# intellerce/controlanimate

Hardware: AMD Instinct MI355X
Metric: frames_per_sec (higher is better)
Workload: dtype fp16

## Files before the change

controlanimate_amd/_capi.py:

```python
from __future__ import annotations

import ctypes as C
import os

_HERE = os.path.dirname(os.path.abspath(__file__))
LIB_PATH = os.environ.get("CA_HIP_LIB") or os.path.join(_HERE, "csrc", "libcontrolanimate_hip.so")

CA_BF16, CA_F16 = 0, 1
CA_ACT_NONE, CA_ACT_SILU = 0, 1
ABI_VERSION = 15


class CAHipUnavailable(RuntimeError):
    pass


class CAHipError(RuntimeError):
    pass


class GemmArgs(C.Structure):
    _fields_ = [
        ("a", C.c_void_p), ("a2", C.c_void_p), ("w", C.c_void_p), ("c", C.c_void_p),
        ("bias", C.c_void_p), ("rowbias", C.c_void_p), ("residual", C.c_void_p),
        ("lda", C.c_int64), ("lda2", C.c_int64), ("ldc", C.c_int64), ("ld_res", C.c_int64),
        ("ld_rowbias", C.c_int64),
        ("m", C.c_int32), ("n", C.c_int32), ("k1", C.c_int32), ("k2", C.c_int32),
        ("rows_per_group", C.c_int32),
        ("alpha", C.c_float), ("post_scale", C.c_float),
        ("act", C.c_int32), ("geglu", C.c_int32), ("out_f32", C.c_int32), ("dtype", C.c_int32),
        ("ln_stats", C.c_void_p), ("ln_colsum", C.c_void_p), ("ln_eps", C.c_float),
        ("workspace", C.c_void_p), ("workspace_bytes", C.c_int64),
        ("row_sums_out", C.c_void_p), ("ln_parts", C.c_int32),
        ("w_frag", C.c_void_p),
    ]


class FfArgs(C.Structure):
    _fields_ = [
        ("x", C.c_void_p), ("w1_frag", C.c_void_p), ("bias1", C.c_void_p), ("colsum1", C.c_void_p), ("ln_stats", C.c_void_p),
        ("w2_frag", C.c_void_p), ("bias2", C.c_void_p), ("residual", C.c_void_p), ("y", C.c_void_p),
        ("lda", C.c_int64), ("ldc", C.c_int64), ("ld_res", C.c_int64),
        ("m", C.c_int32), ("c", C.c_int32), ("inner", C.c_int32), ("ln_eps", C.c_float), ("dtype", C.c_int32),
        ("w_out_frag", C.c_void_p), ("bias_out", C.c_void_p), ("residual_out", C.c_void_p), ("ld_res_out", C.c_int64),
    ]


class TattnArgs(C.Structure):
    _fields_ = [
        ("x", C.c_void_p), ("w_frag", C.c_void_p), ("gamma", C.c_void_p), ("bias_pe", C.c_void_p), ("o", C.c_void_p),
        ("lda", C.c_int64), ("ldo", C.c_int64), ("ld_bias_pe", C.c_int64),
        ("batch", C.c_int32), ("frames", C.c_int32), ("tokens", C.c_int32), ("heads", C.c_int32), ("c", C.c_int32),
        ("ln_eps", C.c_float), ("scale", C.c_float), ("dtype", C.c_int32),
        ("w_out_frag", C.c_void_p), ("bias_out", C.c_void_p), ("residual", C.c_void_p), ("ld_res", C.c_int64),
    ]


ATTN_WOUT_FRAG_ELEMS = 102400
TATTN_W_FRAG_ELEMS = 368640


class XattnArgs(C.Structure):
    _fields_ = [
        ("x", C.c_void_p), ("wq_frag", C.c_void_p), ("bias", C.c_void_p), ("kv_frag", C.c_void_p), ("o", C.c_void_p),
        ("lda", C.c_int64), ("ldo", C.c_int64),
        ("m", C.c_int32), ("tokens", C.c_int32), ("frames_per_kv", C.c_int32), ("kv_mod", C.c_int32), ("kv_batches", C.c_int32),
        ("nk", C.c_int32), ("heads", C.c_int32), ("c", C.c_int32),
        ("ln_eps", C.c_float), ("dtype", C.c_int32),
        ("w_out_frag", C.c_void_p), ("bias_out", C.c_void_p), ("residual", C.c_void_p), ("ld_res", C.c_int64),
        ("kv_frag_ip", C.c_void_p), ("nk_ip", C.c_int32), ("ip_scale", C.c_float),
    ]


XATTN_W_FRAG_ELEMS = 122880
XATTN_KV_FRAG_ELEMS = 7680


class ConvArgs(C.Structure):
    _fields_ = [
        ("x", C.c_void_p), ("x2", C.c_void_p), ("w", C.c_void_p), ("y", C.c_void_p),
        ("bias", C.c_void_p), ("rowbias", C.c_void_p), ("residual", C.c_void_p),
        ("ld_res", C.c_int64), ("ld_rowbias", C.c_int64),
        ("images", C.c_int32), ("hin", C.c_int32), ("win", C.c_int32),
        ("cin1", C.c_int32), ("cin2", C.c_int32), ("cout", C.c_int32),
        ("stride", C.c_int32), ("upsample", C.c_int32), ("rows_per_group", C.c_int32),
        ("alpha", C.c_float), ("post_scale", C.c_float),
        ("act", C.c_int32), ("out_f32", C.c_int32), ("dtype", C.c_int32),
        ("workspace", C.c_void_p), ("workspace_bytes", C.c_int64), ("pad_asym", C.c_int32),
        ("w_wino", C.c_void_p), ("x_is_wino_v", C.c_int32),
    ]


class GroupNormArgs(C.Structure):
    _fields_ = [
        ("x", C.c_void_p), ("x2", C.c_void_p), ("y", C.c_void_p),
        ("gamma", C.c_void_p), ("beta", C.c_void_p), ("partials", C.c_void_p),
        ("images", C.c_int32), ("hw", C.c_int32), ("c1", C.c_int32), ("c2", C.c_int32),
        ("groups", C.c_int32), ("frames_per_stat", C.c_int32),
        ("eps", C.c_float), ("act", C.c_int32), ("dtype", C.c_int32),
        ("wino_v", C.c_void_p), ("wino_h", C.c_int32), ("wino_w", C.c_int32),
    ]


class LayerNormArgs(C.Structure):
    _fields_ = [
        ("x", C.c_void_p), ("y", C.c_void_p), ("gamma", C.c_void_p), ("beta", C.c_void_p),
        ("pos", C.c_void_p),
        ("rows", C.c_int64),
        ("c", C.c_int32), ("rows_per_frame", C.c_int32), ("frames", C.c_int32),
        ("eps", C.c_float), ("dtype", C.c_int32), ("stats", C.c_void_p),
    ]


class AttnArgs(C.Structure):
    _fields_ = [
        ("q", C.c_void_p), ("k", C.c_void_p), ("v", C.c_void_p), ("o", C.c_void_p),
        ("q_outer", C.c_int64), ("q_inner", C.c_int64), ("q_row", C.c_int64),
        ("o_outer", C.c_int64), ("o_inner", C.c_int64), ("o_row", C.c_int64),
        ("k_outer", C.c_int64), ("k_inner", C.c_int64), ("k_row", C.c_int64),
        ("inner_count", C.c_int32), ("kv_inner_count", C.c_int32), ("kv_div", C.c_int32), ("kv_mod", C.c_int32),
        ("batches", C.c_int32), ("heads", C.c_int32), ("head_dim", C.c_int32),
        ("nq", C.c_int32), ("nk", C.c_int32),
        ("scale", C.c_float), ("out_scale", C.c_float),
        ("accumulate", C.c_int32), ("dtype", C.c_int32), ("causal", C.c_int32),
        ("key_mask", C.c_void_p), ("key_mask_stride", C.c_int64),
    ]


class ConvNarrowArgs(C.Structure):
    _fields_ = [
        ("x", C.c_void_p), ("w", C.c_void_p), ("y", C.c_void_p), ("bias", C.c_void_p), ("r1", C.c_void_p), ("r2", C.c_void_p),
        ("ldx", C.c_int64), ("ldy", C.c_int64), ("ld_r1", C.c_int64), ("ld_r2", C.c_int64),
        ("images", C.c_int32), ("hin", C.c_int32), ("win", C.c_int32), ("cin", C.c_int32), ("cout", C.c_int32),
        ("channel_offset", C.c_int32), ("upsample", C.c_int32), ("leaky_relu", C.c_int32),
        ("s0", C.c_float), ("s1", C.c_float), ("s2", C.c_float),
        ("out_u8", C.c_int32), ("dtype", C.c_int32),
    ]


SYMBOLS = {
    "ca_abi_version": (C.c_int, []),
    "ca_last_error": (C.c_char_p, []),
    "ca_gemm": (C.c_int, [C.POINTER(GemmArgs), C.c_void_p]),
    "ca_pack_w_frag": (C.c_int, [C.c_void_p, C.c_int32, C.c_int32, C.c_int32, C.c_void_p, C.c_void_p]),
    "ca_pack_w2_frag": (C.c_int, [C.c_void_p, C.c_int32, C.c_int32, C.c_void_p, C.c_void_p]),
    "ca_ff_fused": (C.c_int, [C.POINTER(FfArgs), C.c_void_p]),
    "ca_ff_fused_supported": (C.c_int, [C.POINTER(FfArgs)]),
    "ca_tattn_fused": (C.c_int, [C.POINTER(TattnArgs), C.c_void_p]),
    "ca_tattn_fused_supported": (C.c_int, [C.POINTER(TattnArgs)]),
    "ca_pack_w_tattn": (C.c_int, [C.c_void_p, C.c_int32, C.c_int32, C.c_void_p, C.c_void_p]),
    "ca_pack_w_out": (C.c_int, [C.c_void_p, C.c_int32, C.c_int32, C.c_void_p, C.c_void_p]),
    "ca_xattn_fused": (C.c_int, [C.POINTER(XattnArgs), C.c_void_p]),
    "ca_xattn_fused_supported": (C.c_int, [C.POINTER(XattnArgs)]),
    "ca_xattn_pack_w": (C.c_int, [C.c_void_p, C.c_int32, C.c_int32, C.c_void_p, C.c_void_p]),
    "ca_xattn_pack_kv": (C.c_int, [C.c_void_p, C.c_int64, C.c_int32, C.c_int32, C.c_int32, C.c_int32, C.c_float, C.c_int32, C.c_void_p, C.c_void_p]),
    "ca_gemm_ln_inline_supported": (C.c_int, [C.POINTER(GemmArgs)]),
    "ca_gemm_wants_finished_stats": (C.c_int, [C.POINTER(GemmArgs)]),
    "ca_ln_finish_sums": (C.c_int, [C.c_void_p, C.c_int, C.c_int64, C.c_int, C.c_float, C.c_void_p, C.c_void_p]),
    "ca_gemm_workspace_bytes": (C.c_int64, [C.POINTER(GemmArgs)]),
    "ca_gemm_row_sums_parts": (C.c_int, [C.POINTER(GemmArgs)]),
    "ca_gemm_plan_name": (C.c_int, [C.POINTER(GemmArgs), C.c_char_p, C.c_int32]),
    "ca_conv3x3_plan_name": (C.c_int, [C.POINTER(ConvArgs), C.c_char_p, C.c_int32]),
    "ca_conv3x3": (C.c_int, [C.POINTER(ConvArgs), C.c_void_p]),
    "ca_pack_w_wino": (C.c_int, [C.c_void_p, C.c_int32, C.c_int32, C.c_int32, C.c_void_p, C.c_void_p]),
    "ca_conv3x3_workspace_bytes": (C.c_int64, [C.POINTER(ConvArgs)]),
    "ca_softmax_rows": (C.c_int, [C.c_void_p, C.c_void_p, C.c_int64, C.c_int32, C.c_int64, C.c_int64, C.c_float, C.c_int32, C.c_void_p]),
    "ca_groupnorm_partials_floats": (C.c_int64, [C.c_int32, C.c_int32, C.c_int32, C.c_int32]),
    "ca_groupnorm_stats": (C.c_int, [C.POINTER(GroupNormArgs), C.c_void_p]),
    "ca_groupnorm_apply": (C.c_int, [C.POINTER(GroupNormArgs), C.c_void_p]),
    "ca_groupnorm": (C.c_int, [C.POINTER(GroupNormArgs), C.c_void_p]),
    "ca_groupnorm_wino_supported": (C.c_int, [C.POINTER(GroupNormArgs)]),
    "ca_layernorm": (C.c_int, [C.POINTER(LayerNormArgs), C.c_void_p]),
    "ca_attention": (C.c_int, [C.POINTER(AttnArgs), C.c_void_p]),
    "ca_attention_plan_name": (C.c_int, [C.POINTER(AttnArgs), C.c_char_p, C.c_int32]),
    "ca_add_bcast": (C.c_int, [C.c_void_p, C.c_void_p, C.c_void_p, C.c_int64, C.c_int64, C.c_int32, C.c_void_p]),
    "ca_repeat": (C.c_int, [C.c_void_p, C.c_void_p, C.c_int64, C.c_int32, C.c_void_p]),
    "ca_silu_f32": (C.c_int, [C.c_void_p, C.c_void_p, C.c_int64, C.c_void_p]),
    "ca_timestep_embedding": (C.c_int, [C.c_void_p, C.c_float, C.c_void_p, C.c_int32, C.c_int32, C.c_int32, C.c_void_p]),
    "ca_latents_to_nhwc": (C.c_int, [C.c_void_p, C.c_void_p, C.c_int32, C.c_int32, C.c_int32, C.c_int32, C.c_int32,
                                      C.c_int32, C.c_int32, C.c_float, C.c_int32, C.c_void_p]),
    "ca_nhwc_to_ncfhw_f32": (C.c_int, [C.c_void_p, C.c_void_p, C.c_int32, C.c_int32, C.c_int32, C.c_int32, C.c_int32,
                                        C.c_int32, C.c_int32, C.c_int32, C.c_void_p]),
    "ca_ncfhw_to_nhwc": (C.c_int, [C.c_void_p, C.c_int32, C.POINTER(C.c_int64), C.c_void_p, C.c_int32, C.c_int32,
                                    C.c_int32, C.c_int32, C.c_int32, C.c_int32, C.c_int32, C.c_void_p]),
    "ca_cfg_scheduler_step": (C.c_int, [C.c_void_p, C.c_int32, C.c_int32, C.c_float, C.c_void_p, C.c_void_p,
                                         C.c_void_p, C.c_void_p, C.c_int32, C.c_int32, C.c_int32, C.c_int32,
                                         C.POINTER(C.c_float), C.c_float, C.c_void_p]),
    "ca_lincomb": (C.c_int, [C.c_void_p, C.POINTER(C.c_void_p), C.POINTER(C.c_float), C.c_int32, C.c_int64, C.c_void_p]),
    "ca_conv3x3_narrow": (C.c_int, [C.POINTER(ConvNarrowArgs), C.c_void_p]),
    "ca_conv3x3_narrow_plan_name": (C.c_int, [C.POINTER(ConvNarrowArgs), C.c_char_p, C.c_int32]),
    "ca_rgb8_to_nhwc": (C.c_int, [C.c_void_p, C.c_void_p, C.c_int32, C.c_int32, C.c_int32, C.c_int32, C.c_void_p]),
    "ca_resize_lanczos4_u8": (C.c_int, [C.c_void_p, C.c_void_p, C.c_int32, C.c_int32, C.c_int32, C.c_int32, C.c_int32,
                                         C.c_void_p, C.c_void_p, C.c_void_p, C.c_void_p, C.c_void_p]),
    "ca_color_match_workspace_bytes": (C.c_int64, [C.c_int32, C.c_int64]),
    "ca_hist_u8x3": (C.c_int, [C.c_void_p, C.c_void_p, C.c_int32, C.c_int64, C.c_void_p]),
    "ca_color_moments_f64": (C.c_int, [C.c_void_p, C.c_void_p, C.c_void_p, C.c_void_p, C.c_int32, C.c_int64, C.c_void_p, C.c_int64, C.c_void_p]),
    "ca_color_transform_f64": (C.c_int, [C.c_void_p, C.c_void_p, C.c_void_p, C.c_void_p, C.c_void_p, C.c_void_p, C.c_int32, C.c_int64, C.c_void_p]),
    "ca_sort_f64_segments": (C.c_int, [C.c_void_p, C.c_void_p, C.c_int32, C.c_int64, C.c_void_p, C.c_int64, C.c_void_p]),
    "ca_color_rank_map_f64": (C.c_int, [C.c_void_p, C.c_void_p, C.c_void_p, C.c_void_p, C.c_void_p, C.c_void_p, C.c_int32, C.c_int64,
                                         C.c_void_p, C.c_int64, C.c_void_p]),
    "ca_color_finish_u8": (C.c_int, [C.c_void_p, C.c_void_p, C.c_int32, C.c_int64, C.c_int32, C.c_void_p, C.c_int64, C.c_void_p]),
}

_lib = None


def lib() -> C.CDLL:
    global _lib
    if _lib is not None:
        return _lib
    import torch
    if not os.path.exists(LIB_PATH):
        raise CAHipUnavailable(
            f"{LIB_PATH} is missing: the HIP extension is not built. Run "
            "`python -m controlanimate_amd._build` (needs hipcc); there is no CPU fallback.")
    try:
        handle = C.CDLL(LIB_PATH)
    except OSError as e:
        raise CAHipUnavailable(f"cannot load {LIB_PATH}: {e}") from e
    for name, (res, args) in SYMBOLS.items():
        fn = getattr(handle, name)
        fn.restype = res
        fn.argtypes = args
    if handle.ca_abi_version() != ABI_VERSION:
        raise CAHipUnavailable(f"ABI mismatch: library {handle.ca_abi_version()} vs binding {ABI_VERSION}; rebuild")
    _lib = handle
    return handle


def check(rc: int, what: str) -> None:
    if rc != 0:
        msg = lib().ca_last_error()
        raise CAHipError(f"{what} failed with code {rc}: {msg.decode() if msg else ''}")
```

controlanimate_amd/attention_processor.py:

```python
from __future__ import annotations

from typing import Optional

import torch
from torch import nn

from . import kernels as K
from .context import dispatch
from .layers import HipLinear, LnFold, WeightArena, ln_fold_enabled, pack_concat_rows


class AttnProcessor2_0(nn.Module):

    num_tokens = 0
    drop_ip_tokens = False

    def __init__(self, hidden_size=None, cross_attention_dim=None):
        super().__init__()

    def ip_branch(self, attn, q, ctx, out, images, tokens, kv_rows, frames_per_kv, kv_mod, cache):
        return out

    def ip_fragments(self, attn, ctx, cache):
        return None

    def __call__(self, attn: "Attention", hidden_states: torch.Tensor, encoder_hidden_states: Optional[torch.Tensor] = None,
                 attention_mask=None, temb=None, *, residual: Optional[torch.Tensor] = None, frames_per_kv: int = 1,
                 kv_mod: int = 0, temporal=None, cache: Optional[dict] = None, ln=None, row_sums: bool = False) -> torch.Tensor:
        if attention_mask is not None:
            raise NotImplementedError("attention_mask is not used anywhere on the reference's path")
        B, N, C = hidden_states.shape
        x = hidden_states.reshape(B * N, C)
        res = None if residual is None else residual.reshape(B * N, C)
        if ln is not None and encoder_hidden_states is None and temporal is not None and getattr(attn, "tfrag", None) is not None:
            b, f, n = temporal
            ofrag = getattr(attn, "ofrag", None)
            if ofrag is not None and dispatch.attn_out_fused:
                to_out = attn.to_out[0]
                out = K.tattn_fused(x, attn.tfrag.t, attn.tgamma.t, attn.tbias_pe.t, b, f, n, attn.heads, attn.tln_eps, attn.scale,
                                    w_out_frag=ofrag.t, bias_out=None if to_out.b is None else to_out.b.t, residual=res)
                if out is not None:
                    return out.reshape(B, N, C)
            o = K.tattn_fused(x, attn.tfrag.t, attn.tgamma.t, attn.tbias_pe.t, b, f, n, attn.heads, attn.tln_eps, attn.scale)
            if o is not None:
                out = attn.to_out[0].run(o, residual=res, row_sums=row_sums)
                return K.carry_row_sums(out.reshape(B, N, C), out)
        builtin = type(self).ip_branch is AttnProcessor2_0.ip_branch
        with_ip = (not builtin and type(self).ip_fragments is not AttnProcessor2_0.ip_fragments and dispatch.attn_out_fused and dispatch.xattn_ip_fused
                   and getattr(attn, "ofrag", None) is not None)
        if (ln is not None and encoder_hidden_states is not None and cache is not None and getattr(attn, "xfrag", None) is not None
                and (builtin or with_ip)):
            ctx = encoder_hidden_states
            nb, L, cd = ctx.shape
            nk = L - self.num_tokens
            kv = cache.get(("kv", id(attn)))
            if kv is None:
                kv = cache[("kv", id(attn))] = K.gemm(ctx.reshape(nb * L, cd), attn.kv.t)
            ent = cache.get(("kvf", id(attn)))
            if ent is None:
                ent = cache[("kvf", id(attn))] = (K.xattn_pack_kv(kv, nb, L, nk, attn.scale), nk, L)
            if ent[0] is not None and ent[1] == nk:
                ofrag = getattr(attn, "ofrag", None)
                if ofrag is not None and dispatch.attn_out_fused:
                    to_out = attn.to_out[0]
                    ipf = self.ip_fragments(attn, ctx, cache) if with_ip else None
                    if not with_ip or ipf is not None:
                        out = K.xattn_fused(x, attn.xfrag.t, ln[1].b.t, ent[0], B, N, frames_per_kv, kv_mod, nk, ln[1].eps, w_out_frag=ofrag.t,
                                            bias_out=None if to_out.b is None else to_out.b.t, residual=res,
                                            kv_frag_ip=None if ipf is None else ipf[0], nk_ip=0 if ipf is None else ipf[1],
                                            ip_scale=1.0 if ipf is None else ipf[2])
                        if out is not None:
                            return out.reshape(B, N, C)
                o = K.xattn_fused(x, attn.xfrag.t, ln[1].b.t, ent[0], B, N, frames_per_kv, kv_mod, nk, ln[1].eps) if builtin else None
                if o is not None:
                    out = attn.to_out[0].run(o, residual=res, row_sums=row_sums)
                    return K.carry_row_sums(out.reshape(B, N, C), out)
        if ln is not None:
            st, fold = ln
            if encoder_hidden_states is None and temporal is not None and fold.pe is not None:
                b, f, n = temporal
                qkv = K.gemm(x, fold.w.t, bias=fold.b.t, ln=(st, fold.cs.t), rowbias=fold.rowbias(b, f), rows_per_group=n)
            else:
                qkv = K.gemm(x, fold.w.t, bias=fold.b.t, ln=(st, fold.cs.t))
        if encoder_hidden_states is None:
            if ln is None:
                qkv = K.gemm(x, attn.qkv.t)
            if temporal is not None:
                b, f, n = temporal
                o = K.attention_temporal(qkv, b, f, n, attn.heads)
            else:
                o = K.attention_spatial(qkv, B, N, attn.heads)
        else:
            ctx = encoder_hidden_states
            nb, L, cd = ctx.shape
            q = qkv if ln is not None else K.gemm(x, attn.to_q.w.t)
            kv = None if cache is None else cache.get(("kv", id(attn)))
            if kv is None:
                kv = K.gemm(ctx.reshape(nb * L, cd), attn.kv.t)
                if cache is not None:
                    cache[("kv", id(attn))] = kv
            nk = L - self.num_tokens
            o = K.attention_cross(q, kv, B, N, attn.heads, nk, L, frames_per_kv, kv_mod=kv_mod)
            o = self.ip_branch(attn, q, ctx, o, B, N, L, frames_per_kv, kv_mod, cache)
        out = attn.to_out[0].run(o, residual=res, row_sums=row_sums)
        return K.carry_row_sums(out.reshape(B, N, C), out)


class IPAttnProcessor2_0(AttnProcessor2_0):

    def __init__(self, hidden_size, cross_attention_dim=None, scale=1.0, num_tokens=4):
        super().__init__()
        self.hidden_size = hidden_size
        self.cross_attention_dim = cross_attention_dim
        self.scale = scale
        self.num_tokens = num_tokens
        self.to_k_ip = HipLinear(cross_attention_dim or hidden_size, hidden_size, bias=False)
        self.to_v_ip = HipLinear(cross_attention_dim or hidden_size, hidden_size, bias=False)
        self.kv_ip = None

    def pack(self, arena: WeightArena, dtype):
        self.kv_ip = pack_concat_rows(arena, dtype, [self.to_k_ip, self.to_v_ip])

    def _kv_ip(self, ctx, cache):
        if self.kv_ip is None:
            raise RuntimeError("IPAttnProcessor2_0 installed after prepare(); call model.prepare() again")
        nb, L, cd = ctx.shape
        kvip = None if cache is None else cache.get(("kv_ip", id(self)))
        if kvip is None:
            kvip = K.gemm(ctx.reshape(nb * L, cd), self.kv_ip.t)
            if cache is not None:
                cache[("kv_ip", id(self))] = kvip
        return kvip

    def ip_fragments(self, attn, ctx, cache):
        nb, L, cd = ctx.shape
        if cache is None or not (1 <= self.num_tokens <= 16):
            return None
        ent = cache.get(("kvf_ip", id(self)))
        if ent is None:
            kvip = self._kv_ip(ctx, cache)
            ent = cache[("kvf_ip", id(self))] = (K.xattn_pack_kv(kvip, nb, L, self.num_tokens, attn.scale, row_offset=L - self.num_tokens),
                                                 self.num_tokens, L, attn.scale)
        if ent[0] is None or ent[1] != self.num_tokens or ent[2] != L:
            return None
        return ent[0], self.num_tokens, float(self.scale)

    def ip_branch(self, attn, q, ctx, out, images, tokens, kv_rows, frames_per_kv, kv_mod, cache):
        nb, L, cd = ctx.shape
        kvip = self._kv_ip(ctx, cache)
        return K.attention_cross(q, kvip, images, tokens, attn.heads, self.num_tokens, L, frames_per_kv, out=out,
                                 out_scale=float(self.scale), accumulate=True, kv_row_offset=L - self.num_tokens,
                                 kv_mod=kv_mod)


class CNAttnProcessor2_0(AttnProcessor2_0):

    def __init__(self, num_tokens=4):
        super().__init__()
        self.num_tokens = num_tokens


AttnProcessor = AttnProcessor2_0
IPAttnProcessor = IPAttnProcessor2_0
CNAttnProcessor = CNAttnProcessor2_0


class Attention(nn.Module):

    def __init__(self, query_dim: int, cross_attention_dim: Optional[int] = None, heads: int = 8, dim_head: int = 64,
                 dropout: float = 0.0, bias: bool = False, upcast_attention: bool = False, processor=None, **_):
        super().__init__()
        inner = heads * dim_head
        self.is_cross = cross_attention_dim is not None
        ctx_dim = cross_attention_dim if self.is_cross else query_dim
        self.query_dim, self.cross_attention_dim, self.inner_dim = query_dim, ctx_dim, inner
        self.heads = heads
        self.scale = dim_head ** -0.5
        self.spatial_norm = None
        self.group_norm = None
        self.norm_cross = None
        self.residual_connection = False
        self.rescale_output_factor = 1.0
        self.to_q = HipLinear(query_dim, inner, bias=bias)
        self.to_k = HipLinear(ctx_dim, inner, bias=bias)
        self.to_v = HipLinear(ctx_dim, inner, bias=bias)
        self.to_out = nn.ModuleList([HipLinear(inner, query_dim, bias=True), nn.Identity()])
        self.processor = processor if processor is not None else AttnProcessor2_0()
        self.qkv = self.kv = self.fold = None

    def set_processor(self, processor, _remove_lora: bool = False):
        if isinstance(getattr(self, "processor", None), nn.Module) and not isinstance(processor, nn.Module):
            self._modules.pop("processor", None)
        self.processor = processor

    def get_processor(self, return_deprecated_lora: bool = False):
        return self.processor

    def builtin_processor(self) -> bool:
        return type(self.processor) in (AttnProcessor2_0, IPAttnProcessor2_0, CNAttnProcessor2_0)

    def pack(self, arena: WeightArena, dtype, fold_ln=None, pe=None):
        self.fold = None
        if fold_ln is not None and self.builtin_processor() and ln_fold_enabled():
            self.fold = LnFold(arena, dtype, fold_ln, [self.to_q] if self.is_cross else [self.to_q, self.to_k, self.to_v], pe=pe)
            if self.is_cross:
                self.kv = pack_concat_rows(arena, dtype, [self.to_k, self.to_v])
                self.xfrag = None
                if (self.heads, self.inner_dim, self.query_dim) == (8, 320, 320):
                    from .layers import frag_order_xattn
                    fold = self.fold
                    self.xfrag = arena.add((122880,), dtype, lambda: frag_order_xattn(fold.w_fold().to(dtype).float()))
        elif self.is_cross:
            self.to_q.pack(arena, dtype)
            self.kv = pack_concat_rows(arena, dtype, [self.to_k, self.to_v])
        else:
            self.qkv = pack_concat_rows(arena, dtype, [self.to_q, self.to_k, self.to_v])
        self.to_out[0].pack(arena, dtype)
        self.ofrag = None
        if (self.heads, self.inner_dim, self.query_dim) == (8, 320, 320) and self.fold is not None:
            from .layers import _f32, frag_order_wout
            to_out = self.to_out[0]
            self.ofrag = arena.add((102400,), dtype, lambda: frag_order_wout(_f32(to_out.weight)))
        if hasattr(self.processor, "pack"):
            self.processor.pack(arena, dtype)

    def forward(self, hidden_states, encoder_hidden_states=None, attention_mask=None, **kw):
        return self.processor(self, hidden_states, encoder_hidden_states=encoder_hidden_states,
                              attention_mask=attention_mask, **kw)
```

controlanimate_amd/context.py:

```python
from __future__ import annotations

from dataclasses import dataclass, field
from typing import Optional

import torch


@dataclass
class ExecCtx:
    b: int
    f: int
    dtype: torch.dtype
    temb: torch.Tensor
    emb_groups: int
    ehs: Optional[torch.Tensor] = None
    frames_per_kv: int = 1
    kv_mod: int = 0
    gn_frames_per_stat: int = 1
    cache: dict = field(default_factory=dict)

    @property
    def images(self) -> int:
        return self.b * self.f

    def rows_per_emb_group(self, h: int, w: int) -> int:
        return self.images // self.emb_groups * h * w


class Dispatch:
    gemm_ar = True
    ff_fused = True
    tattn_fused = True
    xattn_fused = True
    attn_out_fused = True
    xattn_ip_fused = True
    conv_winograd = True
    gn_winograd = True
    ln_row_sums = True
    repeat_kernel = True
    ln_fold = True
    cfg_shared = True
    cn_cfg_dedup = True
    controlnet_streams = 2


dispatch = Dispatch()
```

controlanimate_amd/csrc/ca_attn_out.h:

```cpp
__device__ __forceinline__ int ca_wout_col(int j, int i) { return j < 4 ? 32 * (j >> 1) + 8 * (i >> 2) + 4 * (j & 1) + (i & 3) : 64 + i; }

constexpr int CA_WOUT_ELEMS = 320 * 320;

__global__ __launch_bounds__(256) void k_pack_w_out(const u16* __restrict__ w, u16* __restrict__ dst) {
  const int idx = blockIdx.x * 256 + threadIdx.x;
  if (idx >= CA_WOUT_ELEMS / 8) return;
  const int L = idx & 63;
  int t = idx >> 6;
  const int j = t % 5;
  t /= 5;
  const int kq = t % 10;
  const int cg = t / 10;
  const int row = cg * 80 + ca_wout_col(j, L & 15);
  st16(dst + (int64_t)idx * 8, ld16(w + (int64_t)row * 320 + kq * 32 + (L >> 4) * 8));
}

__device__ __forceinline__ void ca_lds_store8(unsigned char* p, u32x2 v) {
  const unsigned addr = (unsigned)(size_t)(__attribute__((address_space(3))) unsigned char*)p;
  asm volatile("ds_write_b64 %0, %1" ::"v"(addr), "v"(v) : "memory");
}

struct AttnOutParams {
  const u16* wof;
  const float* bias;
  const u16* res;
  int ld_res;
  unsigned res_bytes;
};

struct AttnOutRegs {
  u32x4 fb[2][5];
  u32x4 rr[4][2];
  u32x2 r4[4];
};

__device__ __forceinline__ unsigned attn_out_row(unsigned row_base, unsigned step_a, unsigned step_b, int i) { return row_base + (unsigned)(i & 1) * step_a + (unsigned)(i >> 1) * step_b; }

template <int DT>
__device__ __forceinline__ void attn_out_prefetch(AttnOutRegs& R, const AttnOutParams& a, __amdgpu_buffer_rsrc_t rs_wo, __amdgpu_buffer_rsrc_t rs_res, int wid,
                                                  int lane, unsigned row_base, unsigned step_a, unsigned step_b) {
  const int cg = wid & 3, g = lane >> 4;
  const unsigned wv = (unsigned)lane * 16u;
  const unsigned wbase = (unsigned)cg * (10u * 5u * 1024u);
#pragma unroll
  for (int c = 0; c < 2; ++c)
#pragma unroll
    for (int j = 0; j < 5; ++j) R.fb[c][j] = __builtin_bit_cast(u32x4, __builtin_amdgcn_raw_buffer_load_b128(rs_wo, wv, wbase + (unsigned)(c * 5 + j) * 1024u, 0));
#pragma unroll
  for (int i = 0; i < 4; ++i) {
    const unsigned ro = attn_out_row(row_base, step_a, step_b, i) * (unsigned)a.ld_res * 2u + (unsigned)(cg * 80) * 2u;
    R.rr[i][0] = __builtin_bit_cast(u32x4, __builtin_amdgcn_raw_buffer_load_b128(rs_res, ro + (unsigned)(8 * g) * 2u, 0, 0));
    R.rr[i][1] = __builtin_bit_cast(u32x4, __builtin_amdgcn_raw_buffer_load_b128(rs_res, ro + (unsigned)(32 + 8 * g) * 2u, 0, 0));
    R.r4[i] = __builtin_bit_cast(u32x2, __builtin_amdgcn_raw_buffer_load_b64(rs_res, ro + (unsigned)(64 + 4 * g) * 2u, 0, 0));
  }
}

template <int DT>
__device__ __forceinline__ unsigned attn_out_add(unsigned w, unsigned r_) {
  if (DT == CA_F16) {
    unsigned s_;
    asm("v_pk_add_f16 %0, %1, %2" : "=v"(s_) : "v"(w), "v"(r_));
    return s_;
  }
  return pack2<DT>(Elem<DT>::to_f((u16)(w & 0xffffu)) + Elem<DT>::to_f((u16)(r_ & 0xffffu)), Elem<DT>::to_f((u16)(w >> 16)) + Elem<DT>::to_f((u16)(r_ >> 16)));
}

template <int DT>
__device__ __forceinline__ void attn_out_run(AttnOutRegs& R, const unsigned char* tile, const int (&fa_b)[2][2], const AttnOutParams& a,
                                             __amdgpu_buffer_rsrc_t rs_wo, __amdgpu_buffer_rsrc_t rs_bo, __amdgpu_buffer_rsrc_t rs_y, int wid, int lane,
                                             unsigned row_base, unsigned step_a, unsigned step_b, unsigned ldo) {
  constexpr int KQ = 10, ROWB = 640;
  const int rh = wid >> 2, cg = wid & 3;
  int lane_k = lane;
  asm volatile("" : "+v"(lane_k));
  const unsigned wv = (unsigned)lane_k * 16u;
  const unsigned wbase = (unsigned)cg * (10u * 5u * 1024u);
  f32x4 acc[4][5];
  u32x4 fa[4];
#pragma unroll
  for (int i = 0; i < 4; ++i) fa[i] = ld16(tile + fa_b[rh][0] + i * 16 * ROWB);
  __builtin_amdgcn_sched_barrier(0);
#pragma unroll
  for (int kq = 0; kq < KQ; ++kq) {
    const int nk = kq + 1;
    const int fa_off = (nk >> 1) * 128;
#pragma unroll
    for (int j = 0; j < 5; ++j) {
      __builtin_amdgcn_s_setprio(1);
#pragma unroll
      for (int i = 0; i < 4; ++i) {
        if (kq == 0) acc[i][j] = Elem<DT>::mfma(R.fb[0][j], fa[i], (f32x4){0.f, 0.f, 0.f, 0.f});
        else acc[i][j] = Elem<DT>::mfma(R.fb[kq & 1][j], fa[i], acc[i][j]);
        if (j == 4 && nk < KQ) {
          __builtin_amdgcn_sched_barrier(0);
          fa[i] = ld16(tile + fa_b[rh][nk & 1] + fa_off + i * 16 * ROWB);
          __builtin_amdgcn_sched_barrier(0);
        }
      }
      __builtin_amdgcn_s_setprio(0);
      __builtin_amdgcn_sched_barrier(0);
      if (kq + 2 < KQ) R.fb[kq & 1][j] = __builtin_bit_cast(u32x4, __builtin_amdgcn_raw_buffer_load_b128(rs_wo, wv, wbase + (unsigned)(((kq + 2) * 5 + j) * 1024), 0));
      __builtin_amdgcn_sched_barrier(0);
    }
  }
  int lane_e = lane;
  asm volatile("" : "+v"(lane_e));
  const int g = lane_e >> 4;
  f32x4 bi[5];
#pragma unroll
  for (int j = 0; j < 5; ++j) {
    const unsigned c4 = (unsigned)(cg * 80 + (j < 4 ? 32 * (j >> 1) + 8 * g + 4 * (j & 1) : 64 + 4 * g)) * 4u;
    bi[j] = __builtin_bit_cast(f32x4, __builtin_amdgcn_raw_buffer_load_b128(rs_bo, c4, 0, 0));
  }
  unsigned w[4][10];
#pragma unroll
  for (int i = 0; i < 4; ++i) {
#pragma unroll
    for (int j = 0; j < 5; ++j) {
      w[i][2 * j] = pack2<DT>(acc[i][j][0] + bi[j][0], acc[i][j][1] + bi[j][1]);
      w[i][2 * j + 1] = pack2<DT>(acc[i][j][2] + bi[j][2], acc[i][j][3] + bi[j][3]);
    }
    if (a.res) {
#pragma unroll
      for (int k = 0; k < 8; ++k) w[i][k] = attn_out_add<DT>(w[i][k], R.rr[i][k >> 2][k & 3]);
      w[i][8] = attn_out_add<DT>(w[i][8], R.r4[i][0]);
      w[i][9] = attn_out_add<DT>(w[i][9], R.r4[i][1]);
    }
  }
  __builtin_amdgcn_sched_barrier(0);
#pragma unroll
  for (int i = 0; i < 4; ++i) {
    const unsigned ro = attn_out_row(row_base, step_a, step_b, i) * ldo * 2u + (unsigned)(cg * 80) * 2u;
    __builtin_amdgcn_raw_buffer_store_b128((u32x4){w[i][0], w[i][1], w[i][2], w[i][3]}, rs_y, ro + (unsigned)(8 * g) * 2u, 0, 0);
    __builtin_amdgcn_raw_buffer_store_b128((u32x4){w[i][4], w[i][5], w[i][6], w[i][7]}, rs_y, ro + (unsigned)(32 + 8 * g) * 2u, 0, 0);
    __builtin_amdgcn_raw_buffer_store_b64((u32x2){w[i][8], w[i][9]}, rs_y, ro + (unsigned)(64 + 4 * g) * 2u, 0, 0);
  }
  __builtin_amdgcn_sched_barrier(0);
}
```

controlanimate_amd/csrc/ca_gemm_ar.hip:

```cpp
#include "ca_gemm_core.h"
#include <atomic>

__attribute__((visibility("hidden"))) int ar_cu_count() {
  static std::atomic<int> cache[64];
  int dev = 0;
  if (hipGetDevice(&dev) != hipSuccess || dev < 0 || dev >= 64) dev = 0;
  int n = cache[dev].load(std::memory_order_relaxed);
  if (n <= 0) {
    hipDeviceProp_t prop;
    n = (hipGetDeviceProperties(&prop, dev) == hipSuccess && prop.multiProcessorCount > 0) ? prop.multiProcessorCount : 256;
    cache[dev].store(n, std::memory_order_relaxed);
  }
  return n;
}

namespace {
using namespace ca_gemm_detail;
#include "ca_gemm_ar.h"
#include "ca_attn_out.h"
#include "ca_ff_fused.h"
#include "ca_tattn_fused.h"
#include "ca_xattn_fused.h"

template <int DT>
int launch_ar(const GemmKParams& p, hipStream_t st) {
  const int tiles_m = (p.m + 127) / 128;
  const unsigned c_bytes = (unsigned)((((int64_t)p.m - 1) * p.ldc + (p.geglu ? p.n / 2 : p.n)) * 2);
  const unsigned res_bytes = p.res ? (unsigned)((((int64_t)p.m - 1) * p.ld_res + p.n) * 2) : 0u;
  const int slots = 2 * ar_cu_count();
  const unsigned grid = (unsigned)(tiles_m < slots ? tiles_m : slots);
  float* ws = p.ln_inline ? p.partial : nullptr;
  if (p.geglu) hipLaunchKernelGGL((k_gemm_ar<DT, 2>), dim3(grid), dim3(256), 0, st, p, p.wf, tiles_m, c_bytes, 0u, ws);
  else if (p.ln_colsum) hipLaunchKernelGGL((k_gemm_ar<DT, 1>), dim3(grid), dim3(256), 0, st, p, p.wf, tiles_m, c_bytes, 0u, ws);
  else hipLaunchKernelGGL((k_gemm_ar<DT, 0>), dim3(grid), dim3(256), 0, st, p, p.wf, tiles_m, c_bytes, res_bytes, ws);
  return CA_OK;
}
}

int ca_launch_gemm_ar(const ca_gemm_detail::GemmKParams& p0, int dtype, hipStream_t st) {
  static const int dbg = CA_KNOB("CA_PP_DBG", 0);
  ca_gemm_detail::GemmKParams p = p0;
  p.dbg = dbg;
  return dtype == CA_BF16 ? launch_ar<CA_BF16>(p, st) : launch_ar<CA_F16>(p, st);
}

extern "C" int ca_pack_w_frag(const void* w, int32_t n, int32_t k, int32_t geglu, void* dst, void* stream) {
  CA_REQUIRE(w && dst, "ca_pack_w_frag: null operand");
  CA_REQUIRE(k == 320 && n > 0 && n % 64 == 0, "ca_pack_w_frag: n=%d (multiple of 64) k=%d (320)", n, k);
  CA_REQUIRE((((uintptr_t)w | (uintptr_t)dst) & 15) == 0, "ca_pack_w_frag: operands must be 16-byte aligned");
  const int64_t pieces = (int64_t)n * 40;
  hipLaunchKernelGGL(k_pack_w_frag, dim3((unsigned)((pieces + 255) / 256)), dim3(256), 0, (hipStream_t)stream, (const u16*)w, (u16*)dst, n, geglu);
  CA_CHECK_LAUNCH("ca_pack_w_frag");
  return CA_OK;
}

extern "C" int ca_pack_w2_frag(const void* w, int32_t n, int32_t k, void* dst, void* stream) {
  CA_REQUIRE(w && dst, "ca_pack_w2_frag: null operand");
  CA_REQUIRE(n == 320 && k == 1280, "ca_pack_w2_frag: n=%d k=%d (320 x 1280)", n, k);
  CA_REQUIRE((((uintptr_t)w | (uintptr_t)dst) & 15) == 0, "ca_pack_w2_frag: operands must be 16-byte aligned");
  hipLaunchKernelGGL(k_pack_w2_frag, dim3(200), dim3(256), 0, (hipStream_t)stream, (const u16*)w, (u16*)dst);
  CA_CHECK_LAUNCH("ca_pack_w2_frag");
  return CA_OK;
}

static int attn_out_args_ok(const void* w_out_frag, const float* bias_out, const void* residual, int64_t ld_res, int64_t rows) {
  if (!w_out_frag) return (bias_out || residual) ? 0 : 1;
  if ((((uintptr_t)w_out_frag | (uintptr_t)bias_out | (uintptr_t)residual) & 15) != 0) return 0;
  if (residual && (ld_res % 8 || ld_res < 320 || ((rows - 1) * ld_res + 320) * 2 >= 0x7FFFFF00ll)) return 0;
  return 1;
}

extern "C" int ca_ff_fused_supported(const ca_ff_args* a) {
  if (!a || !a->x || !a->w1_frag || !a->bias1 || !a->colsum1 || !a->w2_frag || !a->y) return 0;
  if (a->c != 320 || a->inner != 1280 || a->m < 16384) return 0;
  if (a->dtype != CA_BF16 && a->dtype != CA_F16) return 0;
  if (a->lda % 8 || a->ldc % 8 || (a->residual && a->ld_res % 8)) return 0;
  if (a->lda < 320 || a->ldc < 320 || (a->residual && a->ld_res < 320)) return 0;
  if ((((uintptr_t)a->x | (uintptr_t)a->y | (uintptr_t)a->w1_frag | (uintptr_t)a->w2_frag | (uintptr_t)a->residual) & 15) != 0) return 0;
  if (((uintptr_t)a->ln_stats & 7) != 0 || (((uintptr_t)a->bias1 | (uintptr_t)a->colsum1 | (uintptr_t)a->bias2) & 15) != 0) return 0;
  const int64_t lim = 0x7FFFFF00ll;
  if (((int64_t)(a->m - 1) * a->lda + 320) * 2 >= lim || ((int64_t)(a->m - 1) * a->ldc + 320) * 2 >= lim) return 0;
  if (a->residual && ((int64_t)(a->m - 1) * a->ld_res + 320) * 2 >= lim) return 0;
  if (!a->ln_stats && !(a->ln_eps > 0.f)) return 0;
  if (!attn_out_args_ok(a->w_out_frag, a->bias_out, a->residual_out, a->ld_res_out, a->m)) return 0;
  if (a->w_out_frag && a->m % 128) return 0;
  return 1;
}

extern "C" int ca_ff_fused(const ca_ff_args* a, void* stream) {
  CA_REQUIRE(a != nullptr, "ca_ff_fused: null args");
  CA_REQUIRE(ca_ff_fused_supported(a), "ca_ff_fused: arguments outside what the fused feed-forward takes (C = 320, inner 1280, M >= 16384, fragment-ordered weights, "
                                        "16-byte aligned operands, 32-bit byte offsets): ask ca_ff_fused_supported() first");
  FfParams p{};
  p.x = (const u16*)a->x;
  p.w1f = (const u16*)a->w1_frag;
  p.bias1 = a->bias1;
  p.cs1 = a->colsum1;
  p.w2f = (const u16*)a->w2_frag;
  p.bias2 = a->bias2;
  p.res = (const u16*)a->residual;
  p.y = (u16*)a->y;
  p.ln_stats = a->ln_stats;
  p.lda = a->lda, p.ldc = a->ldc, p.ld_res = a->ld_res;
  p.m = a->m;
  p.ln_eps = a->ln_eps;
  p.x_bytes = (unsigned)(((int64_t)(a->m - 1) * a->lda + 320) * 2);
  p.y_bytes = (unsigned)(((int64_t)(a->m - 1) * a->ldc + 320) * 2);
  p.res_bytes = a->residual ? (unsigned)(((int64_t)(a->m - 1) * a->ld_res + 320) * 2) : 0u;
  if (a->w_out_frag) {
    p.out.wof = (const u16*)a->w_out_frag;
    p.out.bias = a->bias_out;
    p.out.res = (const u16*)a->residual_out;
    p.out.ld_res = (int)a->ld_res_out;
    p.out.res_bytes = a->residual_out ? (unsigned)(((int64_t)(a->m - 1) * a->ld_res_out + 320) * 2) : 0u;
  }
  const int tiles_m = (a->m + 127) / 128;
  const unsigned grid = (unsigned)(tiles_m < ar_cu_count() ? tiles_m : ar_cu_count());
  if (a->w_out_frag) {
    if (a->dtype == CA_BF16) hipLaunchKernelGGL((k_ff_fused<CA_BF16, true>), dim3(grid), dim3(512), 0, (hipStream_t)stream, p, tiles_m);
    else hipLaunchKernelGGL((k_ff_fused<CA_F16, true>), dim3(grid), dim3(512), 0, (hipStream_t)stream, p, tiles_m);
  } else {
    if (a->dtype == CA_BF16) hipLaunchKernelGGL((k_ff_fused<CA_BF16, false>), dim3(grid), dim3(512), 0, (hipStream_t)stream, p, tiles_m);
    else hipLaunchKernelGGL((k_ff_fused<CA_F16, false>), dim3(grid), dim3(512), 0, (hipStream_t)stream, p, tiles_m);
  }
  CA_CHECK_LAUNCH("ca_ff_fused");
  return CA_OK;
}

extern "C" int ca_pack_w_tattn(const void* w, int32_t n, int32_t k, void* dst, void* stream) {
  CA_REQUIRE(w && dst, "ca_pack_w_tattn: null operand");
  CA_REQUIRE(n == 960 && k == 320, "ca_pack_w_tattn: n=%d k=%d (Wq | Wk | Wv rows: 960 x 320)", n, k);
  CA_REQUIRE((((uintptr_t)w | (uintptr_t)dst) & 15) == 0, "ca_pack_w_tattn: operands must be 16-byte aligned");
  static_assert(CA_TATTN_WF_ELEMS == CA_TATTN_W_FRAG_ELEMS, "header constant");
  hipLaunchKernelGGL(k_pack_w_tattn, dim3((CA_TATTN_WF_ELEMS / 8 + 255) / 256), dim3(256), 0, (hipStream_t)stream, (const u16*)w, (u16*)dst);
  CA_CHECK_LAUNCH("ca_pack_w_tattn");
  return CA_OK;
}

extern "C" int ca_pack_w_out(const void* w, int32_t n, int32_t k, void* dst, void* stream) {
  CA_REQUIRE(w && dst, "ca_pack_w_out: null operand");
  CA_REQUIRE(n == 320 && k == 320, "ca_pack_w_out: n=%d k=%d (to_out[0].weight: 320 x 320)", n, k);
  CA_REQUIRE((((uintptr_t)w | (uintptr_t)dst) & 15) == 0, "ca_pack_w_out: operands must be 16-byte aligned");
  static_assert(CA_WOUT_ELEMS == CA_ATTN_WOUT_FRAG_ELEMS, "header constant");
  hipLaunchKernelGGL(k_pack_w_out, dim3((CA_WOUT_ELEMS / 8 + 255) / 256), dim3(256), 0, (hipStream_t)stream, (const u16*)w, (u16*)dst);
  CA_CHECK_LAUNCH("ca_pack_w_out");
  return CA_OK;
}

extern "C" int ca_tattn_fused_supported(const ca_tattn_args* a) {
  if (!a || !a->x || !a->w_frag || !a->gamma || !a->bias_pe || !a->o) return 0;
  if (a->c != 320 || a->heads != 8 || a->batch < 1) return 0;
  if (a->frames != 16 && !((a->frames == 8 || a->frames == 32) && a->w_out_frag)) return 0;
  {
    const int px = 128 / a->frames;
    if (a->tokens < px || a->tokens % px) return 0;
  }
  if (a->dtype != CA_BF16 && a->dtype != CA_F16) return 0;
  const int64_t rows = (int64_t)a->batch * a->frames * a->tokens;
  if (rows < 16384) return 0;
  if (a->lda % 8 || a->ldo % 8 || a->lda < 320 || a->ldo < 320 || a->ld_bias_pe % 4 || a->ld_bias_pe < 320) return 0;
  if ((((uintptr_t)a->x | (uintptr_t)a->o | (uintptr_t)a->w_frag | (uintptr_t)a->gamma | (uintptr_t)a->bias_pe) & 15) != 0) return 0;
  const int64_t lim = 0x7FFFFF00ll;
  if (((rows - 1) * a->lda + 320) * 2 >= lim || ((rows - 1) * a->ldo + 320) * 2 >= lim) return 0;
  if (!(a->ln_eps > 0.f) || !(a->scale > 0.f)) return 0;
  if (!attn_out_args_ok(a->w_out_frag, a->bias_out, a->residual, a->ld_res, rows)) return 0;
  return 1;
}

extern "C" int ca_tattn_fused(const ca_tattn_args* a, void* stream) {
  CA_REQUIRE(a != nullptr, "ca_tattn_fused: null args");
  CA_REQUIRE(ca_tattn_fused_supported(a), "ca_tattn_fused: arguments outside what the fused temporal attention takes (C = 320, 8 heads, 16 frames -- or 8 / 32 with w_out_frag --, tokens %% (128 / frames) == 0, "
                                           ">= 16384 rows, fragment-ordered weights, 16-byte aligned operands, 32-bit byte offsets): ask ca_tattn_fused_supported() first");
  const int64_t rows = (int64_t)a->batch * a->frames * a->tokens;
  TattnParams p{};
  p.x = (const u16*)a->x;
  p.wf = (const u16*)a->w_frag;
  p.gamma = a->gamma;
  p.bp = a->bias_pe;
  p.o = (u16*)a->o;
  p.lda = (int)a->lda, p.ldo = (int)a->ldo, p.ld_bp = (int)a->ld_bias_pe;
  p.hw = a->tokens;
  p.ln_eps = a->ln_eps;
  p.scale_log2 = a->scale * 1.4426950408889634f;
  p.x_bytes = (unsigned)(((rows - 1) * a->lda + 320) * 2);
  p.o_bytes = (unsigned)(((rows - 1) * a->ldo + 320) * 2);
  const int tiles = (int)((int64_t)a->batch * a->tokens / (128 / a->frames));
  static const int dbg = CA_KNOB("CA_TATTN_DBG", 0);
  p.dbg = dbg;
  if (a->w_out_frag) {
    p.out.wof = (const u16*)a->w_out_frag;
    p.out.bias = a->bias_out;
    p.out.res = (const u16*)a->residual;
    p.out.ld_res = (int)a->ld_res;
    p.out.res_bytes = a->residual ? (unsigned)(((rows - 1) * a->ld_res + 320) * 2) : 0u;
    const unsigned grid1 = (unsigned)(tiles < ar_cu_count() ? tiles : ar_cu_count());
#define CA_TATTN_OUT(FR)                                                                                                              \
  if (a->dtype == CA_BF16) hipLaunchKernelGGL((k_tattn_out<CA_BF16, FR>), dim3(grid1), dim3(512), 0, (hipStream_t)stream, p, tiles); \
  else hipLaunchKernelGGL((k_tattn_out<CA_F16, FR>), dim3(grid1), dim3(512), 0, (hipStream_t)stream, p, tiles);
    if (a->frames == 8) { CA_TATTN_OUT(8) }
    else if (a->frames == 32) { CA_TATTN_OUT(32) }
    else { CA_TATTN_OUT(16) }
#undef CA_TATTN_OUT
    CA_CHECK_LAUNCH("ca_tattn_fused(out)");
    return CA_OK;
  }
  const int slots = (dbg & 16) ? ar_cu_count() : 2 * ar_cu_count();
  const unsigned grid = (unsigned)(tiles < slots ? tiles : slots);
  if (a->dtype == CA_BF16) hipLaunchKernelGGL((k_tattn_fused<CA_BF16>), dim3(grid), dim3(256), 0, (hipStream_t)stream, p, tiles);
  else hipLaunchKernelGGL((k_tattn_fused<CA_F16>), dim3(grid), dim3(256), 0, (hipStream_t)stream, p, tiles);
  CA_CHECK_LAUNCH("ca_tattn_fused");
  return CA_OK;
}

extern "C" int ca_xattn_pack_w(const void* w, int32_t n, int32_t k, void* dst, void* stream) {
  CA_REQUIRE(w && dst, "ca_xattn_pack_w: null operand");
  CA_REQUIRE(n == 320 && k == 320, "ca_xattn_pack_w: n=%d k=%d (Wq: 320 x 320)", n, k);
  CA_REQUIRE((((uintptr_t)w | (uintptr_t)dst) & 15) == 0, "ca_xattn_pack_w: operands must be 16-byte aligned");
  static_assert(CA_XATTN_WF_ELEMS == CA_XATTN_W_FRAG_ELEMS && CA_XATTN_KVF_ELEMS == CA_XATTN_KV_FRAG_ELEMS, "header constants");
  hipLaunchKernelGGL(k_xattn_pack_w, dim3((CA_XATTN_WF_ELEMS / 8 + 255) / 256), dim3(256), 0, (hipStream_t)stream, (const u16*)w, (u16*)dst);
  CA_CHECK_LAUNCH("ca_xattn_pack_w");
  return CA_OK;
}

extern "C" int ca_xattn_pack_kv(const void* kv, int64_t ld, int32_t kv_batches, int32_t rows_per_batch, int32_t row_offset, int32_t nk, float scale, int32_t dtype,
                                void* dst, void* stream) {
  CA_REQUIRE(kv && dst, "ca_xattn_pack_kv: null operand");
  CA_REQUIRE(kv_batches > 0 && rows_per_batch > 0 && row_offset >= 0 && ((nk > 64 && nk <= 80) || (nk >= 1 && nk <= 16)) && row_offset + nk <= rows_per_batch && ld >= 640,
             "ca_xattn_pack_kv: kv_batches=%d rows_per_batch=%d row_offset=%d nk=%d (65..80 text keys, or 1..16 image-prompt tokens) ld=%lld (>= 640: K | V of 8 heads x 40)", kv_batches, rows_per_batch, row_offset, nk,
             (long long)ld);
  CA_REQUIRE(dtype == CA_BF16 || dtype == CA_F16, "ca_xattn_pack_kv: dtype %d", dtype);
  CA_REQUIRE(((uintptr_t)dst & 15) == 0 && scale > 0.f, "ca_xattn_pack_kv: dst must be 16-byte aligned, scale > 0");
  const float sl2 = scale * 1.4426950408889634f;
  if (dtype == CA_BF16) hipLaunchKernelGGL((k_xattn_pack_kv<CA_BF16>), dim3((unsigned)kv_batches * 8), dim3(64), 0, (hipStream_t)stream, (const u16*)kv, ld, rows_per_batch, row_offset, nk, sl2, (u16*)dst);
  else hipLaunchKernelGGL((k_xattn_pack_kv<CA_F16>), dim3((unsigned)kv_batches * 8), dim3(64), 0, (hipStream_t)stream, (const u16*)kv, ld, rows_per_batch, row_offset, nk, sl2, (u16*)dst);
  CA_CHECK_LAUNCH("ca_xattn_pack_kv");
  return CA_OK;
}

extern "C" int ca_xattn_fused_supported(const ca_xattn_args* a) {
  if (!a || !a->x || !a->wq_frag || !a->kv_frag || !a->o) return 0;
  if (a->c != 320 || a->heads != 8 || a->m < 16384 || a->tokens < 128 || a->tokens % 128 || a->m % a->tokens) return 0;
  if (a->nk <= 64 || a->nk > 80 || a->frames_per_kv < 1 || a->kv_mod < 1) return 0;
  {
    const int images = a->m / a->tokens;
    const int groups = (images + a->frames_per_kv - 1) / a->frames_per_kv;
    const int needed = groups < a->kv_mod ? groups : a->kv_mod;
    if (a->kv_batches < needed) return 0;
  }
  if (a->dtype != CA_BF16 && a->dtype != CA_F16) return 0;
  if (a->lda % 8 || a->ldo % 8 || a->lda < 320 || a->ldo < 320) return 0;
  if ((((uintptr_t)a->x | (uintptr_t)a->o | (uintptr_t)a->wq_frag | (uintptr_t)a->kv_frag | (uintptr_t)a->bias) & 15) != 0) return 0;
  const int64_t lim = 0x7FFFFF00ll;
  if (((int64_t)(a->m - 1) * a->lda + 320) * 2 >= lim || ((int64_t)(a->m - 1) * a->ldo + 320) * 2 >= lim) return 0;
  if (!(a->ln_eps > 0.f)) return 0;
  if (!attn_out_args_ok(a->w_out_frag, a->bias_out, a->residual, a->ld_res, a->m)) return 0;
  if (a->kv_frag_ip) {
    if (!a->w_out_frag || a->nk_ip < 1 || a->nk_ip > 16 || ((uintptr_t)a->kv_frag_ip & 15) != 0 || !(a->ip_scale == a->ip_scale) || a->ip_scale - a->ip_scale != 0.f) return 0;
  } else if (a->nk_ip != 0) {
    return 0;
  }
  return 1;
}

extern "C" int ca_xattn_fused(const ca_xattn_args* a, void* stream) {
  CA_REQUIRE(a != nullptr, "ca_xattn_fused: null args");
  CA_REQUIRE(ca_xattn_fused_supported(a), "ca_xattn_fused: arguments outside what the fused text cross-attention takes (C = 320, 8 heads, 65..80 keys, tokens %% 128 == 0, "
                                           ">= 16384 rows, packed weights and K / V, 16-byte aligned operands, 32-bit byte offsets): ask ca_xattn_fused_supported() first");
  XattnParams p{};
  p.x = (const u16*)a->x;
  p.wf = (const u16*)a->wq_frag;
  p.bias = a->bias;
  p.kvf = (const u16*)a->kv_frag;
  p.o = (u16*)a->o;
  p.lda = (int)a->lda, p.ldo = (int)a->ldo;
  p.m = a->m, p.tokens = a->tokens, p.frames_per_kv = a->frames_per_kv, p.kv_mod = a->kv_mod, p.nk = a->nk;
  p.ln_eps = a->ln_eps;
  p.x_bytes = (unsigned)(((int64_t)(a->m - 1) * a->lda + 320) * 2);
  p.o_bytes = (unsigned)(((int64_t)(a->m - 1) * a->ldo + 320) * 2);
  p.kvf_bytes = (unsigned)((int64_t)a->kv_batches * 8 * CA_XATTN_KVF_ELEMS * 2);
  const int tiles = a->m / 128;
  if (a->w_out_frag) {
    p.out.wof = (const u16*)a->w_out_frag;
    p.out.bias = a->bias_out;
    p.out.res = (const u16*)a->residual;
    p.out.ld_res = (int)a->ld_res;
    p.out.res_bytes = a->residual ? (unsigned)(((int64_t)(a->m - 1) * a->ld_res + 320) * 2) : 0u;
    const unsigned grid1 = (unsigned)(tiles < ar_cu_count() ? tiles : ar_cu_count());
    if (a->kv_frag_ip) {
      p.kvf_ip = (const u16*)a->kv_frag_ip, p.nk_ip = a->nk_ip, p.ip_scale = a->ip_scale;
      if (a->dtype == CA_BF16) hipLaunchKernelGGL((k_xattn_out<CA_BF16, true>), dim3(grid1), dim3(512), 0, (hipStream_t)stream, p, tiles);
      else hipLaunchKernelGGL((k_xattn_out<CA_F16, true>), dim3(grid1), dim3(512), 0, (hipStream_t)stream, p, tiles);
    } else if (a->dtype == CA_BF16) hipLaunchKernelGGL((k_xattn_out<CA_BF16, false>), dim3(grid1), dim3(512), 0, (hipStream_t)stream, p, tiles);
    else hipLaunchKernelGGL((k_xattn_out<CA_F16, false>), dim3(grid1), dim3(512), 0, (hipStream_t)stream, p, tiles);
    CA_CHECK_LAUNCH("ca_xattn_fused(out)");
    return CA_OK;
  }
  const int slots = 2 * ar_cu_count();
  const unsigned grid = (unsigned)(tiles < slots ? tiles : slots);
  if (a->dtype == CA_BF16) hipLaunchKernelGGL((k_xattn_fused<CA_BF16>), dim3(grid), dim3(256), 0, (hipStream_t)stream, p, tiles);
  else hipLaunchKernelGGL((k_xattn_fused<CA_F16>), dim3(grid), dim3(256), 0, (hipStream_t)stream, p, tiles);
  CA_CHECK_LAUNCH("ca_xattn_fused");
  return CA_OK;
}

#ifdef CA_EXPERIMENTS
extern "C" int ca_debug_ff_stamps(unsigned long long* out) {
  return hipMemcpyFromSymbol(out, HIP_SYMBOL(ca_ff_stamps), sizeof(unsigned long long) * 512) == hipSuccess ? 0 : -1;
}
#endif
```

controlanimate_amd/csrc/ca_tattn_fused.h:

```cpp
template <int N>
struct IntC {
  static constexpr int value = N;
};

struct TattnParams {
  const u16* x;
  const u16* wf;
  const float* gamma;
  const float* bp;
  u16* o;
  int lda, ldo, ld_bp;
  int hw;
  float ln_eps, scale_log2;
  unsigned x_bytes, o_bytes;
  int dbg;
  AttnOutParams out;
};

constexpr int CA_TATTN_WF_ELEMS = 4 * 2 * 3 * 10 * 3 * 64 * 8;

__global__ __launch_bounds__(256) void k_pack_w_tattn(const u16* __restrict__ w, u16* __restrict__ dst) {
  const int idx = blockIdx.x * 256 + threadIdx.x;
  if (idx >= CA_TATTN_WF_ELEMS / 8) return;
  const int L = idx & 63;
// ... 346 lines not shown
      constexpr int PS = decltype(pass_c)::value;
#pragma unroll
      for (int kq = 0; kq < KQ; ++kq) {
        const int nk = (kq + 1) % KQ;
        const int fa_off = (nk >> 1) * 128;
#pragma unroll
        for (int j = 0; j < TJ; ++j) {
          __builtin_amdgcn_s_setprio(1);
#pragma unroll
          for (int i = 0; i < TM; ++i) {
            const f32x4 c0 = kq == 0 ? (f32x4){0.f, 0.f, 0.f, 0.f} : acc[i][j];
            if (PS == 2) acc[i][j] = Elem<DT>::mfma(fa[i], fb[kq & 1][j], c0);
            else acc[i][j] = Elem<DT>::mfma(fb[kq & 1][j], fa[i], c0);
            if (j == TJ - 1) {
              __builtin_amdgcn_sched_barrier(0);
              fa[i] = ld16(xb + fa_b[i >> 2][nk & 1] + fa_off + (i & 3) * 16 * ROWB);
              __builtin_amdgcn_sched_barrier(0);
            }
          }
          __builtin_amdgcn_s_setprio(0);
          __builtin_amdgcn_sched_barrier(0);
          const int sn = PS * 10 + kq + 2;
          if (sn < 30) fb[kq & 1][j] = __builtin_bit_cast(u32x4, __builtin_amdgcn_raw_buffer_load_b128(rs_w, wv, whead + (unsigned)(sn * TJ + j) * 1024u, 0));
          __builtin_amdgcn_sched_barrier(0);
        }
      }
    };

    u32x2 qp[TM][TJ];
    {
      f32x4 acc[TM][TJ];
      kloop(IntC<0>{}, acc);
#pragma unroll
      for (int i = 0; i < TM; ++i)
#pragma unroll
        for (int j = 0; j < TJ; ++j)
          qp[i][j] = (u32x2){pack2<DT>(acc[i][j][0] * p.scale_log2, acc[i][j][1] * p.scale_log2), pack2<DT>(acc[i][j][2] * p.scale_log2, acc[i][j][3] * p.scale_log2)};
    }
    u32x2 pp[TM][FR == 32 ? 2 : 1];
    {
      f32x4 acc[TM][TJ];
      kloop(IntC<1>{}, acc);
      int lane_s = lane;
      asm volatile("" : "+v"(lane_s));
      const int l15s = lane_s & 15, gs = lane_s >> 4;
      if constexpr (FR != 32) {
#pragma unroll
        for (int i = 0; i < TM; ++i) {
          f32x4 st = {0.f, 0.f, 0.f, 0.f};
#pragma unroll
          for (int j = 0; j < TJ; ++j) {
            const u32x2 kp = {pack2<DT>(acc[i][j][0], acc[i][j][1]), pack2<DT>(acc[i][j][2], acc[i][j][3])};
            st = Elem<DT>::mfma16(kp, qp[i][j], st);
          }
          if constexpr (FR == 8) {
            if ((gs >> 1) != (l15s >> 3)) st = (f32x4){-INFINITY, -INFINITY, -INFINITY, -INFINITY};
          }
          const float m = rowgroup_max(fmaxf(fmaxf(st[0], st[1]), fmaxf(st[2], st[3])));
          float e[4];
#pragma unroll
          for (int r = 0; r < 4; ++r) e[r] = __builtin_amdgcn_exp2f(st[r] - m);
          const float inv = __builtin_amdgcn_rcpf(rowgroup_sum((e[0] + e[1]) + (e[2] + e[3])));
          pp[i][0] = (u32x2){pack2<DT>(e[0] * inv, e[1] * inv), pack2<DT>(e[2] * inv, e[3] * inv)};
        }
      } else {
#pragma unroll
        for (int px = 0; px < 4; ++px) {
          u32x2 kp[2][TJ];
#pragma unroll
          for (int kt = 0; kt < 2; ++kt)
#pragma unroll
            for (int j = 0; j < TJ; ++j)
              kp[kt][j] = (u32x2){pack2<DT>(acc[2 * px + kt][j][0], acc[2 * px + kt][j][1]), pack2<DT>(acc[2 * px + kt][j][2], acc[2 * px + kt][j][3])};
#pragma unroll
          for (int qt = 0; qt < 2; ++qt) {
            f32x4 st[2];
#pragma unroll
            for (int kt = 0; kt < 2; ++kt) {
              st[kt] = (f32x4){0.f, 0.f, 0.f, 0.f};
#pragma unroll
              for (int j = 0; j < TJ; ++j) st[kt] = Elem<DT>::mfma16(kp[kt][j], qp[2 * px + qt][j], st[kt]);
            }
            const float m = rowgroup_max(fmaxf(fmaxf(fmaxf(st[0][0], st[0][1]), fmaxf(st[0][2], st[0][3])), fmaxf(fmaxf(st[1][0], st[1][1]), fmaxf(st[1][2], st[1][3]))));
            float e[2][4], l = 0.f;
#pragma unroll
            for (int kt = 0; kt < 2; ++kt)
#pragma unroll
              for (int r = 0; r < 4; ++r) {
                e[kt][r] = __builtin_amdgcn_exp2f(st[kt][r] - m);
                l += e[kt][r];
              }
            const float inv = __builtin_amdgcn_rcpf(rowgroup_sum(l));
#pragma unroll
            for (int kt = 0; kt < 2; ++kt) pp[2 * px + kt][qt] = (u32x2){pack2<DT>(e[kt][0] * inv, e[kt][1] * inv), pack2<DT>(e[kt][2] * inv, e[kt][3] * inv)};
          }
        }
      }
    }
    u32x2 op[TM][TJ];
    {
      f32x4 acc[TM][TJ];
      kloop(IntC<2>{}, acc);
      if constexpr (FR != 32) {
#pragma unroll
        for (int i = 0; i < TM; ++i)
#pragma unroll
          for (int j = 0; j < TJ; ++j) {
            const u32x2 vp = {pack2<DT>(acc[i][j][0], acc[i][j][1]), pack2<DT>(acc[i][j][2], acc[i][j][3])};
            const f32x4 ot = Elem<DT>::mfma16(vp, pp[i][0], (f32x4){0.f, 0.f, 0.f, 0.f});
            op[i][j] = (u32x2){pack2<DT>(ot[0], ot[1]), pack2<DT>(ot[2], ot[3])};
          }
      } else {
#pragma unroll
        for (int px = 0; px < 4; ++px)
#pragma unroll
          for (int j = 0; j < TJ; ++j) {
            u32x2 vp[2];
#pragma unroll
            for (int kt = 0; kt < 2; ++kt) vp[kt] = (u32x2){pack2<DT>(acc[2 * px + kt][j][0], acc[2 * px + kt][j][1]), pack2<DT>(acc[2 * px + kt][j][2], acc[2 * px + kt][j][3])};
#pragma unroll
            for (int qt = 0; qt < 2; ++qt) {
              f32x4 ot = Elem<DT>::mfma16(vp[0], pp[2 * px][qt], (f32x4){0.f, 0.f, 0.f, 0.f});
              ot = Elem<DT>::mfma16(vp[1], pp[2 * px + 1][qt], ot);
              op[2 * px + qt][j] = (u32x2){pack2<DT>(ot[0], ot[1]), pack2<DT>(ot[2], ot[3])};
            }
          }
      }
    }
    int lane_e = lane;
    asm volatile("" : "+v"(lane_e));
    const int l15e = lane_e & 15, ge = lane_e >> 4;
    const int rh_ = wid >> 2;
    const unsigned row_base = FR == 16 ? (unsigned)((bimg * 16 + l15e) * p.hw + pix0 + 4 * rh_)
                                       : FR == 32 ? (unsigned)((bimg * 32 + l15e) * p.hw + pix0 + 2 * rh_) : (unsigned)((bimg * 8 + (l15e & 7)) * p.hw + pix0 + 8 * rh_ + (l15e >> 3));
    const unsigned step_a = FR == 16 ? 1u : FR == 32 ? 16u * (unsigned)p.hw : 2u, step_b = FR == 16 ? 2u : FR == 32 ? 1u : 4u;
    AttnOutRegs R;
    attn_out_prefetch<DT>(R, p.out, rs_wo, rs_res, wid, lane_e, row_base, step_a, step_b);
    __syncthreads();
#pragma unroll
    for (int i = 0; i < TM; ++i)
#pragma unroll
      for (int j = 0; j < TJ; ++j) {
        const int dv = 16 * j + 4 * ge;
        if (dv < HD) {
          const int col = wid * HD + dv;
          ca_lds_store8(xb + (16 * i + l15e) * ROWB + (((col >> 3) ^ ((l15e >> 1) & 7)) << 4) + (col & 7) * 2, op[i][j]);
        }
      }
    asm volatile("s_waitcnt lgkmcnt(0)" ::: "memory");
    __syncthreads();
    attn_out_run<DT>(R, xb, fa_b, p.out, rs_wo, rs_bo, rs_o, wid, lane_e, row_base, step_a, step_b, (unsigned)p.ldo);
  }
}
```

controlanimate_amd/csrc/ca_xattn_fused.h:

```cpp
struct XattnParams {
  const u16* x;
  const u16* wf;
  const float* bias;
  const u16* kvf;
  u16* o;
  int lda, ldo;
  int m, tokens, frames_per_kv, kv_mod, nk;
  float ln_eps;
  unsigned x_bytes, o_bytes, kvf_bytes;
  AttnOutParams out;
  const u16* kvf_ip;
  int nk_ip;
  float ip_scale;
};

constexpr int CA_XATTN_WF_ELEMS = 4 * 2 * 10 * 3 * 64 * 8;
constexpr int CA_XATTN_KVF_ELEMS = 30 * 64 * 4;

__global__ __launch_bounds__(256) void k_xattn_pack_w(const u16* __restrict__ w, u16* __restrict__ dst) {
  const int idx = blockIdx.x * 256 + threadIdx.x;
  if (idx >= CA_XATTN_WF_ELEMS / 8) return;
  const int L = idx & 63;
  int t = idx >> 6;
  const int j = t % 3;
  t /= 3;
  const int kq = t % 10;
  t /= 10;
  const int hi = t & 1, wv = t >> 1;
  const int dd = 16 * j + (L & 15);
  const u32x4 zero4 = {0u, 0u, 0u, 0u};
  st16(dst + (int64_t)idx * 8, dd < 40 ? ld16(w + (int64_t)((wv + 4 * hi) * 40 + dd) * 320 + kq * 32 + (L >> 4) * 8) : zero4);
}

template <int DT>
__global__ __launch_bounds__(64) void k_xattn_pack_kv(const u16* __restrict__ kv, int64_t ld, int rows_per_batch, int row_offset, int nk, float scale_log2,
                                                      u16* __restrict__ dst) {
  const int head = blockIdx.x & 7, zk = blockIdx.x >> 3;
  const int L = threadIdx.x, g = L >> 4, l15 = L & 15;
  const u16* kp = kv + ((int64_t)zk * rows_per_batch + row_offset) * ld + head * 40;
  const u16* vp = kp + 320;
  u16* out = dst + ((int64_t)blockIdx.x * 30 * 64 + L) * 4;
#pragma unroll 1
  for (int f = 0; f < 15; ++f) {
    const int kt = f / 3, c = f - kt * 3;
    const int key = 16 * kt + l15, d0 = 16 * c + 4 * g;
    float v[4];
#pragma unroll
    for (int r = 0; r < 4; ++r) v[r] = (key < nk && d0 + r < 40) ? Elem<DT>::to_f(kp[(int64_t)key * ld + d0 + r]) * scale_log2 : 0.f;
    *reinterpret_cast<u32x2*>(out + (int64_t)f * 64 * 4) = (u32x2){pack2<DT>(v[0], v[1]), pack2<DT>(v[2], v[3])};
  }
#pragma unroll 1
  for (int f = 0; f < 15; ++f) {
    const int j = f / 5, kt = f - j * 5;
    const int dv = 16 * j + l15, k0 = 16 * kt + 4 * g;
    u16 v[4];
#pragma unroll
    for (int r = 0; r < 4; ++r) v[r] = (k0 + r < nk && dv < 40) ? vp[(int64_t)(k0 + r) * ld + dv] : (u16)0;
    *reinterpret_cast<u32x2*>(out + (int64_t)(15 + f) * 64 * 4) = (u32x2){(unsigned)v[0] | ((unsigned)v[1] << 16), (unsigned)v[2] | ((unsigned)v[3] << 16)};
  }
}

template <int DT>
__global__ __launch_bounds__(256, 2) void k_xattn_fused(XattnParams p, int tiles) {
  constexpr int K = 320, KQ = 10, TM = 8, TJ = 3, BM = 128, HD = 40, KT = 5;
  constexpr int ROWB = K * 2;
  constexpr unsigned CHUNKB = TJ * 1024u;
  __shared__ __attribute__((aligned(16))) unsigned char smem[BM * ROWB];
  static_assert(2 * BM * ROWB <= 160 * 1024, "two blocks per CU");

  const int tid = threadIdx.x;
  const int lane = tid & 63;
  const int wid = __builtin_amdgcn_readfirstlane(tid >> 6);
  const int g = lane >> 4, l15 = lane & 15;
  constexpr unsigned OOB_V = 0x80000000u;

  const __amdgpu_buffer_rsrc_t rs_x = __builtin_amdgcn_make_buffer_rsrc((void*)p.x, 0, p.x_bytes, 0x00020000);
  const __amdgpu_buffer_rsrc_t rs_w = __builtin_amdgcn_make_buffer_rsrc((void*)p.wf, 0, (unsigned)CA_XATTN_WF_ELEMS * 2u, 0x00020000);
  const __amdgpu_buffer_rsrc_t rs_o = __builtin_amdgcn_make_buffer_rsrc((void*)p.o, 0, p.o_bytes, 0x00020000);
  const __amdgpu_buffer_rsrc_t rs_kv = __builtin_amdgcn_make_buffer_rsrc((void*)p.kvf, 0, p.kvf_bytes, 0x00020000);
  const __amdgpu_buffer_rsrc_t rs_bi = __builtin_amdgcn_make_buffer_rsrc((void*)(p.bias ? (const void*)p.bias : (const void*)p.wf), 0, p.bias ? 320u * 4u : 0u, 0x00020000);

  const int f_sw = (l15 >> 1) & 7;
  const int fa_lane = l15 * ROWB + (((f_sw >> 2) << 2) + (g ^ (f_sw & 3))) * 16;
  int fa_b[2][2] = {{fa_lane, fa_lane ^ 64}, {fa_lane + 4 * 16 * ROWB, (fa_lane ^ 64) + 4 * 16 * ROWB}};
  asm volatile("" : "+v"(fa_b[0][0]), "+v"(fa_b[0][1]), "+v"(fa_b[1][0]), "+v"(fa_b[1][1]));

  for (int tile = blockIdx.x; tile < tiles; tile += gridDim.x) {
    const int m0 = tile * BM;
    const int zk = ((m0 / p.tokens) / p.frames_per_kv) % p.kv_mod;
    __syncthreads();
    {
      int lane_o = lane;
      asm volatile("" : "+v"(lane_o));
#pragma unroll
      for (int q = 0; q < 20; ++q) {
        const unsigned idx = (unsigned)((wid * 20 + q) * 64 + lane_o);
        const unsigned r = __umulhi(idx >> 3, 0xCCCCCCCDu) >> 2;
        const unsigned cp = idx - r * 40u;
        const unsigned c = cp ^ ((r >> 1) & 7u);
        const unsigned off = (m0 + (int)r) < p.m ? (unsigned)(m0 + (int)r) * (unsigned)p.lda * 2u + c * 16u : OOB_V;
        __builtin_amdgcn_raw_ptr_buffer_load_lds(rs_x, (__attribute__((address_space(3))) void*)(smem + (wid * 20 + q) * 1024), 16, off, 0, 0, 0);
      }
    }
    asm volatile("s_waitcnt vmcnt(0)" ::: "memory");
    __syncthreads();
    {
      const int r = tid >> 1, h = tid & 1;
      unsigned char* src = smem + r * ROWB + h * 320;
      float s = 0.f, ss = 0.f;
#pragma unroll 4
      for (int q = 0; q < 20; ++q) {
        const u32x4 v = ld16(src + q * 16);
#pragma unroll
        for (int e = 0; e < 4; ++e) {
          const float a0 = Elem<DT>::to_f((u16)(v[e] & 0xffffu)), a1 = Elem<DT>::to_f((u16)(v[e] >> 16));
          s += a0 + a1;
          ss = fmaf(a0, a0, fmaf(a1, a1, ss));
        }
      }
      s += __shfl_xor(s, 1);
      ss += __shfl_xor(ss, 1);
      const float mean = s * (1.f / K);
      const float rstd = rsqrtf(fmaxf(ss * (1.f / K) - mean * mean, 0.f) + p.ln_eps);
      const float nb = -mean * rstd;
#pragma unroll 4
      for (int q = 0; q < 20; ++q) {
        u32x4 v = ld16(src + q * 16);
#pragma unroll
        for (int e = 0; e < 4; ++e) {
          const float a0 = Elem<DT>::to_f((u16)(v[e] & 0xffffu)), a1 = Elem<DT>::to_f((u16)(v[e] >> 16));
          v[e] = pack2<DT>(fmaf(a0, rstd, nb), fmaf(a1, rstd, nb));
        }
        st16(src + q * 16, v);
      }
    }
    __syncthreads();

    int lane_k = lane;
    asm volatile("" : "+v"(lane_k));
    const unsigned wv = (unsigned)lane_k * 16u;
    const unsigned wwave = (unsigned)wid * (20u * CHUNKB);
    u32x4 fa[TM], fb[2][TJ];
#pragma unroll
    for (int c = 0; c < 2; ++c)
#pragma unroll
      for (int j = 0; j < TJ; ++j) fb[c][j] = __builtin_bit_cast(u32x4, __builtin_amdgcn_raw_buffer_load_b128(rs_w, wv, wwave + (unsigned)(c * TJ + j) * 1024u, 0));
#pragma unroll
    for (int i = 0; i < TM; ++i) fa[i] = ld16(smem + fa_b[i >> 2][0] + (i & 3) * 16 * ROWB);
    __builtin_amdgcn_sched_barrier(0);

    for (int hi = 0; hi < 2; ++hi) {
      const int head = wid + 4 * hi;
      const unsigned whead = wwave + (unsigned)hi * (10u * CHUNKB);
      const unsigned kvb = (unsigned)(zk * 8 + head) * (unsigned)(CA_XATTN_KVF_ELEMS * 2) + (unsigned)lane_k * 8u;
      u32x2 kf[KT][TJ], vf[TJ][KT];
      f32x4 acc[TM][TJ];
#pragma unroll
      for (int kq = 0; kq < KQ; ++kq) {
        const int nk = (kq + 1) % KQ;
        const int fa_off = (nk >> 1) * 128;
#pragma unroll
        for (int j = 0; j < TJ; ++j) {
          __builtin_amdgcn_s_setprio(1);
#pragma unroll
          for (int i = 0; i < TM; ++i) {
            const f32x4 c0 = kq == 0 ? (f32x4){0.f, 0.f, 0.f, 0.f} : acc[i][j];
            acc[i][j] = Elem<DT>::mfma(fb[kq & 1][j], fa[i], c0);
            if (j == TJ - 1) {
              __builtin_amdgcn_sched_barrier(0);
              fa[i] = ld16(smem + fa_b[i >> 2][nk & 1] + fa_off + (i & 3) * 16 * ROWB);
              __builtin_amdgcn_sched_barrier(0);
            }
          }
          __builtin_amdgcn_s_setprio(0);
          __builtin_amdgcn_sched_barrier(0);
          const int sn = kq + 2;
          if (sn < 10 || hi == 0) fb[kq & 1][j] = __builtin_bit_cast(u32x4, __builtin_amdgcn_raw_buffer_load_b128(rs_w, wv, whead + (unsigned)(sn * TJ + j) * 1024u, 0));
          __builtin_amdgcn_sched_barrier(0);
        }
        if (kq == KQ - 2) {
#pragma unroll
          for (int kt = 0; kt < KT; ++kt)
#pragma unroll
            for (int c = 0; c < TJ; ++c) kf[kt][c] = __builtin_bit_cast(u32x2, __builtin_amdgcn_raw_buffer_load_b64(rs_kv, kvb, (unsigned)((kt * 3 + c) * 512), 0));
          __builtin_amdgcn_sched_barrier(0);
        }
      }

      int lane_e = lane;
      asm volatile("" : "+v"(lane_e));
      const int l15e = lane_e & 15, ge = lane_e >> 4;
      u32x2 qp[TM][TJ];
      {
        f32x4 bi[TJ];
#pragma unroll
        for (int j = 0; j < TJ; ++j)
#pragma unroll
          for (int kt = 0; kt < KT; ++kt) vf[j][kt] = __builtin_bit_cast(u32x2, __builtin_amdgcn_raw_buffer_load_b64(rs_kv, kvb, (unsigned)((15 + j * 5 + kt) * 512), 0));
#pragma unroll
        for (int j = 0; j < TJ; ++j) bi[j] = __builtin_bit_cast(f32x4, __builtin_amdgcn_raw_buffer_load_b128(rs_bi, (unsigned)(head * HD + 16 * j + 4 * ge) * 4u, 0, 0));
#pragma unroll
        for (int i = 0; i < TM; ++i)
#pragma unroll
          for (int j = 0; j < TJ; ++j)
            qp[i][j] = (u32x2){pack2<DT>(acc[i][j][0] + bi[j][0], acc[i][j][1] + bi[j][1]), pack2<DT>(acc[i][j][2] + bi[j][2], acc[i][j][3] + bi[j][3])};
      }
      __builtin_amdgcn_sched_barrier(0);
#pragma unroll
      for (int i = 0; i < TM; ++i) {
        f32x4 st[KT];
#pragma unroll
// ... 153 lines not shown
    {
      f32x4 acc[TM][TJ];
#pragma unroll
      for (int kq = 0; kq < KQ; ++kq) {
        const int nk = (kq + 1) % KQ;
        const int fa_off = (nk >> 1) * 128;
#pragma unroll
        for (int j = 0; j < TJ; ++j) {
          __builtin_amdgcn_s_setprio(1);
#pragma unroll
          for (int i = 0; i < TM; ++i) {
            const f32x4 c0 = kq == 0 ? (f32x4){0.f, 0.f, 0.f, 0.f} : acc[i][j];
            acc[i][j] = Elem<DT>::mfma(fb[kq & 1][j], fa[i], c0);
            if (j == TJ - 1 && kq + 1 < KQ) {
              __builtin_amdgcn_sched_barrier(0);
              fa[i] = ld16(xb + fa_b[i >> 2][nk & 1] + fa_off + (i & 3) * 16 * ROWB);
              __builtin_amdgcn_sched_barrier(0);
            }
          }
          __builtin_amdgcn_s_setprio(0);
          __builtin_amdgcn_sched_barrier(0);
          if (kq + 2 < KQ) fb[kq & 1][j] = __builtin_bit_cast(u32x4, __builtin_amdgcn_raw_buffer_load_b128(rs_w, wv, whead + (unsigned)((kq + 2) * TJ + j) * 1024u, 0));
          __builtin_amdgcn_sched_barrier(0);
        }
        if (kq == KQ - 2) {
#pragma unroll
          for (int kt = 0; kt < KT; ++kt)
#pragma unroll
            for (int c = 0; c < TJ; ++c) kf[kt][c] = __builtin_bit_cast(u32x2, __builtin_amdgcn_raw_buffer_load_b64(rs_kv, kvb, (unsigned)((kt * 3 + c) * 512), 0));
          __builtin_amdgcn_sched_barrier(0);
        }
      }
      int lane_q = lane;
      asm volatile("" : "+v"(lane_q));
      const int gq = lane_q >> 4;
      u32x2 qp[TM][TJ];
      {
        f32x4 bi[TJ];
#pragma unroll
        for (int j = 0; j < TJ; ++j)
#pragma unroll
          for (int kt = 0; kt < KT; ++kt) vf[j][kt] = __builtin_bit_cast(u32x2, __builtin_amdgcn_raw_buffer_load_b64(rs_kv, kvb, (unsigned)((15 + j * 5 + kt) * 512), 0));
        if (IP) {
#pragma unroll
          for (int c = 0; c < TJ; ++c) kfi[c] = __builtin_bit_cast(u32x2, __builtin_amdgcn_raw_buffer_load_b64(rs_kvi, kvb, (unsigned)(c * 512), 0));
#pragma unroll
          for (int j = 0; j < TJ; ++j) vfi[j] = __builtin_bit_cast(u32x2, __builtin_amdgcn_raw_buffer_load_b64(rs_kvi, kvb, (unsigned)((15 + j * 5) * 512), 0));
        }
#pragma unroll
        for (int j = 0; j < TJ; ++j) bi[j] = __builtin_bit_cast(f32x4, __builtin_amdgcn_raw_buffer_load_b128(rs_bi, (unsigned)(head * HD + 16 * j + 4 * gq) * 4u, 0, 0));
#pragma unroll
        for (int i = 0; i < TM; ++i)
#pragma unroll
          for (int j = 0; j < TJ; ++j)
            qp[i][j] = (u32x2){pack2<DT>(acc[i][j][0] + bi[j][0], acc[i][j][1] + bi[j][1]), pack2<DT>(acc[i][j][2] + bi[j][2], acc[i][j][3] + bi[j][3])};
      }
      __builtin_amdgcn_sched_barrier(0);
      const int l15q = lane_q & 15;
      if (IP) __syncthreads();
#pragma unroll
      for (int i = 0; i < TM; ++i) {
        f32x4 st[KT];
#pragma unroll
        for (int kt = 0; kt < KT; ++kt) {
          st[kt] = Elem<DT>::mfma16(kf[kt][0], qp[i][0], (f32x4){0.f, 0.f, 0.f, 0.f});
          st[kt] = Elem<DT>::mfma16(kf[kt][1], qp[i][1], st[kt]);
          st[kt] = Elem<DT>::mfma16(kf[kt][2], qp[i][2], st[kt]);
        }
#pragma unroll
        for (int kt = 0; kt < KT; ++kt)
#pragma unroll
          for (int r = 0; r < 4; ++r)
            if (kt >= 4 && 16 * kt + 4 * gq + r >= p.nk) st[kt][r] = -INFINITY;
        float m = fmaxf(fmaxf(st[0][0], st[0][1]), fmaxf(st[0][2], st[0][3]));
#pragma unroll
        for (int kt = 1; kt < KT; ++kt) m = fmaxf(m, fmaxf(fmaxf(st[kt][0], st[kt][1]), fmaxf(st[kt][2], st[kt][3])));
        m = rowgroup_max(m);
        float l = 0.f;
        u32x2 pp[KT];
#pragma unroll
        for (int kt = 0; kt < KT; ++kt) {
          float e[4];
#pragma unroll
          for (int r = 0; r < 4; ++r) {
            e[r] = __builtin_amdgcn_exp2f(st[kt][r] - m);
            l += e[r];
          }
          pp[kt] = (u32x2){pack2_prob<DT>(e[0], e[1]), pack2_prob<DT>(e[2], e[3])};
        }
        const float inv = __builtin_amdgcn_rcpf(rowgroup_sum(l));
        u32x2 ppi;
        float invi = 0.f;
        if (IP) {
          f32x4 si = Elem<DT>::mfma16(kfi[0], qp[i][0], (f32x4){0.f, 0.f, 0.f, 0.f});
          si = Elem<DT>::mfma16(kfi[1], qp[i][1], si);
          si = Elem<DT>::mfma16(kfi[2], qp[i][2], si);
#pragma unroll
          for (int r = 0; r < 4; ++r)
            if (4 * gq + r >= p.nk_ip) si[r] = -INFINITY;
          const float mi = rowgroup_max(fmaxf(fmaxf(si[0], si[1]), fmaxf(si[2], si[3])));
          float ei[4], li = 0.f;
#pragma unroll
          for (int r = 0; r < 4; ++r) {
            ei[r] = __builtin_amdgcn_exp2f(si[r] - mi);
            li += ei[r];
          }
          ppi = (u32x2){pack2_prob<DT>(ei[0], ei[1]), pack2_prob<DT>(ei[2], ei[3])};
          invi = p.ip_scale * __builtin_amdgcn_rcpf(rowgroup_sum(li));
        }
#pragma unroll
        for (int j = 0; j < TJ; ++j) {
          f32x4 ot = Elem<DT>::mfma16(vf[j][0], pp[0], (f32x4){0.f, 0.f, 0.f, 0.f});
#pragma unroll
          for (int kt = 1; kt < KT; ++kt) ot = Elem<DT>::mfma16(vf[j][kt], pp[kt], ot);
          if (IP) {
            const f32x4 oi = Elem<DT>::mfma16(vfi[j], ppi, (f32x4){0.f, 0.f, 0.f, 0.f});
            const u32x2 ov = {pack2<DT>(fmaf(oi[0], invi, ot[0] * inv), fmaf(oi[1], invi, ot[1] * inv)), pack2<DT>(fmaf(oi[2], invi, ot[2] * inv), fmaf(oi[3], invi, ot[3] * inv))};
            const int dv = 16 * j + 4 * gq;
            if (dv < HD) {
              const int col = head * HD + dv;
              ca_lds_store8(xb + (16 * i + l15q) * ROWB + (((col >> 3) ^ ((l15q >> 1) & 7)) << 4) + (col & 7) * 2, ov);
            }
          } else {
            op[i][j] = (u32x2){pack2<DT>(ot[0] * inv, ot[1] * inv), pack2<DT>(ot[2] * inv, ot[3] * inv)};
          }
        }
      }
      __builtin_amdgcn_sched_barrier(0);
    }
    int lane_e = lane;
    asm volatile("" : "+v"(lane_e));
    const int l15e = lane_e & 15, ge = lane_e >> 4;
    const unsigned row_base = (unsigned)(m0 + (wid >> 2) * 64 + l15e);
    AttnOutRegs R;
    attn_out_prefetch<DT>(R, p.out, rs_wo, rs_res, wid, lane_e, row_base, 16u, 32u);
    if (!IP) {
      __syncthreads();
#pragma unroll
      for (int i = 0; i < TM; ++i)
#pragma unroll
        for (int j = 0; j < TJ; ++j) {
          const int dv = 16 * j + 4 * ge;
          if (dv < HD) {
            const int col = head * HD + dv;
            ca_lds_store8(xb + (16 * i + l15e) * ROWB + (((col >> 3) ^ ((l15e >> 1) & 7)) << 4) + (col & 7) * 2, op[i][j]);
          }
        }
    }
    asm volatile("s_waitcnt lgkmcnt(0)" ::: "memory");
    __syncthreads();
    attn_out_run<DT>(R, xb, fa_b, p.out, rs_wo, rs_bo, rs_o, wid, lane_e, row_base, 16u, 32u, (unsigned)p.ldo);
  }
}
```

controlanimate_amd/kernels.py:

```python
from __future__ import annotations

import ctypes as C
from typing import Optional

import torch

from . import _capi
from .context import dispatch
from ._capi import (AttnArgs, ConvArgs, ConvNarrowArgs, FfArgs, TattnArgs, XattnArgs, GemmArgs, GroupNormArgs, LayerNormArgs, CA_ACT_NONE,
                    CA_ACT_SILU, CA_BF16, CA_F16, check, lib)

ACT_NONE, ACT_SILU = CA_ACT_NONE, CA_ACT_SILU
ACT_QUICK_GELU, ACT_GELU = 2, 3


def dt_code(dtype: torch.dtype) -> int:
    if dtype == torch.bfloat16:
        return CA_BF16
    if dtype == torch.float16:
        return CA_F16
    raise TypeError(f"activations must be bf16 or fp16, got {dtype}")


def _stream() -> int:
    return torch.cuda.current_stream().cuda_stream


def _p(t: Optional[torch.Tensor]) -> Optional[int]:
    return None if t is None else t.data_ptr()


def _req_cuda(*ts):
    for t in ts:
        if t is not None and not t.is_cuda:
            raise _capi.CAHipError("HIP kernels need device tensors (no CPU fallback)")


_plan_sink = None


def _record_plan(query, args) -> None:
    if _plan_sink is not None:
        buf = C.create_string_buffer(64)
        _plan_sink.append(buf.value.decode() if query(C.byref(args), buf, 64) == 0 else "?")


def gemm(a: torch.Tensor, w: torch.Tensor, *, a2: Optional[torch.Tensor] = None,
         bias: Optional[torch.Tensor] = None, rowbias: Optional[torch.Tensor] = None,
         rows_per_group: int = 0, residual: Optional[torch.Tensor] = None, alpha: float = 1.0,
         post_scale: float = 1.0, act: int = ACT_NONE, geglu: bool = False, out_f32: bool = False,
         out: Optional[torch.Tensor] = None, ln=None, row_sums: bool = False) -> torch.Tensor:
    _req_cuda(a, w, a2, bias, rowbias, residual, out)
    assert a.dim() == 2 and a.stride(1) == 1 and w.dim() == 2 and w.is_contiguous()
    m, k1 = a.shape
    k2 = 0
    if a2 is not None:
        assert a2.dim() == 2 and a2.stride(1) == 1 and a2.shape[0] == m and a2.dtype == a.dtype
        k2 = a2.shape[1]
    n = w.shape[0]
    assert w.shape[1] == k1 + k2 and w.dtype == a.dtype
    ncols = n // 2 if geglu else n
    if out is None:
        out = torch.empty((m, ncols), device=a.device, dtype=torch.float32 if out_f32 else a.dtype)
    assert out.shape == (m, ncols) and out.stride(1) == 1
    if residual is not None:
        assert residual.shape == (m, n) and residual.stride(1) == 1 and residual.dtype == a.dtype
    if bias is not None:
        assert bias.dtype == torch.float32 and bias.numel() == n
    if rowbias is not None:
        assert rowbias.dtype == torch.float32 and rowbias.dim() == 2 and rowbias.shape[1] == n and rows_per_group > 0
    args = GemmArgs(a=_p(a), a2=_p(a2), w=_p(w), c=_p(out), bias=_p(bias), rowbias=_p(rowbias),
                    residual=_p(residual), lda=a.stride(0), lda2=a2.stride(0) if a2 is not None else 0,
                    ldc=out.stride(0), ld_res=residual.stride(0) if residual is not None else 0,
                    ld_rowbias=rowbias.stride(0) if rowbias is not None else 0,
                    m=m, n=n, k1=k1, k2=k2, rows_per_group=rows_per_group, alpha=alpha,
                    post_scale=post_scale, act=act, geglu=int(geglu), out_f32=int(out_f32),
                    dtype=dt_code(a.dtype))
    frag = getattr(w, "_frag", None)
    if frag is not None and frag[1] == bool(geglu) and dispatch.gemm_ar:
        args.w_frag = _p(frag[0])
    if ln is not None:
        st, cs = ln
        assert cs.dtype == torch.float32 and cs.numel() == n
        args.ln_colsum = _p(cs)
        if isinstance(st, RowStats):
            assert st.x.data_ptr() == a.data_ptr() and st.x.shape == a.shape, "RowStats belongs to another tensor"
            args.ln_eps = st.eps
            if lib().ca_gemm_ln_inline_supported(C.byref(args)):
                pass
            elif st.sums is not None:
                rs, parts = st.sums
                assert rs.shape == (m, parts, 2) and rs.dtype == torch.float32 and rs.is_contiguous()
                args.ln_stats, args.ln_parts = _p(rs), min(parts, 4)
                if parts > 4 or lib().ca_gemm_wants_finished_stats(C.byref(args)):
                    fin = getattr(st, "_finished", None)
                    if fin is None:
                        fin = torch.empty((m, 2), device=a.device, dtype=torch.float32)
                        check(lib().ca_ln_finish_sums(_p(rs), parts, m, k1 + k2, st.eps, _p(fin), _stream()), "ca_ln_finish_sums")
                        st._finished = fin
                    args.ln_stats, args.ln_parts = _p(fin), 0
            else:
                st = st.tensor()
        if not isinstance(st, RowStats):
            assert st.dtype == torch.float32 and st.shape == (m, 2) and st.is_contiguous()
            args.ln_stats = _p(st)
    if hasattr(out, "_row_sums"):
        del out._row_sums
    if row_sums and dispatch.ln_row_sums and not geglu and not out_f32:
        parts = int(lib().ca_gemm_row_sums_parts(C.byref(args)))
        if parts > 0:
            rs = torch.empty((m, parts, 2), device=a.device, dtype=torch.float32)
            args.row_sums_out = _p(rs)
            out._row_sums = (rs, parts)
    wbytes = 0 if args.row_sums_out else int(lib().ca_gemm_workspace_bytes(C.byref(args)))
    if wbytes > 0:
        ws = torch.empty((wbytes,), device=a.device, dtype=torch.uint8)
        args.workspace, args.workspace_bytes = _p(ws), wbytes
    _record_plan(lib().ca_gemm_plan_name, args)
    check(lib().ca_gemm(C.byref(args), _stream()), "ca_gemm")
    return out


def attach_w_frag(w: torch.Tensor, geglu: bool = False) -> torch.Tensor:
    _req_cuda(w)
    if w.dim() != 2 or w.shape[1] != 320 or w.shape[0] % 320 != 0 or not w.is_contiguous() or w.dtype not in (torch.float16, torch.bfloat16):
        return w
    dst = torch.empty_like(w)
    check(lib().ca_pack_w_frag(w.data_ptr(), w.shape[0], w.shape[1], int(bool(geglu)), dst.data_ptr(), _stream()), "ca_pack_w_frag")
    w._frag = (dst, bool(geglu))
    return w


def ff_fused(x: torch.Tensor, w1_frag: torch.Tensor, bias1: torch.Tensor, colsum1: torch.Tensor, w2_frag: torch.Tensor,
             bias2: Optional[torch.Tensor], ln_eps: float, residual: Optional[torch.Tensor] = None,
             ln_stats: Optional[torch.Tensor] = None, *, w_out_frag: Optional[torch.Tensor] = None, bias_out: Optional[torch.Tensor] = None,
             residual_out: Optional[torch.Tensor] = None) -> Optional[torch.Tensor]:
    if not dispatch.ff_fused:
        return None
    _req_cuda(x, w1_frag, bias1, colsum1, w2_frag, bias2, residual, ln_stats, w_out_frag, bias_out, residual_out)
    if x.dim() != 2 or x.stride(1) != 1 or (residual is not None and (residual.shape != x.shape or residual.stride(1) != 1 or residual.dtype != x.dtype)):
        return None
    if w_out_frag is None and (bias_out is not None or residual_out is not None):
        return None
    if residual_out is not None and (residual_out.shape != x.shape or residual_out.stride(1) != 1 or residual_out.dtype != x.dtype):
        return None
    m, c = x.shape
    inner = w2_frag.shape[1]
    y = torch.empty((m, c), device=x.device, dtype=x.dtype)
    args = FfArgs(x=_p(x), w1_frag=_p(w1_frag), bias1=_p(bias1), colsum1=_p(colsum1), ln_stats=_p(ln_stats), w2_frag=_p(w2_frag),
                  bias2=_p(bias2), residual=_p(residual), y=_p(y), lda=x.stride(0), ldc=y.stride(0),
                  ld_res=residual.stride(0) if residual is not None else 0, m=m, c=c, inner=inner, ln_eps=float(ln_eps), dtype=dt_code(x.dtype),
                  w_out_frag=_p(w_out_frag), bias_out=_p(bias_out), residual_out=_p(residual_out),
                  ld_res_out=residual_out.stride(0) if residual_out is not None else 0)
    if not lib().ca_ff_fused_supported(C.byref(args)):
        return None
    if _plan_sink is not None:
        _plan_sink.append("ff_out128" if w_out_frag is not None else "ff_fused128")
    check(lib().ca_ff_fused(C.byref(args), _stream()), "ca_ff_fused")
    return y


def tattn_fused(x: torch.Tensor, w_frag: torch.Tensor, gamma: torch.Tensor, bias_pe: torch.Tensor, b: int, frames: int, tokens: int,
                heads: int, ln_eps: float, scale: float, *, w_out_frag: Optional[torch.Tensor] = None, bias_out: Optional[torch.Tensor] = None,
                residual: Optional[torch.Tensor] = None) -> Optional[torch.Tensor]:
    if not dispatch.tattn_fused:
        return None
    _req_cuda(x, w_frag, gamma, bias_pe, w_out_frag, bias_out, residual)
    if x.dim() != 2 or x.stride(1) != 1 or x.shape[0] != b * frames * tokens or bias_pe.shape[0] < frames or bias_pe.stride(1) != 1:
        return None
    if w_out_frag is None and (bias_out is not None or residual is not None):
        return None
    if residual is not None and (residual.shape != x.shape or residual.stride(1) != 1 or residual.dtype != x.dtype):
        return None
    c = x.shape[1]
    o = torch.empty((x.shape[0], c), device=x.device, dtype=x.dtype)
    args = TattnArgs(x=_p(x), w_frag=_p(w_frag), gamma=_p(gamma), bias_pe=_p(bias_pe), o=_p(o), lda=x.stride(0), ldo=o.stride(0),
                     ld_bias_pe=bias_pe.stride(0), batch=b, frames=frames, tokens=tokens, heads=heads, c=c, ln_eps=float(ln_eps),
                     scale=float(scale), dtype=dt_code(x.dtype), w_out_frag=_p(w_out_frag), bias_out=_p(bias_out), residual=_p(residual),
                     ld_res=residual.stride(0) if residual is not None else 0)
    if not lib().ca_tattn_fused_supported(C.byref(args)):
        return None
    if _plan_sink is not None:
        _plan_sink.append("tattn_out128" if w_out_frag is not None else "tattn_fused128")
    check(lib().ca_tattn_fused(C.byref(args), _stream()), "ca_tattn_fused")
    return o


def xattn_pack_kv(kv: torch.Tensor, kv_batches: int, rows_per_batch: int, nk: int, scale: float, row_offset: int = 0,
                  out: Optional[torch.Tensor] = None) -> Optional[torch.Tensor]:
    if (not dispatch.xattn_fused or kv.dim() != 2 or kv.shape[1] != 640 or kv.stride(1) != 1 or not (64 < nk <= 80 or 1 <= nk <= 16)
            or kv.dtype not in (torch.float16, torch.bfloat16)):
        return None
    _req_cuda(kv)
    dst = out if out is not None else torch.empty((kv_batches, 8, _capi.XATTN_KV_FRAG_ELEMS), device=kv.device, dtype=kv.dtype)
    assert dst.shape == (kv_batches, 8, _capi.XATTN_KV_FRAG_ELEMS) and dst.dtype == kv.dtype and dst.is_contiguous()
    check(lib().ca_xattn_pack_kv(kv.data_ptr(), kv.stride(0), kv_batches, rows_per_batch, row_offset, nk, float(scale), dt_code(kv.dtype),
                                 dst.data_ptr(), _stream()), "ca_xattn_pack_kv")
    return dst


def xattn_fused(x: torch.Tensor, wq_frag: torch.Tensor, bias: Optional[torch.Tensor], kv_frag: torch.Tensor, images: int, tokens: int,
                frames_per_kv: int, kv_mod: int, nk: int, ln_eps: float, *, w_out_frag: Optional[torch.Tensor] = None,
                bias_out: Optional[torch.Tensor] = None, residual: Optional[torch.Tensor] = None, kv_frag_ip: Optional[torch.Tensor] = None,
                nk_ip: int = 0, ip_scale: float = 1.0) -> Optional[torch.Tensor]:
    if not dispatch.xattn_fused or kv_frag is None:
        return None
    _req_cuda(x, wq_frag, bias, kv_frag, w_out_frag, bias_out, residual, kv_frag_ip)
    if kv_frag_ip is not None and (w_out_frag is None or kv_frag_ip.shape != kv_frag.shape or kv_frag_ip.dtype != x.dtype or not kv_frag_ip.is_contiguous()):
        return None
    if x.dim() != 2 or x.stride(1) != 1 or x.shape[0] != images * tokens:
        return None
    if w_out_frag is None and (bias_out is not None or residual is not None):
        return None
    if residual is not None and (residual.shape != x.shape or residual.stride(1) != 1 or residual.dtype != x.dtype):
        return None
    assert kv_frag.dtype == x.dtype and wq_frag.dtype == x.dtype, "ca_xattn_fused: x, the packed Wq and the packed K/V must share one dtype"
    c = x.shape[1]
    o = torch.empty((x.shape[0], c), device=x.device, dtype=x.dtype)
    args = XattnArgs(x=_p(x), wq_frag=_p(wq_frag), bias=_p(bias), kv_frag=_p(kv_frag), o=_p(o), lda=x.stride(0), ldo=o.stride(0), m=x.shape[0],
                     tokens=tokens, frames_per_kv=frames_per_kv, kv_mod=kv_mod if kv_mod > 0 else images, kv_batches=kv_frag.shape[0],
                     nk=nk, heads=8, c=c, ln_eps=float(ln_eps), dtype=dt_code(x.dtype), w_out_frag=_p(w_out_frag), bias_out=_p(bias_out),
                     residual=_p(residual), ld_res=residual.stride(0) if residual is not None else 0, kv_frag_ip=_p(kv_frag_ip),
                     nk_ip=nk_ip if kv_frag_ip is not None else 0, ip_scale=float(ip_scale) if kv_frag_ip is not None else 0.0)
    if not lib().ca_xattn_fused_supported(C.byref(args)):
        return None
    if _plan_sink is not None:
        _plan_sink.append(("xattn_ip_out128" if kv_frag_ip is not None else "xattn_out128") if w_out_frag is not None else "xattn_fused128")
    check(lib().ca_xattn_fused(C.byref(args), _stream()), "ca_xattn_fused")
    return o


def row_sums_of(t: torch.Tensor):
    return getattr(t, "_row_sums", None)


def carry_row_sums(dst: torch.Tensor, src: torch.Tensor) -> torch.Tensor:
    s = getattr(src, "_row_sums", None)
    if s is not None:
        dst._row_sums = s
    return dst


class RowStats:

    def __init__(self, x: torch.Tensor, eps: float = 1e-5, sums=None):
        self.x, self.eps, self._t, self.sums = x, float(eps), None, sums

    def tensor(self) -> torch.Tensor:
        if self._t is None:
            self._t = row_stats(self.x, self.eps)
        return self._t


def conv3x3(x: torch.Tensor, w: torch.Tensor, *, x2: Optional[torch.Tensor] = None,
            bias: Optional[torch.Tensor] = None, rowbias: Optional[torch.Tensor] = None,
            rows_per_group: int = 0, residual: Optional[torch.Tensor] = None, stride: int = 1,
            upsample: bool = False, alpha: float = 1.0, post_scale: float = 1.0, act: int = ACT_NONE,
            out_f32: bool = False, pad_asym: bool = False, w_wino: Optional[torch.Tensor] = None) -> torch.Tensor:
    _req_cuda(x, w, x2, bias, rowbias, residual, w_wino)
    assert x.dim() == 4 and x.is_contiguous() and w.dim() == 4 and w.is_contiguous()
    images, hin, win, cin1 = x.shape
    cin2 = 0
    if x2 is not None:
        assert x2.is_contiguous() and x2.shape[:3] == x.shape[:3] and x2.dtype == x.dtype
        cin2 = x2.shape[3]
    cout = w.shape[0]
    assert tuple(w.shape[1:]) == (3, 3, cin1 + cin2) and w.dtype == x.dtype
    hl, wl = (hin * 2, win * 2) if upsample else (hin, win)
    pad = 1 if pad_asym else 2
    hout, wout = (hl + pad - 3) // stride + 1, (wl + pad - 3) // stride + 1
    y = torch.empty((images, hout, wout, cout), device=x.device, dtype=torch.float32 if out_f32 else x.dtype)
    ld_res = 0
    if residual is not None:
        assert residual.dtype == x.dtype and residual.is_contiguous() and residual.numel() == images * hout * wout * cout, \
            f"residual {tuple(residual.shape)} {residual.dtype} contiguous={residual.is_contiguous()} vs output {(images, hout, wout, cout)} {x.dtype}"
        ld_res = cout
    if rowbias is not None:
        assert rowbias.dtype == torch.float32 and rowbias.dim() == 2 and rowbias.shape[1] == cout and rows_per_group > 0
    if bias is not None:
        assert bias.dtype == torch.float32 and bias.numel() == cout
    args = ConvArgs(x=_p(x), x2=_p(x2), w=_p(w), y=_p(y), bias=_p(bias), rowbias=_p(rowbias),
                    residual=_p(residual), ld_res=ld_res,
                    ld_rowbias=rowbias.stride(0) if rowbias is not None else 0, images=images, hin=hin,
                    win=win, cin1=cin1, cin2=cin2, cout=cout, stride=stride, upsample=int(upsample),
                    rows_per_group=rows_per_group, alpha=alpha, post_scale=post_scale, act=act,
                    out_f32=int(out_f32), dtype=dt_code(x.dtype), pad_asym=int(pad_asym))
    if w_wino is not None and dispatch.conv_winograd:
        assert w_wino.dtype == x.dtype and w_wino.is_contiguous() and tuple(w_wino.shape) == (16, cout, cin1 + cin2)
        args.w_wino = _p(w_wino)
    wbytes = int(lib().ca_conv3x3_workspace_bytes(C.byref(args)))
    if wbytes > 0:
        ws = torch.empty((wbytes,), device=x.device, dtype=torch.uint8)
        args.workspace, args.workspace_bytes = _p(ws), wbytes
    _record_plan(lib().ca_conv3x3_plan_name, args)
    check(lib().ca_conv3x3(C.byref(args), _stream()), "ca_conv3x3")
    return y


_gn_wino_declined: dict = {}


def group_norm_conv3x3_wino(x: torch.Tensor, gamma: torch.Tensor, beta: torch.Tensor, w: torch.Tensor, w_wino: torch.Tensor, *,
                            x2: Optional[torch.Tensor] = None, groups: int = 32, eps: float = 1e-5, act: int = ACT_NONE,
                            bias: Optional[torch.Tensor] = None, rowbias: Optional[torch.Tensor] = None, rows_per_group: int = 0,
                            residual: Optional[torch.Tensor] = None, post_scale: float = 1.0) -> Optional[torch.Tensor]:
    if not (dispatch.conv_winograd and dispatch.gn_winograd):
        return None
    _req_cuda(x, gamma, beta, w, w_wino, x2, bias, rowbias, residual)
    if x.dim() != 4 or not x.is_contiguous() or x.dtype != torch.float16 or (x2 is not None and (not x2.is_contiguous() or x2.shape[:3] != x.shape[:3])):
        return None
    images, h, w_, c1 = x.shape
    c2 = 0 if x2 is None else x2.shape[3]
    c, cout = c1 + c2, w.shape[0]
    tiles = images * (h // 2) * (w_ // 2)
    key = (images, h, w_, c1, c2, cout, groups, act, rowbias is not None, residual is not None, rows_per_group)
    if _gn_wino_declined.get(key):
        return None
    cargs = ConvArgs(x=_p(x), x2=None, w=_p(w), y=_p(x), bias=_p(bias), rowbias=_p(rowbias), residual=_p(residual),
                     ld_res=cout if residual is not None else 0, ld_rowbias=rowbias.stride(0) if rowbias is not None else 0, images=images, hin=h,
                     win=w_, cin1=c, cin2=0, cout=cout, stride=1, upsample=0, rows_per_group=rows_per_group, alpha=1.0, post_scale=post_scale,
                     act=ACT_NONE, out_f32=0, dtype=dt_code(x.dtype), pad_asym=0, w_wino=_p(w_wino), x_is_wino_v=1)
    cargs.workspace, cargs.workspace_bytes = _p(x), 1 << 60
    buf = C.create_string_buffer(64)
    if lib().ca_conv3x3_plan_name(C.byref(cargs), buf, 64) != 0 or not buf.value.decode().startswith("wino"):
        _gn_wino_declined[key] = True
        return None
    wbytes = int(lib().ca_conv3x3_workspace_bytes(C.byref(cargs)))
    gargs = GroupNormArgs(x=_p(x), x2=_p(x2), y=None, gamma=_p(gamma), beta=_p(beta), partials=None, images=images, hw=h * w_, c1=c1, c2=c2,
                          groups=groups, frames_per_stat=1, eps=eps, act=act, dtype=dt_code(x.dtype), wino_v=_p(x), wino_h=h, wino_w=w_)
    if wbytes <= 0 or not lib().ca_groupnorm_wino_supported(C.byref(gargs)):
        _gn_wino_declined[key] = True
        return None
    y = torch.empty((images, h, w_, cout), device=x.device, dtype=x.dtype)
    v = torch.empty((16, tiles, c), device=x.device, dtype=x.dtype)
    if residual is not None:
        assert residual.dtype == x.dtype and residual.is_contiguous() and residual.numel() == y.numel()
    ws = torch.empty((wbytes,), device=x.device, dtype=torch.uint8)
    cargs.x, cargs.y, gargs.wino_v = _p(v), _p(y), _p(v)
    cargs.workspace, cargs.workspace_bytes = _p(ws), wbytes
    if _plan_sink is not None:
        buf = C.create_string_buffer(64)
        _plan_sink.append("gn_" + (buf.value.decode() if lib().ca_conv3x3_plan_name(C.byref(cargs), buf, 64) == 0 else "?"))
    check(lib().ca_groupnorm(C.byref(gargs), _stream()), "ca_groupnorm(wino)")
    check(lib().ca_conv3x3(C.byref(cargs), _stream()), "ca_conv3x3(wino, V given)")
    return y


def group_norm(x: torch.Tensor, gamma: torch.Tensor, beta: torch.Tensor, *, x2: Optional[torch.Tensor] = None,
               groups: int = 32, frames_per_stat: int = 1, eps: float = 1e-5, act: int = ACT_NONE) -> torch.Tensor:
    _req_cuda(x, gamma, beta, x2)
    assert x.dim() == 4 and x.is_contiguous()
    images, h, w_, c1 = x.shape
    c2 = 0
    if x2 is not None:
        assert x2.is_contiguous() and x2.shape[:3] == x.shape[:3] and x2.dtype == x.dtype
        c2 = x2.shape[3]
    c = c1 + c2
    assert gamma.dtype == torch.float32 and beta.dtype == torch.float32 and gamma.numel() == c and beta.numel() == c
    y = torch.empty((images, h, w_, c), device=x.device, dtype=x.dtype)
    nfl = lib().ca_groupnorm_partials_floats(images, h * w_, frames_per_stat, groups)
    partials = torch.empty((max(int(nfl), 1),), device=x.device, dtype=torch.float32)
    args = GroupNormArgs(x=_p(x), x2=_p(x2), y=_p(y), gamma=_p(gamma), beta=_p(beta), partials=_p(partials),
                         images=images, hw=h * w_, c1=c1, c2=c2, groups=groups,
                         frames_per_stat=frames_per_stat, eps=eps, act=act, dtype=dt_code(x.dtype))
    check(lib().ca_groupnorm(C.byref(args), _stream()), "ca_groupnorm")
    return y


def layer_norm(x: torch.Tensor, gamma: torch.Tensor, beta: torch.Tensor, *, pos: Optional[torch.Tensor] = None,
               rows_per_frame: int = 1, frames: int = 1, eps: float = 1e-5) -> torch.Tensor:
    _req_cuda(x, gamma, beta, pos)
    assert x.dim() == 2 and x.is_contiguous()
    rows, c = x.shape
    assert gamma.dtype == torch.float32 and beta.dtype == torch.float32
    if pos is not None:
        assert pos.dtype == torch.float32 and pos.is_contiguous() and pos.shape == (frames, c)
    y = torch.empty_like(x)
    args = LayerNormArgs(x=_p(x), y=_p(y), gamma=_p(gamma), beta=_p(beta), pos=_p(pos), rows=rows, c=c,
                         rows_per_frame=rows_per_frame, frames=frames, eps=eps, dtype=dt_code(x.dtype))
    check(lib().ca_layernorm(C.byref(args), _stream()), "ca_layernorm")
# ... 331 lines not shown
```

controlanimate_amd/layers.py:

```python
from __future__ import annotations

from typing import Callable, List, Optional, Sequence, Tuple

import torch
from torch import nn

from . import kernels as K
from .context import dispatch

ALIGN = 256


class Packed:

    __slots__ = ("shape", "dtype", "fill", "offset", "t", "frag")

    def __init__(self, shape, dtype, fill):
        self.shape = tuple(int(s) for s in shape)
        self.dtype = dtype
        self.fill = fill
        self.offset = -1
        self.t: Optional[torch.Tensor] = None
        self.frag = None

    @property
    def nbytes(self) -> int:
        n = 1
        for s in self.shape:
            n *= s
        return n * torch.empty((), dtype=self.dtype).element_size()


class WeightArena:
    def __init__(self):
        self.items: List[Packed] = []
        self.buffer: Optional[torch.Tensor] = None

    def add(self, shape, dtype, fill: Callable[[], torch.Tensor]) -> Packed:
        p = Packed(shape, dtype, fill)
        self.items.append(p)
        return p

    def finalize(self, device) -> torch.Tensor:
        off = 0
        for p in self.items:
            p.offset = off
            off += (p.nbytes + ALIGN - 1) // ALIGN * ALIGN
        self.buffer = torch.zeros(max(off, ALIGN), dtype=torch.uint8, device=device)
        for p in self.items:
            view = self.buffer[p.offset:p.offset + p.nbytes].view(p.dtype).view(p.shape)
            src = p.fill()
            assert tuple(src.shape) == p.shape, (tuple(src.shape), p.shape)
            view.copy_(src.to(device=device, dtype=p.dtype, non_blocking=False))
            p.t = view
            p.fill = None
        for p in self.items:
            if p.frag is not None:
                p.t._frag = (p.frag[0].t, bool(p.frag[1]))
        return self.buffer

    @property
    def nbytes(self) -> int:
        return 0 if self.buffer is None else self.buffer.numel()


def _f32(t: torch.Tensor) -> torch.Tensor:
    return t.detach().float()


def frag_order(w: torch.Tensor, geglu: bool) -> torch.Tensor:
    n, k = w.shape
    assert k == 320 and n % 64 == 0
    j = torch.arange(4).view(4, 1)
    i = torch.arange(16).view(1, 16)
    col = (16 * (i >> 2) + 4 * j + (i & 3)) if geglu else (32 * (j >> 1) + 8 * (i >> 2) + 4 * (j & 1) + (i & 3))
    rows = (torch.arange(n // 64).view(-1, 1, 1) * 64 + col.view(1, 4, 16)).to(w.device)
    x = w[rows.reshape(-1)].view(n // 64, 4, 16, 10, 4, 8)
    return x.permute(0, 3, 1, 4, 2, 5).reshape(n, k).contiguous()


def frag_order2(w: torch.Tensor) -> torch.Tensor:
    assert tuple(w.shape) == (320, 1280)
    j = torch.arange(5).view(5, 1)
    i = torch.arange(16).view(1, 16)
    col = torch.where(j == 4, 64 + i, 32 * (j >> 1) + 8 * (i >> 2) + 4 * (j & 1) + (i & 3))
    rows = (torch.arange(4).view(4, 1, 1) * 80 + col.view(1, 5, 16)).to(w.device)
    x = w[rows.reshape(-1)].view(4, 5, 16, 40, 4, 8)
    return x.permute(3, 0, 1, 4, 2, 5).reshape(320, 1280).contiguous()


def frag_order_tattn(wqkv: torch.Tensor) -> torch.Tensor:
    assert tuple(wqkv.shape) == (960, 320)
    wpad = wqkv.new_zeros(3, 8, 48, 320)
    wpad[:, :, :40] = wqkv.view(3, 8, 40, 320)
    x = wpad.view(3, 2, 4, 3, 16, 10, 4, 8)
    return x.permute(2, 1, 0, 5, 3, 6, 4, 7).reshape(-1).contiguous()


def frag_order_xattn(wq: torch.Tensor) -> torch.Tensor:
    assert tuple(wq.shape) == (320, 320)
    wpad = wq.new_zeros(8, 48, 320)
    wpad[:, :40] = wq.view(8, 40, 320)
    x = wpad.view(2, 4, 3, 16, 10, 4, 8)
    return x.permute(1, 0, 4, 2, 5, 3, 6).reshape(-1).contiguous()


def frag_order_wout(w: torch.Tensor) -> torch.Tensor:
    assert tuple(w.shape) == (320, 320)
    j = torch.arange(5).view(5, 1)
    i = torch.arange(16).view(1, 16)
    col = torch.where(j == 4, 64 + i, 32 * (j >> 1) + 8 * (i >> 2) + 4 * (j & 1) + (i & 3))
    rows = (torch.arange(4).view(4, 1, 1) * 80 + col.view(1, 5, 16)).to(w.device)
    x = w[rows.reshape(-1)].view(4, 5, 16, 10, 4, 8)
    return x.permute(0, 3, 1, 4, 2, 5).reshape(-1).contiguous()


def frag_wanted(n: int, k: int) -> bool:
    return k == 320 and n % 320 == 0 and n >= 960


class HipLinear(nn.Module):

    def __init__(self, in_features: int, out_features: int, bias: bool = True):
        super().__init__()
        self.in_features, self.out_features = in_features, out_features
        self.weight = nn.Parameter(torch.empty(out_features, in_features))
        self.bias = nn.Parameter(torch.empty(out_features)) if bias else None
        nn.init.normal_(self.weight, std=in_features ** -0.5)
        if bias:
            nn.init.zeros_(self.bias)
        self.w: Optional[Packed] = None
        self.b: Optional[Packed] = None

    def pack(self, arena: WeightArena, dtype):
        self.w = arena.add((self.out_features, self.in_features), dtype, lambda: _f32(self.weight))
        self.b = arena.add((self.out_features,), torch.float32, lambda: _f32(self.bias)) if self.bias is not None else None

    def run(self, a: torch.Tensor, **kw) -> torch.Tensor:
        return K.gemm(a, self.w.t, bias=None if self.b is None else self.b.t, **kw)


class HipConv1x1(nn.Module):

    def __init__(self, in_channels: int, out_channels: int):
        super().__init__()
        self.in_channels, self.out_channels = in_channels, out_channels
        self.weight = nn.Parameter(torch.empty(out_channels, in_channels, 1, 1))
        self.bias = nn.Parameter(torch.zeros(out_channels))
        nn.init.normal_(self.weight, std=in_channels ** -0.5)
        self.w = self.b = None

    def pack(self, arena: WeightArena, dtype):
        self.w = arena.add((self.out_channels, self.in_channels), dtype, lambda: _f32(self.weight).reshape(self.out_channels, self.in_channels))
        self.b = arena.add((self.out_channels,), torch.float32, lambda: _f32(self.bias))

    def run(self, a: torch.Tensor, **kw) -> torch.Tensor:
        return K.gemm(a, self.w.t, bias=self.b.t, **kw)


class HipConv3x3(nn.Module):

    def __init__(self, in_channels: int, out_channels: int, stride: int = 1):
        super().__init__()
        self.in_channels, self.out_channels, self.stride = in_channels, out_channels, stride
        self.cin_pad = (in_channels + 7) // 8 * 8
        self.weight = nn.Parameter(torch.empty(out_channels, in_channels, 3, 3))
        self.bias = nn.Parameter(torch.zeros(out_channels))
        nn.init.normal_(self.weight, std=(9 * in_channels) ** -0.5)
        self.w = self.b = None
        self.winograd = True

    def _packed_weight(self) -> torch.Tensor:
        w = _f32(self.weight).permute(0, 2, 3, 1)
        if self.cin_pad != self.in_channels:
            w = torch.nn.functional.pad(w, (0, self.cin_pad - self.in_channels))
        return w.contiguous()

    def _winograd_weight(self) -> torch.Tensor:
        g = torch.tensor([[1.0, 0.0, 0.0], [0.5, 0.5, 0.5], [0.5, -0.5, 0.5], [0.0, 0.0, 1.0]], dtype=torch.float32, device=self.weight.device)
        u = torch.einsum("xk,oikl,yl->xyoi", g, _f32(self.weight), g)
        return u.reshape(16, self.out_channels, self.in_channels).contiguous()

    def pack(self, arena: WeightArena, dtype):
        self.w = arena.add((self.out_channels, 3, 3, self.cin_pad), dtype, self._packed_weight)
        self.b = arena.add((self.out_channels,), torch.float32, lambda: _f32(self.bias))
        self.u = None
        if (dispatch.conv_winograd and self.stride == 1 and self.winograd and self.in_channels >= 640 and self.in_channels % 64 == 0
                and self.out_channels % 320 == 0):
            self.u = arena.add((16, self.out_channels, self.in_channels), dtype, self._winograd_weight)

    def run(self, x: torch.Tensor, **kw) -> torch.Tensor:
        u = getattr(self, "u", None)
        return K.conv3x3(x, self.w.t, bias=self.b.t, stride=self.stride, w_wino=None if u is None else u.t, **kw)


class HipGroupNorm(nn.Module):
    def __init__(self, num_groups: int, num_channels: int, eps: float = 1e-5):
        super().__init__()
        self.num_groups, self.num_channels, self.eps = num_groups, num_channels, eps
        self.weight = nn.Parameter(torch.ones(num_channels))
        self.bias = nn.Parameter(torch.zeros(num_channels))
        self.g = self.b = None

    def pack(self, arena: WeightArena, dtype):
        self.g = arena.add((self.num_channels,), torch.float32, lambda: _f32(self.weight))
        self.b = arena.add((self.num_channels,), torch.float32, lambda: _f32(self.bias))

    def run(self, x: torch.Tensor, *, x2: Optional[torch.Tensor] = None, frames_per_stat: int = 1, act: int = K.ACT_NONE):
        return K.group_norm(x, self.g.t, self.b.t, x2=x2, groups=self.num_groups, frames_per_stat=frames_per_stat,
                            eps=self.eps, act=act)


class HipLayerNorm(nn.Module):
    def __init__(self, dim: int, eps: float = 1e-5):
        super().__init__()
        self.dim, self.eps = dim, eps
        self.weight = nn.Parameter(torch.ones(dim))
        self.bias = nn.Parameter(torch.zeros(dim))
        self.g = self.b = None

    def pack(self, arena: WeightArena, dtype):
        self.g = arena.add((self.dim,), torch.float32, lambda: _f32(self.weight))
        self.b = arena.add((self.dim,), torch.float32, lambda: _f32(self.bias))

    def run(self, x: torch.Tensor, *, pos: Optional[torch.Tensor] = None, rows_per_frame: int = 1, frames: int = 1):
        return K.layer_norm(x, self.g.t, self.b.t, pos=pos, rows_per_frame=rows_per_frame, frames=frames, eps=self.eps)


def pack_concat_rows(arena: WeightArena, dtype, mods: Sequence[nn.Module]) -> Packed:
    n = sum(m.weight.shape[0] for m in mods)
    k = mods[0].weight.shape[1]
    return arena.add((n, k), dtype, lambda: torch.cat([_f32(m.weight).reshape(m.weight.shape[0], -1) for m in mods], 0))


def pack_concat_bias(arena: WeightArena, mods: Sequence[nn.Module]) -> Packed:
    n = sum(m.weight.shape[0] for m in mods)
    return arena.add((n,), torch.float32, lambda: torch.cat([_f32(m.bias) for m in mods], 0))


def ln_fold_enabled() -> bool:
    from .context import dispatch
    return bool(dispatch.ln_fold)


class LnFold:

    def __init__(self, arena: WeightArena, dtype, ln: "HipLayerNorm", mods: Sequence[nn.Module], geglu: bool = False, pe=None):
        n = sum(m.weight.shape[0] for m in mods)
        k = mods[0].weight.shape[1]
        self.eps = ln.eps

        def w_cat():
            return torch.cat([_f32(m.weight).reshape(m.weight.shape[0], -1) for m in mods], 0)

        def w_fold():
            w = w_cat() * _f32(ln.weight)[None, :]
            return geglu_interleave(w) if geglu else w

        def bias():
            b = w_cat() @ _f32(ln.bias)
            b = b + torch.cat([_f32(m.bias) if getattr(m, "bias", None) is not None else torch.zeros(m.weight.shape[0], device=m.weight.device) for m in mods], 0)
            return geglu_interleave(b) if geglu else b

        self.w = arena.add((n, k), dtype, w_fold)
        self.w_fold = w_fold
        if frag_wanted(n, k):
# ... 22 lines not shown
```

controlanimate_amd/motion_module.py:

```python
from __future__ import annotations

import math

import torch
from torch import nn

from . import kernels as K
from .attention import FeedForward
from .attention_processor import Attention
from .context import ExecCtx
from .layers import HipGroupNorm, HipLayerNorm, HipLinear, WeightArena, _f32


def get_motion_module(in_channels, motion_module_type: str, motion_module_kwargs: dict):
    if motion_module_type == "Vanilla":
        return VanillaTemporalModule(in_channels=in_channels, **motion_module_kwargs)
    raise ValueError(motion_module_type)


class PositionalEncoding(nn.Module):
    def __init__(self, d_model, dropout=0.0, max_len=24):
        super().__init__()
        position = torch.arange(max_len).unsqueeze(1)
        div_term = torch.exp(torch.arange(0, d_model, 2) * (-math.log(10000.0) / d_model))
        pe = torch.zeros(1, max_len, d_model)
        pe[0, :, 0::2] = torch.sin(position * div_term)
        pe[0, :, 1::2] = torch.cos(position * div_term)
        self.register_buffer("pe", pe)
        self.max_len = max_len
        self.table = None

    def pack(self, arena: WeightArena, dtype):
        self.table = arena.add((self.pe.shape[1], self.pe.shape[2]), torch.float32, lambda: _f32(self.pe)[0])


class VersatileAttention(Attention):
    def __init__(self, attention_mode=None, cross_frame_attention_mode=None, temporal_position_encoding=False,
                 temporal_position_encoding_max_len=24, *args, **kwargs):
        super().__init__(*args, **kwargs)
        assert attention_mode == "Temporal"
        self.attention_mode = attention_mode
        self.is_cross_attention = kwargs.get("cross_attention_dim") is not None
        if self.is_cross_attention:
            raise NotImplementedError("Temporal_Cross is not used by inference-v{1,2}.yaml")
        self.pos_encoder = PositionalEncoding(kwargs["query_dim"], max_len=temporal_position_encoding_max_len) \
            if temporal_position_encoding else None

    def pack(self, arena, dtype, fold_ln=None):
        pe = self.pos_encoder.pe if (fold_ln is not None and self.pos_encoder is not None) else None
        super().pack(arena, dtype, fold_ln=fold_ln, pe=pe)
        if self.pos_encoder is not None:
            self.pos_encoder.pack(arena, dtype)
        self.tfrag = self.tgamma = self.tbias_pe = None
        no_bias = all(getattr(m, "bias", None) is None for m in (self.to_q, self.to_k, self.to_v))
        if self.fold is not None and pe is not None and no_bias and (self.heads, self.inner_dim, self.query_dim) == (8, 320, 320):
            from .layers import _f32, frag_order_tattn
            self.tfrag = arena.add((368640,), dtype, lambda: frag_order_tattn(torch.cat([_f32(m.weight) for m in (self.to_q, self.to_k, self.to_v)], 0)))
            self.tgamma = arena.add((320,), torch.float32, lambda: _f32(fold_ln.weight))
            self.tbias_pe = arena.add((pe.shape[-2], 320), torch.float32,
                                      lambda: _f32(pe).reshape(pe.shape[-2], 320).to(fold_ln.bias.device) + _f32(fold_ln.bias)[None, :])
            self.tln_eps = fold_ln.eps

    def pos_table(self, frames: int):
        if self.pos_encoder is None:
            return None
        if frames > self.pos_encoder.max_len:
            raise ValueError(f"video_length {frames} exceeds temporal_position_encoding_max_len {self.pos_encoder.max_len}")
        return self.pos_encoder.table.t[:frames]


class TemporalTransformerBlock(nn.Module):
    def __init__(self, dim, num_attention_heads, attention_head_dim, attention_block_types=("Temporal_Self", "Temporal_Self"),
                 dropout=0.0, cross_attention_dim=768, activation_fn="geglu", attention_bias=False, upcast_attention=False,
                 cross_frame_attention_mode=None, temporal_position_encoding=False, temporal_position_encoding_max_len=24, **_):
        super().__init__()
        self.attention_blocks = nn.ModuleList([
            VersatileAttention(attention_mode=name.split("_")[0],
                               cross_attention_dim=cross_attention_dim if name.endswith("_Cross") else None,
                               query_dim=dim, heads=num_attention_heads, dim_head=attention_head_dim, bias=attention_bias,
                               temporal_position_encoding=temporal_position_encoding,
                               temporal_position_encoding_max_len=temporal_position_encoding_max_len)
            for name in attention_block_types])
        self.norms = nn.ModuleList([HipLayerNorm(dim) for _ in attention_block_types])
        self.ff = FeedForward(dim, activation_fn=activation_fn)
        self.ff_norm = HipLayerNorm(dim)

    def pack(self, arena, dtype):
        for attn, norm in zip(self.attention_blocks, self.norms):
            attn.pack(arena, dtype, fold_ln=norm)
            norm.pack(arena, dtype)
        self.ff.pack(arena, dtype, fold_ln=self.ff_norm)
        self.ff_norm.pack(arena, dtype)

    def forward(self, x: torch.Tensor, ctx: ExecCtx, tokens: int, proj_out=None) -> torch.Tensor:
        rows, C = x.shape
        nblk = len(self.attention_blocks)
        for i, (attn, norm) in enumerate(zip(self.attention_blocks, self.norms)):
            nxt = (self.attention_blocks[i + 1].fold if i + 1 < nblk else self.ff.fold) is not None
            if attn.fold is not None:
                o = attn(x.view(1, rows, C), residual=x.view(1, rows, C), temporal=(ctx.b, ctx.f, tokens),
                         ln=(K.RowStats(x, norm.eps, K.row_sums_of(x)), attn.fold), row_sums=nxt)
            else:
                n = norm.run(x, pos=attn.pos_table(ctx.f), rows_per_frame=tokens, frames=ctx.f)
                o = attn(n.view(1, rows, C), residual=x.view(1, rows, C), temporal=(ctx.b, ctx.f, tokens), row_sums=nxt)
            x = K.carry_row_sums(o.view(rows, C), o)
        if self.ff.fold is None:
            return self.ff.run(self.ff_norm.run(x), residual=x)
        if proj_out is not None and K.row_sums_of(x) is None:
            y = self.ff.run_with_proj_out(x, x, *proj_out)
            if y is not None:
                y._proj_out_done = True
                return y
        return self.ff.run(x, residual=x, sums=K.row_sums_of(x))


class TemporalTransformer3DModel(nn.Module):
    def __init__(self, in_channels, num_attention_heads, attention_head_dim, num_layers, norm_num_groups=32, **kw):
        super().__init__()
        inner = num_attention_heads * attention_head_dim
        self.norm = HipGroupNorm(norm_num_groups, in_channels, eps=1e-6)
        self.proj_in = HipLinear(in_channels, inner)
        self.transformer_blocks = nn.ModuleList([
            TemporalTransformerBlock(dim=inner, num_attention_heads=num_attention_heads,
                                     attention_head_dim=attention_head_dim, **kw) for _ in range(num_layers)])
        self.proj_out = HipLinear(inner, in_channels)

    def pack(self, arena, dtype):
        self.norm.pack(arena, dtype)
        self.proj_in.pack(arena, dtype)
        for b in self.transformer_blocks:
            b.pack(arena, dtype)
        self.proj_out.pack(arena, dtype)
        self.proj_out_frag = None
        po = self.proj_out
        if tuple(po.weight.shape) == (320, 320) and getattr(self.transformer_blocks[-1].ff, "w2f", None) is not None:
            from .layers import frag_order_wout
            self.proj_out_frag = arena.add((102400,), dtype, lambda: frag_order_wout(_f32(po.weight)))

    def forward(self, x: torch.Tensor, ctx: ExecCtx) -> torch.Tensor:
        images, h, w, c = x.shape
        rows = images * h * w
        y = self.norm.run(x)
        y = self.proj_in.run(y.view(rows, c), row_sums=self.transformer_blocks[0].attention_blocks[0].fold is not None)
        pfrag = getattr(self, "proj_out_frag", None)
        last = len(self.transformer_blocks) - 1
        for k, blk in enumerate(self.transformer_blocks):
            y = blk(y, ctx, h * w, proj_out=(pfrag, self.proj_out.b, x.view(rows, c)) if (k == last and pfrag is not None) else None)
        if getattr(y, "_proj_out_done", False):
            return y.view(images, h, w, c)
        return self.proj_out.run(y, residual=x.view(rows, c)).view(images, h, w, c)


class VanillaTemporalModule(nn.Module):
    def __init__(self, in_channels, num_attention_heads=8, num_transformer_block=2,
                 attention_block_types=("Temporal_Self", "Temporal_Self"), cross_frame_attention_mode=None,
                 temporal_position_encoding=False, temporal_position_encoding_max_len=24, temporal_attention_dim_div=1,
                 zero_initialize=True):
        super().__init__()
        self.temporal_transformer = TemporalTransformer3DModel(
            in_channels=in_channels, num_attention_heads=num_attention_heads,
            attention_head_dim=in_channels // num_attention_heads // temporal_attention_dim_div,
            num_layers=num_transformer_block, attention_block_types=attention_block_types,
            cross_frame_attention_mode=cross_frame_attention_mode, temporal_position_encoding=temporal_position_encoding,
            temporal_position_encoding_max_len=temporal_position_encoding_max_len)
        if zero_initialize:
            nn.init.zeros_(self.temporal_transformer.proj_out.weight)
            nn.init.zeros_(self.temporal_transformer.proj_out.bias)

    def pack(self, arena, dtype):
        self.temporal_transformer.pack(arena, dtype)

    def forward(self, x: torch.Tensor, ctx: ExecCtx) -> torch.Tensor:
        return self.temporal_transformer(x, ctx)
```

include/controlanimate_hip.h:

```cpp
#ifndef CONTROLANIMATE_HIP_H
#define CONTROLANIMATE_HIP_H

#include <stdint.h>

#ifdef __cplusplus
extern "C" {
#endif

#define CA_ABI_VERSION 15

#define CA_BF16 0
#define CA_F16 1

#define CA_OK 0
#define CA_ERR_INVALID_ARG (-1)
#define CA_ERR_UNSUPPORTED (-2)
#define CA_ERR_LAUNCH (-3)

#define CA_ACT_NONE 0
#define CA_ACT_SILU 1
#define CA_ACT_QUICK_GELU 2
#define CA_ACT_GELU 3

int ca_abi_version(void);
const char* ca_last_error(void);

typedef struct ca_gemm_args {
  const void* a;
  const void* a2;
  const void* w;
  void* c;
  const float* bias;
  const float* rowbias;
  const void* residual;
  int64_t lda, lda2, ldc, ld_res, ld_rowbias;
  int32_t m, n, k1, k2;
  int32_t rows_per_group;
  float alpha, post_scale;
  int32_t act;
  int32_t geglu;
  int32_t out_f32;
  int32_t dtype;
  const float* ln_stats;
  const float* ln_colsum;
  float ln_eps;
  void* workspace;
  int64_t workspace_bytes;
  float* row_sums_out;
  int32_t ln_parts;
  const void* w_frag;
} ca_gemm_args;
int ca_gemm(const ca_gemm_args* args, void* stream);
int ca_pack_w_frag(const void* w, int32_t n, int32_t k, int32_t geglu, void* dst, void* stream);
typedef struct ca_ff_args {
  const void* x;
  const void* w1_frag;
  const float* bias1;
  const float* colsum1;
  const float* ln_stats;
  const void* w2_frag;
  const float* bias2;
  const void* residual;
  void* y;
  int64_t lda, ldc, ld_res;
  int32_t m, c, inner;
  float ln_eps;
  int32_t dtype;
  const void* w_out_frag;
  const float* bias_out;
  const void* residual_out;
  int64_t ld_res_out;
} ca_ff_args;
int ca_ff_fused(const ca_ff_args* args, void* stream);
int ca_ff_fused_supported(const ca_ff_args* args);
int ca_pack_w2_frag(const void* w, int32_t n, int32_t k, void* dst, void* stream);
#define CA_TATTN_W_FRAG_ELEMS 368640
typedef struct ca_tattn_args {
  const void* x;
  const void* w_frag;
  const float* gamma;
  const float* bias_pe;
  void* o;
  int64_t lda, ldo, ld_bias_pe;
  int32_t batch, frames, tokens, heads, c;
  float ln_eps, scale;
  int32_t dtype;
  const void* w_out_frag;
  const float* bias_out;
  const void* residual;
  int64_t ld_res;
} ca_tattn_args;
int ca_tattn_fused(const ca_tattn_args* args, void* stream);
int ca_tattn_fused_supported(const ca_tattn_args* args);
#define CA_ATTN_WOUT_FRAG_ELEMS 102400
int ca_pack_w_out(const void* w, int32_t n, int32_t k, void* dst, void* stream);
int ca_pack_w_tattn(const void* w, int32_t n, int32_t k, void* dst, void* stream);
#define CA_XATTN_W_FRAG_ELEMS 122880
#define CA_XATTN_KV_FRAG_ELEMS 7680
typedef struct ca_xattn_args {
  const void* x;
  const void* wq_frag;
  const float* bias;
  const void* kv_frag;
  void* o;
  int64_t lda, ldo;
  int32_t m, tokens, frames_per_kv, kv_mod, kv_batches, nk, heads, c;
  float ln_eps;
  int32_t dtype;
  const void* w_out_frag;
  const float* bias_out;
  const void* residual;
  int64_t ld_res;
  const void* kv_frag_ip;
  int32_t nk_ip;
  float ip_scale;
} ca_xattn_args;
int ca_xattn_fused(const ca_xattn_args* args, void* stream);
int ca_xattn_fused_supported(const ca_xattn_args* args);
int ca_xattn_pack_w(const void* w, int32_t n, int32_t k, void* dst, void* stream);
int ca_xattn_pack_kv(const void* kv, int64_t ld, int32_t kv_batches, int32_t rows_per_batch, int32_t row_offset, int32_t nk, float scale, int32_t dtype,
                     void* dst, void* stream);
int64_t ca_gemm_workspace_bytes(const ca_gemm_args* args);
int ca_gemm_row_sums_parts(const ca_gemm_args* args);
int ca_gemm_ln_inline_supported(const ca_gemm_args* args);
int ca_gemm_wants_finished_stats(const ca_gemm_args* args);
int ca_ln_finish_sums(const float* sums, int parts, int64_t rows, int k, float eps, float* mean_rstd, void* stream);
int ca_gemm_plan_name(const ca_gemm_args* args, char* buf, int32_t len);

typedef struct ca_conv_args {
  const void* x;
  const void* x2;
  const void* w;
  void* y;
  const float* bias;
  const float* rowbias;
  const void* residual;
  int64_t ld_res, ld_rowbias;
  int32_t images, hin, win, cin1, cin2, cout;
  int32_t stride;
  int32_t upsample;
  int32_t rows_per_group;
  float alpha, post_scale;
  int32_t act;
  int32_t out_f32;
  int32_t dtype;
  void* workspace;
  int64_t workspace_bytes;
  int32_t pad_asym;
  const void* w_wino;
  int32_t x_is_wino_v;
} ca_conv_args;
int ca_pack_w_wino(const void* w, int32_t cout, int32_t cin, int32_t dtype, void* dst, void* stream);
int64_t ca_conv3x3_workspace_bytes(const ca_conv_args* args);
int ca_conv3x3(const ca_conv_args* args, void* stream);
int ca_conv3x3_plan_name(const ca_conv_args* args, char* buf, int32_t len);

typedef struct ca_groupnorm_args {
  const void* x;
  const void* x2;
  void* y;
  const float* gamma;
  const float* beta;
  float* partials;
  int32_t images, hw, c1, c2;
  int32_t groups;
  int32_t frames_per_stat;
  float eps;
  int32_t act;
  int32_t dtype;
  void* wino_v;
  int32_t wino_h, wino_w;
} ca_groupnorm_args;
int ca_groupnorm_wino_supported(const ca_groupnorm_args* args);
int64_t ca_groupnorm_partials_floats(int32_t images, int32_t hw, int32_t frames_per_stat, int32_t groups);
int ca_groupnorm_stats(const ca_groupnorm_args* args, void* stream);
int ca_groupnorm_apply(const ca_groupnorm_args* args, void* stream);
int ca_groupnorm(const ca_groupnorm_args* args, void* stream);

typedef struct ca_layernorm_args {
  const void* x; void* y;
  const float* gamma; const float* beta;
  const float* pos;
  int64_t rows;
  int32_t c;
  int32_t rows_per_frame, frames;
  float eps;
  int32_t dtype;
  float* stats;
} ca_layernorm_args;
int ca_layernorm(const ca_layernorm_args* args, void* stream);

typedef struct ca_attn_args {
  const void* q; const void* k; const void* v; void* o;
  int64_t q_outer, q_inner, q_row;
  int64_t o_outer, o_inner, o_row;
  int64_t k_outer, k_inner, k_row;
  int32_t inner_count, kv_inner_count, kv_div, kv_mod;
  int32_t batches, heads, head_dim;
  int32_t nq, nk;
  float scale;
  float out_scale;
  int32_t accumulate;
  int32_t dtype;
  int32_t causal;
  const uint8_t* key_mask;
  int64_t key_mask_stride;
} ca_attn_args;
int ca_attention(const ca_attn_args* args, void* stream);
int ca_attention_plan_name(const ca_attn_args* args, char* buf, int32_t len);


int ca_add_bcast(const void* a, const void* b, void* out, int64_t n, int64_t b_period,
                 int32_t dtype, void* stream);
int ca_repeat(const void* src, void* dst, int64_t bytes, int32_t times, void* stream);

int ca_softmax_rows(const float* x, void* y, int64_t rows, int32_t cols, int64_t ldx, int64_t ldy,
                    float scale, int32_t dtype, void* stream);

int ca_silu_f32(const float* x, float* y, int64_t n, void* stream);

int ca_timestep_embedding(const float* t_dev, float t_host, void* out, int32_t batch,
                          int32_t dim, int32_t dtype, void* stream);

int ca_latents_to_nhwc(const float* latents, void* out, int32_t b0, int32_t c, int32_t f,
                       int32_t h, int32_t w, int32_t cpad, int32_t rep, float in_scale,
                       int32_t dtype, void* stream);

int ca_nhwc_to_ncfhw_f32(const void* x, float* out, int32_t b, int32_t c, int32_t f, int32_t h,
                         int32_t w, int32_t ldx, int32_t x_is_f32, int32_t dtype, void* stream);

int ca_ncfhw_to_nhwc(const void* x, int32_t x_kind , const int64_t strides[5],
                     void* out, int32_t b, int32_t c, int32_t f, int32_t h, int32_t w, int32_t cpad,
                     int32_t dtype, void* stream);

int ca_cfg_scheduler_step(const float* eps, int32_t ld_eps, int32_t rep, float guidance,
                          const float* latents, const float* noise, float* prev, float* denoised,
                          int32_t c, int32_t f, int32_t h, int32_t w, const float coef[7],
                          float clip, void* stream);

int ca_lincomb(float* out, const float* const* x, const float* coef, int32_t n_terms, int64_t n, void* stream);

typedef struct ca_conv3x3_narrow_args {
  const void* x;
  const void* w;
  void* y;
  const float* bias;
  const void* r1;
  const void* r2;
  int64_t ldx, ldy, ld_r1, ld_r2;
  int32_t images, hin, win, cin, cout;
  int32_t channel_offset;
  int32_t upsample;
  int32_t leaky_relu;
  float s0, s1, s2;
  int32_t out_u8;
  int32_t dtype;
} ca_conv3x3_narrow_args;
int ca_conv3x3_narrow(const ca_conv3x3_narrow_args* args, void* stream);
int ca_conv3x3_narrow_plan_name(const ca_conv3x3_narrow_args* args, char* buf, int32_t len);

int ca_rgb8_to_nhwc(const uint8_t* src, void* dst, int32_t images, int32_t h, int32_t w, int32_t dtype, void* stream);

int ca_resize_lanczos4_u8(const uint8_t* src, uint8_t* dst, int32_t images, int32_t sh, int32_t sw, int32_t dh, int32_t dw,
                          const int32_t* xofs, const int16_t* alpha, const int32_t* yofs, const int16_t* beta, void* stream);


int64_t ca_color_match_workspace_bytes(int32_t images, int64_t pixels);

int ca_hist_u8x3(const uint8_t* src, uint32_t* hist, int32_t images, int64_t pixels, void* stream);

int ca_color_moments_f64(const uint8_t* src, const double* lut, const double* mean, double* moments, int32_t images,
                         int64_t pixels, void* workspace, int64_t workspace_bytes, void* stream);

int ca_color_transform_f64(const uint8_t* src, const double* lut, const double* mean, const double* t, const double* my,
// ... 17 lines not shown
```

Before: 16.05.

## Extend fused temporal and cross attention kernels to C=640 blocks

Adds 640-channel (head_dim 80) variants of the fused temporal-attention and cross-attention kernels, including their output projection. It also adds weight and KV fragment packers and routing in the Python layer, so the 640-wide transformer blocks use the fused path instead of separate GEMM, attention and projection launches. Cross attention at C=640 is only routed above a row-count threshold. The cost is new kernel code paths and larger packed weight buffers, and the new kernels may use registers and LDS differently at the wider head dimension.

```diff
diff --git a/controlanimate_amd/_capi.py b/controlanimate_amd/_capi.py
--- a/controlanimate_amd/_capi.py
+++ b/controlanimate_amd/_capi.py
@@ -8,7 +8,7 @@
 
 CA_BF16, CA_F16 = 0, 1
 CA_ACT_NONE, CA_ACT_SILU = 0, 1
-ABI_VERSION = 15
+ABI_VERSION = 16
 
 
 class CAHipUnavailable(RuntimeError):
@@ -74,6 +74,10 @@
 
 XATTN_W_FRAG_ELEMS = 122880
 XATTN_KV_FRAG_ELEMS = 7680
+TATTN_W_FRAG_ELEMS_C640 = 1228800
+ATTN_WOUT_FRAG_ELEMS_C640 = 409600
+XATTN_W_FRAG_ELEMS_C640 = 409600
+XATTN_KV_FRAG_ELEMS_C640 = 12800
 
 
 class ConvArgs(C.Structure):
@@ -154,6 +158,7 @@
     "ca_xattn_fused_supported": (C.c_int, [C.POINTER(XattnArgs)]),
     "ca_xattn_pack_w": (C.c_int, [C.c_void_p, C.c_int32, C.c_int32, C.c_void_p, C.c_void_p]),
     "ca_xattn_pack_kv": (C.c_int, [C.c_void_p, C.c_int64, C.c_int32, C.c_int32, C.c_int32, C.c_int32, C.c_float, C.c_int32, C.c_void_p, C.c_void_p]),
+    "ca_xattn_pack_kv_hd": (C.c_int, [C.c_void_p, C.c_int64, C.c_int32, C.c_int32, C.c_int32, C.c_int32, C.c_int32, C.c_float, C.c_int32, C.c_void_p, C.c_void_p]),
     "ca_gemm_ln_inline_supported": (C.c_int, [C.POINTER(GemmArgs)]),
     "ca_gemm_wants_finished_stats": (C.c_int, [C.POINTER(GemmArgs)]),
     "ca_ln_finish_sums": (C.c_int, [C.c_void_p, C.c_int, C.c_int64, C.c_int, C.c_float, C.c_void_p, C.c_void_p]),
diff --git a/controlanimate_amd/attention_processor.py b/controlanimate_amd/attention_processor.py
--- a/controlanimate_amd/attention_processor.py
+++ b/controlanimate_amd/attention_processor.py
@@ -56,10 +56,11 @@
             kv = cache.get(("kv", id(attn)))
             if kv is None:
                 kv = cache[("kv", id(attn))] = K.gemm(ctx.reshape(nb * L, cd), attn.kv.t)
+            routed = C != 640 or B * N >= dispatch.xattn_c640_min_rows
             ent = cache.get(("kvf", id(attn)))
-            if ent is None:
+            if ent is None and routed:
                 ent = cache[("kvf", id(attn))] = (K.xattn_pack_kv(kv, nb, L, nk, attn.scale), nk, L)
-            if ent[0] is not None and ent[1] == nk:
+            if routed and ent[0] is not None and ent[1] == nk:
                 ofrag = getattr(attn, "ofrag", None)
                 if ofrag is not None and dispatch.attn_out_fused:
                     to_out = attn.to_out[0]
@@ -206,10 +207,10 @@
             if self.is_cross:
                 self.kv = pack_concat_rows(arena, dtype, [self.to_k, self.to_v])
                 self.xfrag = None
-                if (self.heads, self.inner_dim, self.query_dim) == (8, 320, 320):
+                if (self.heads, self.inner_dim, self.query_dim) in ((8, 320, 320), (8, 640, 640)):
                     from .layers import frag_order_xattn
                     fold = self.fold
-                    self.xfrag = arena.add((122880,), dtype, lambda: frag_order_xattn(fold.w_fold().to(dtype).float()))
+                    self.xfrag = arena.add((122880 if self.query_dim == 320 else 409600,), dtype, lambda: frag_order_xattn(fold.w_fold().to(dtype).float()))
         elif self.is_cross:
             self.to_q.pack(arena, dtype)
             self.kv = pack_concat_rows(arena, dtype, [self.to_k, self.to_v])
@@ -217,10 +218,10 @@
             self.qkv = pack_concat_rows(arena, dtype, [self.to_q, self.to_k, self.to_v])
         self.to_out[0].pack(arena, dtype)
         self.ofrag = None
-        if (self.heads, self.inner_dim, self.query_dim) == (8, 320, 320) and self.fold is not None:
+        if (self.heads, self.inner_dim, self.query_dim) in ((8, 320, 320), (8, 640, 640)) and self.fold is not None:
             from .layers import _f32, frag_order_wout
             to_out = self.to_out[0]
-            self.ofrag = arena.add((102400,), dtype, lambda: frag_order_wout(_f32(to_out.weight)))
+            self.ofrag = arena.add((self.query_dim * self.query_dim,), dtype, lambda: frag_order_wout(_f32(to_out.weight)))
         if hasattr(self.processor, "pack"):
             self.processor.pack(arena, dtype)
 
diff --git a/controlanimate_amd/context.py b/controlanimate_amd/context.py
--- a/controlanimate_amd/context.py
+++ b/controlanimate_amd/context.py
@@ -32,6 +32,9 @@
     ff_fused = True
     tattn_fused = True
     xattn_fused = True
+    tattn_fused_c640 = True
+    xattn_fused_c640 = True
+    xattn_c640_min_rows = 32768
     attn_out_fused = True
     xattn_ip_fused = True
     conv_winograd = True
diff --git a/controlanimate_amd/csrc/ca_attn_out.h b/controlanimate_amd/csrc/ca_attn_out.h
--- a/controlanimate_amd/csrc/ca_attn_out.h
+++ b/controlanimate_amd/csrc/ca_attn_out.h
@@ -2,17 +2,18 @@
 
 constexpr int CA_WOUT_ELEMS = 320 * 320;
 
-__global__ __launch_bounds__(256) void k_pack_w_out(const u16* __restrict__ w, u16* __restrict__ dst) {
+__global__ __launch_bounds__(256) void k_pack_w_out(const u16* __restrict__ w, u16* __restrict__ dst, int c) {
   const int idx = blockIdx.x * 256 + threadIdx.x;
-  if (idx >= CA_WOUT_ELEMS / 8) return;
+  if (idx >= c * c / 8) return;
+  const int nkq = c / 32;
   const int L = idx & 63;
   int t = idx >> 6;
   const int j = t % 5;
   t /= 5;
-  const int kq = t % 10;
-  const int cg = t / 10;
+  const int kq = t % nkq;
+  const int cg = t / nkq;
   const int row = cg * 80 + ca_wout_col(j, L & 15);
-  st16(dst + (int64_t)idx * 8, ld16(w + (int64_t)row * 320 + kq * 32 + (L >> 4) * 8));
+  st16(dst + (int64_t)idx * 8, ld16(w + (int64_t)row * c + kq * 32 + (L >> 4) * 8));
 }
 
 __device__ __forceinline__ void ca_lds_store8(unsigned char* p, u32x2 v) {
@@ -36,12 +37,12 @@
 
 __device__ __forceinline__ unsigned attn_out_row(unsigned row_base, unsigned step_a, unsigned step_b, int i) { return row_base + (unsigned)(i & 1) * step_a + (unsigned)(i >> 1) * step_b; }
 
-template <int DT>
+template <int DT, int C = 320>
 __device__ __forceinline__ void attn_out_prefetch(AttnOutRegs& R, const AttnOutParams& a, __amdgpu_buffer_rsrc_t rs_wo, __amdgpu_buffer_rsrc_t rs_res, int wid,
                                                   int lane, unsigned row_base, unsigned step_a, unsigned step_b) {
-  const int cg = wid & 3, g = lane >> 4;
+  const int cg = wid % (C / 80), g = lane >> 4;
   const unsigned wv = (unsigned)lane * 16u;
-  const unsigned wbase = (unsigned)cg * (10u * 5u * 1024u);
+  const unsigned wbase = (unsigned)cg * ((unsigned)(C / 32) * 5u * 1024u);
 #pragma unroll
   for (int c = 0; c < 2; ++c)
 #pragma unroll
@@ -65,16 +66,16 @@
   return pack2<DT>(Elem<DT>::to_f((u16)(w & 0xffffu)) + Elem<DT>::to_f((u16)(r_ & 0xffffu)), Elem<DT>::to_f((u16)(w >> 16)) + Elem<DT>::to_f((u16)(r_ >> 16)));
 }
 
-template <int DT>
+template <int DT, int C = 320>
 __device__ __forceinline__ void attn_out_run(AttnOutRegs& R, const unsigned char* tile, const int (&fa_b)[2][2], const AttnOutParams& a,
                                              __amdgpu_buffer_rsrc_t rs_wo, __amdgpu_buffer_rsrc_t rs_bo, __amdgpu_buffer_rsrc_t rs_y, int wid, int lane,
                                              unsigned row_base, unsigned step_a, unsigned step_b, unsigned ldo) {
-  constexpr int KQ = 10, ROWB = 640;
-  const int rh = wid >> 2, cg = wid & 3;
+  constexpr int KQ = C / 32, ROWB = C * 2;
+  const int rh = wid / (C / 80), cg = wid % (C / 80);
   int lane_k = lane;
   asm volatile("" : "+v"(lane_k));
   const unsigned wv = (unsigned)lane_k * 16u;
-  const unsigned wbase = (unsigned)cg * (10u * 5u * 1024u);
+  const unsigned wbase = (unsigned)cg * ((unsigned)KQ * 5u * 1024u);
   f32x4 acc[4][5];
   u32x4 fa[4];
 #pragma unroll
diff --git a/controlanimate_amd/csrc/ca_gemm_ar.hip b/controlanimate_amd/csrc/ca_gemm_ar.hip
--- a/controlanimate_amd/csrc/ca_gemm_ar.hip
+++ b/controlanimate_amd/csrc/ca_gemm_ar.hip
@@ -63,10 +63,10 @@
   return CA_OK;
 }
 
-static int attn_out_args_ok(const void* w_out_frag, const float* bias_out, const void* residual, int64_t ld_res, int64_t rows) {
+static int attn_out_args_ok(const void* w_out_frag, const float* bias_out, const void* residual, int64_t ld_res, int64_t rows, int c = 320) {
   if (!w_out_frag) return (bias_out || residual) ? 0 : 1;
   if ((((uintptr_t)w_out_frag | (uintptr_t)bias_out | (uintptr_t)residual) & 15) != 0) return 0;
-  if (residual && (ld_res % 8 || ld_res < 320 || ((rows - 1) * ld_res + 320) * 2 >= 0x7FFFFF00ll)) return 0;
+  if (residual && (ld_res % 8 || ld_res < c || ((rows - 1) * ld_res + c) * 2 >= 0x7FFFFF00ll)) return 0;
   return 1;
 }
 
@@ -129,47 +129,52 @@
 
 extern "C" int ca_pack_w_tattn(const void* w, int32_t n, int32_t k, void* dst, void* stream) {
   CA_REQUIRE(w && dst, "ca_pack_w_tattn: null operand");
-  CA_REQUIRE(n == 960 && k == 320, "ca_pack_w_tattn: n=%d k=%d (Wq | Wk | Wv rows: 960 x 320)", n, k);
+  CA_REQUIRE((n == 960 && k == 320) || (n == 1920 && k == 640), "ca_pack_w_tattn: n=%d k=%d (Wq | Wk | Wv rows: 960 x 320 or 1920 x 640)", n, k);
   CA_REQUIRE((((uintptr_t)w | (uintptr_t)dst) & 15) == 0, "ca_pack_w_tattn: operands must be 16-byte aligned");
   static_assert(CA_TATTN_WF_ELEMS == CA_TATTN_W_FRAG_ELEMS, "header constant");
-  hipLaunchKernelGGL(k_pack_w_tattn, dim3((CA_TATTN_WF_ELEMS / 8 + 255) / 256), dim3(256), 0, (hipStream_t)stream, (const u16*)w, (u16*)dst);
+  static_assert(CA_TATTN640_WF_ELEMS == CA_TATTN_W_FRAG_ELEMS_C640, "header constant");
+  if (k == 640) hipLaunchKernelGGL(k_pack_w_tattn640, dim3((CA_TATTN640_WF_ELEMS / 8 + 255) / 256), dim3(256), 0, (hipStream_t)stream, (const u16*)w, (u16*)dst);
+  else hipLaunchKernelGGL(k_pack_w_tattn, dim3((CA_TATTN_WF_ELEMS / 8 + 255) / 256), dim3(256), 0, (hipStream_t)stream, (const u16*)w, (u16*)dst);
   CA_CHECK_LAUNCH("ca_pack_w_tattn");
   return CA_OK;
 }
 
 extern "C" int ca_pack_w_out(const void* w, int32_t n, int32_t k, void* dst, void* stream) {
   CA_REQUIRE(w && dst, "ca_pack_w_out: null operand");
-  CA_REQUIRE(n == 320 && k == 320, "ca_pack_w_out: n=%d k=%d (to_out[0].weight: 320 x 320)", n, k);
+  CA_REQUIRE((n == 320 && k == 320) || (n == 640 && k == 640), "ca_pack_w_out: n=%d k=%d (to_out[0].weight: 320 x 320 or 640 x 640)", n, k);
   CA_REQUIRE((((uintptr_t)w | (uintptr_t)dst) & 15) == 0, "ca_pack_w_out: operands must be 16-byte aligned");
   static_assert(CA_WOUT_ELEMS == CA_ATTN_WOUT_FRAG_ELEMS, "header constant");
-  hipLaunchKernelGGL(k_pack_w_out, dim3((CA_WOUT_ELEMS / 8 + 255) / 256), dim3(256), 0, (hipStream_t)stream, (const u16*)w, (u16*)dst);
+  static_assert(640 * 640 == CA_ATTN_WOUT_FRAG_ELEMS_C640, "header constant");
+  hipLaunchKernelGGL(k_pack_w_out, dim3((unsigned)((n * k / 8 + 255) / 256)), dim3(256), 0, (hipStream_t)stream, (const u16*)w, (u16*)dst, (int)k);
   CA_CHECK_LAUNCH("ca_pack_w_out");
   return CA_OK;
 }
 
 extern "C" int ca_tattn_fused_supported(const ca_tattn_args* a) {
   if (!a || !a->x || !a->w_frag || !a->gamma || !a->bias_pe || !a->o) return 0;
-  if (a->c != 320 || a->heads != 8 || a->batch < 1) return 0;
+  if ((a->c != 320 && a->c != 640) || a->heads != 8 || a->batch < 1) return 0;
+  const int c = a->c;
   if (a->frames != 16 && !((a->frames == 8 || a->frames == 32) && a->w_out_frag)) return 0;
+  if (c == 640 && (a->frames != 16 || !a->w_out_frag)) return 0;
   {
-    const int px = 128 / a->frames;
+    const int px = (c == 640 ? 64 : 128) / a->frames;
     if (a->tokens < px || a->tokens % px) return 0;
   }
   if (a->dtype != CA_BF16 && a->dtype != CA_F16) return 0;
   const int64_t rows = (int64_t)a->batch * a->frames * a->tokens;
   if (rows < 16384) return 0;
-  if (a->lda % 8 || a->ldo % 8 || a->lda < 320 || a->ldo < 320 || a->ld_bias_pe % 4 || a->ld_bias_pe < 320) return 0;
+  if (a->lda % 8 || a->ldo % 8 || a->lda < c || a->ldo < c || a->ld_bias_pe % 4 || a->ld_bias_pe < c) return 0;
   if ((((uintptr_t)a->x | (uintptr_t)a->o | (uintptr_t)a->w_frag | (uintptr_t)a->gamma | (uintptr_t)a->bias_pe) & 15) != 0) return 0;
   const int64_t lim = 0x7FFFFF00ll;
-  if (((rows - 1) * a->lda + 320) * 2 >= lim || ((rows - 1) * a->ldo + 320) * 2 >= lim) return 0;
+  if (((rows - 1) * a->lda + c) * 2 >= lim || ((rows - 1) * a->ldo + c) * 2 >= lim) return 0;
   if (!(a->ln_eps > 0.f) || !(a->scale > 0.f)) return 0;
-  if (!attn_out_args_ok(a->w_out_frag, a->bias_out, a->residual, a->ld_res, rows)) return 0;
+  if (!attn_out_args_ok(a->w_out_frag, a->bias_out, a->residual, a->ld_res, rows, c)) return 0;
   return 1;
 }
 
 extern "C" int ca_tattn_fused(const ca_tattn_args* a, void* stream) {
   CA_REQUIRE(a != nullptr, "ca_tattn_fused: null args");
-  CA_REQUIRE(ca_tattn_fused_supported(a), "ca_tattn_fused: arguments outside what the fused temporal attention takes (C = 320, 8 heads, 16 frames -- or 8 / 32 with w_out_frag --, tokens %% (128 / frames) == 0, "
+  CA_REQUIRE(ca_tattn_fused_supported(a), "ca_tattn_fused: arguments outside what the fused temporal attention takes (C = 320, 8 heads, 16 frames -- or 8 / 32 with w_out_frag --, tokens %% (128 / frames) == 0; C = 640: 16 frames with w_out_frag; "
                                            ">= 16384 rows, fragment-ordered weights, 16-byte aligned operands, 32-bit byte offsets): ask ca_tattn_fused_supported() first");
   const int64_t rows = (int64_t)a->batch * a->frames * a->tokens;
   TattnParams p{};
@@ -182,9 +187,9 @@
   p.hw = a->tokens;
   p.ln_eps = a->ln_eps;
   p.scale_log2 = a->scale * 1.4426950408889634f;
-  p.x_bytes = (unsigned)(((rows - 1) * a->lda + 320) * 2);
-  p.o_bytes = (unsigned)(((rows - 1) * a->ldo + 320) * 2);
-  const int tiles = (int)((int64_t)a->batch * a->tokens / (128 / a->frames));
+  p.x_bytes = (unsigned)(((rows - 1) * a->lda + a->c) * 2);
+  p.o_bytes = (unsigned)(((rows - 1) * a->ldo + a->c) * 2);
+  const int tiles = (int)((int64_t)a->batch * a->tokens / ((a->c == 640 ? 64 : 128) / a->frames));
   static const int dbg = CA_KNOB("CA_TATTN_DBG", 0);
   p.dbg = dbg;
   if (a->w_out_frag) {
@@ -192,8 +197,14 @@
     p.out.bias = a->bias_out;
     p.out.res = (const u16*)a->residual;
     p.out.ld_res = (int)a->ld_res;
-    p.out.res_bytes = a->residual ? (unsigned)(((rows - 1) * a->ld_res + 320) * 2) : 0u;
+    p.out.res_bytes = a->residual ? (unsigned)(((rows - 1) * a->ld_res + a->c) * 2) : 0u;
     const unsigned grid1 = (unsigned)(tiles < ar_cu_count() ? tiles : ar_cu_count());
+    if (a->c == 640) {
+      if (a->dtype == CA_BF16) hipLaunchKernelGGL((k_tattn_out640<CA_BF16>), dim3(grid1), dim3(512), 0, (hipStream_t)stream, p, tiles);
+      else hipLaunchKernelGGL((k_tattn_out640<CA_F16>), dim3(grid1), dim3(512), 0, (hipStream_t)stream, p, tiles);
+      CA_CHECK_LAUNCH("ca_tattn_fused(out, c640)");
+      return CA_OK;
+    }
 #define CA_TATTN_OUT(FR)                                                                                                              \
   if (a->dtype == CA_BF16) hipLaunchKernelGGL((k_tattn_out<CA_BF16, FR>), dim3(grid1), dim3(512), 0, (hipStream_t)stream, p, tiles); \
   else hipLaunchKernelGGL((k_tattn_out<CA_F16, FR>), dim3(grid1), dim3(512), 0, (hipStream_t)stream, p, tiles);
@@ -214,10 +225,12 @@
 
 extern "C" int ca_xattn_pack_w(const void* w, int32_t n, int32_t k, void* dst, void* stream) {
   CA_REQUIRE(w && dst, "ca_xattn_pack_w: null operand");
-  CA_REQUIRE(n == 320 && k == 320, "ca_xattn_pack_w: n=%d k=%d (Wq: 320 x 320)", n, k);
+  CA_REQUIRE((n == 320 && k == 320) || (n == 640 && k == 640), "ca_xattn_pack_w: n=%d k=%d (Wq: 320 x 320 or 640 x 640)", n, k);
   CA_REQUIRE((((uintptr_t)w | (uintptr_t)dst) & 15) == 0, "ca_xattn_pack_w: operands must be 16-byte aligned");
   static_assert(CA_XATTN_WF_ELEMS == CA_XATTN_W_FRAG_ELEMS && CA_XATTN_KVF_ELEMS == CA_XATTN_KV_FRAG_ELEMS, "header constants");
-  hipLaunchKernelGGL(k_xattn_pack_w, dim3((CA_XATTN_WF_ELEMS / 8 + 255) / 256), dim3(256), 0, (hipStream_t)stream, (const u16*)w, (u16*)dst);
+  static_assert(CA_XATTN640_WF_ELEMS == CA_XATTN_W_FRAG_ELEMS_C640 && CA_XATTN640_KVF_ELEMS == CA_XATTN_KV_FRAG_ELEMS_C640, "header constants");
+  if (k == 640) hipLaunchKernelGGL(k_xattn_pack_w640, dim3((CA_XATTN640_WF_ELEMS / 8 + 255) / 256), dim3(256), 0, (hipStream_t)stream, (const u16*)w, (u16*)dst);
+  else hipLaunchKernelGGL(k_xattn_pack_w, dim3((CA_XATTN_WF_ELEMS / 8 + 255) / 256), dim3(256), 0, (hipStream_t)stream, (const u16*)w, (u16*)dst);
   CA_CHECK_LAUNCH("ca_xattn_pack_w");
   return CA_OK;
 }
@@ -237,9 +250,28 @@
   return CA_OK;
 }
 
+extern "C" int ca_xattn_pack_kv_hd(const void* kv, int64_t ld, int32_t head_dim, int32_t kv_batches, int32_t rows_per_batch, int32_t row_offset, int32_t nk, float scale,
+                                   int32_t dtype, void* dst, void* stream) {
+  if (head_dim == 40) return ca_xattn_pack_kv(kv, ld, kv_batches, rows_per_batch, row_offset, nk, scale, dtype, dst, stream);
+  CA_REQUIRE(kv && dst, "ca_xattn_pack_kv_hd: null operand");
+  CA_REQUIRE(head_dim == 80, "ca_xattn_pack_kv_hd: head_dim=%d (40 or 80)", head_dim);
+  CA_REQUIRE(kv_batches > 0 && rows_per_batch > 0 && row_offset >= 0 && nk > 64 && nk <= 80 && row_offset + nk <= rows_per_batch && ld >= 1280,
+             "ca_xattn_pack_kv_hd: kv_batches=%d rows_per_batch=%d row_offset=%d nk=%d (65..80 text keys) ld=%lld (>= 1280: K | V of 8 heads x 80)", kv_batches, rows_per_batch,
+             row_offset, nk, (long long)ld);
+  CA_REQUIRE(dtype == CA_BF16 || dtype == CA_F16, "ca_xattn_pack_kv_hd: dtype %d", dtype);
+  CA_REQUIRE(((uintptr_t)dst & 15) == 0 && scale > 0.f, "ca_xattn_pack_kv_hd: dst must be 16-byte aligned, scale > 0");
+  const float sl2 = scale * 1.4426950408889634f;
+  if (dtype == CA_BF16) hipLaunchKernelGGL((k_xattn_pack_kv<CA_BF16, 80>), dim3((unsigned)kv_batches * 8), dim3(64), 0, (hipStream_t)stream, (const u16*)kv, ld, rows_per_batch, row_offset, nk, sl2, (u16*)dst);
+  else hipLaunchKernelGGL((k_xattn_pack_kv<CA_F16, 80>), dim3((unsigned)kv_batches * 8), dim3(64), 0, (hipStream_t)stream, (const u16*)kv, ld, rows_per_batch, row_offset, nk, sl2, (u16*)dst);
+  CA_CHECK_LAUNCH("ca_xattn_pack_kv_hd");
+  return CA_OK;
+}
+
 extern "C" int ca_xattn_fused_supported(const ca_xattn_args* a) {
   if (!a || !a->x || !a->wq_frag || !a->kv_frag || !a->o) return 0;
-  if (a->c != 320 || a->heads != 8 || a->m < 16384 || a->tokens < 128 || a->tokens % 128 || a->m % a->tokens) return 0;
+  if ((a->c != 320 && a->c != 640) || a->heads != 8 || a->m < 16384 || a->tokens < 128 || a->tokens % 128 || a->m % a->tokens) return 0;
+  const int c = a->c;
+  if (c == 640 && (!a->w_out_frag || a->kv_frag_ip)) return 0;
   if (a->nk <= 64 || a->nk > 80 || a->frames_per_kv < 1 || a->kv_mod < 1) return 0;
   {
     const int images = a->m / a->tokens;
@@ -248,12 +280,12 @@
     if (a->kv_batches < needed) return 0;
   }
   if (a->dtype != CA_BF16 && a->dtype != CA_F16) return 0;
-  if (a->lda % 8 || a->ldo % 8 || a->lda < 320 || a->ldo < 320) return 0;
+  if (a->lda % 8 || a->ldo % 8 || a->lda < c || a->ldo < c) return 0;
   if ((((uintptr_t)a->x | (uintptr_t)a->o | (uintptr_t)a->wq_frag | (uintptr_t)a->kv_frag | (uintptr_t)a->bias) & 15) != 0) return 0;
   const int64_t lim = 0x7FFFFF00ll;
-  if (((int64_t)(a->m - 1) * a->lda + 320) * 2 >= lim || ((int64_t)(a->m - 1) * a->ldo + 320) * 2 >= lim) return 0;
+  if (((int64_t)(a->m - 1) * a->lda + c) * 2 >= lim || ((int64_t)(a->m - 1) * a->ldo + c) * 2 >= lim) return 0;
   if (!(a->ln_eps > 0.f)) return 0;
-  if (!attn_out_args_ok(a->w_out_frag, a->bias_out, a->residual, a->ld_res, a->m)) return 0;
+  if (!attn_out_args_ok(a->w_out_frag, a->bias_out, a->residual, a->ld_res, a->m, c)) return 0;
   if (a->kv_frag_ip) {
     if (!a->w_out_frag || a->nk_ip < 1 || a->nk_ip > 16 || ((uintptr_t)a->kv_frag_ip & 15) != 0 || !(a->ip_scale == a->ip_scale) || a->ip_scale - a->ip_scale != 0.f) return 0;
   } else if (a->nk_ip != 0) {
@@ -264,7 +296,7 @@
 
 extern "C" int ca_xattn_fused(const ca_xattn_args* a, void* stream) {
   CA_REQUIRE(a != nullptr, "ca_xattn_fused: null args");
-  CA_REQUIRE(ca_xattn_fused_supported(a), "ca_xattn_fused: arguments outside what the fused text cross-attention takes (C = 320, 8 heads, 65..80 keys, tokens %% 128 == 0, "
+  CA_REQUIRE(ca_xattn_fused_supported(a), "ca_xattn_fused: arguments outside what the fused text cross-attention takes (C = 320, or 640 with w_out_frag; 8 heads, 65..80 keys, tokens %% 128 == 0, "
                                            ">= 16384 rows, packed weights and K / V, 16-byte aligned operands, 32-bit byte offsets): ask ca_xattn_fused_supported() first");
   XattnParams p{};
   p.x = (const u16*)a->x;
@@ -275,17 +307,23 @@
   p.lda = (int)a->lda, p.ldo = (int)a->ldo;
   p.m = a->m, p.tokens = a->tokens, p.frames_per_kv = a->frames_per_kv, p.kv_mod = a->kv_mod, p.nk = a->nk;
   p.ln_eps = a->ln_eps;
-  p.x_bytes = (unsigned)(((int64_t)(a->m - 1) * a->lda + 320) * 2);
-  p.o_bytes = (unsigned)(((int64_t)(a->m - 1) * a->ldo + 320) * 2);
-  p.kvf_bytes = (unsigned)((int64_t)a->kv_batches * 8 * CA_XATTN_KVF_ELEMS * 2);
-  const int tiles = a->m / 128;
+  p.x_bytes = (unsigned)(((int64_t)(a->m - 1) * a->lda + a->c) * 2);
+  p.o_bytes = (unsigned)(((int64_t)(a->m - 1) * a->ldo + a->c) * 2);
+  p.kvf_bytes = (unsigned)((int64_t)a->kv_batches * 8 * (a->c == 640 ? CA_XATTN640_KVF_ELEMS : CA_XATTN_KVF_ELEMS) * 2);
+  const int tiles = a->m / (a->c == 640 ? 64 : 128);
   if (a->w_out_frag) {
     p.out.wof = (const u16*)a->w_out_frag;
     p.out.bias = a->bias_out;
     p.out.res = (const u16*)a->residual;
     p.out.ld_res = (int)a->ld_res;
-    p.out.res_bytes = a->residual ? (unsigned)(((int64_t)(a->m - 1) * a->ld_res + 320) * 2) : 0u;
+    p.out.res_bytes = a->residual ? (unsigned)(((int64_t)(a->m - 1) * a->ld_res + a->c) * 2) : 0u;
     const unsigned grid1 = (unsigned)(tiles < ar_cu_count() ? tiles : ar_cu_count());
+    if (a->c == 640) {
+      if (a->dtype == CA_BF16) hipLaunchKernelGGL((k_xattn_out640<CA_BF16>), dim3(grid1), dim3(512), 0, (hipStream_t)stream, p, tiles);
+      else hipLaunchKernelGGL((k_xattn_out640<CA_F16>), dim3(grid1), dim3(512), 0, (hipStream_t)stream, p, tiles);
+      CA_CHECK_LAUNCH("ca_xattn_fused(out, c640)");
+      return CA_OK;
+    }
     if (a->kv_frag_ip) {
       p.kvf_ip = (const u16*)a->kv_frag_ip, p.nk_ip = a->nk_ip, p.ip_scale = a->ip_scale;
       if (a->dtype == CA_BF16) hipLaunchKernelGGL((k_xattn_out<CA_BF16, true>), dim3(grid1), dim3(512), 0, (hipStream_t)stream, p, tiles);
diff --git a/controlanimate_amd/csrc/ca_tattn_fused.h b/controlanimate_amd/csrc/ca_tattn_fused.h
--- a/controlanimate_amd/csrc/ca_tattn_fused.h
+++ b/controlanimate_amd/csrc/ca_tattn_fused.h
@@ -522,3 +522,225 @@
     attn_out_run<DT>(R, xb, fa_b, p.out, rs_wo, rs_bo, rs_o, wid, lane_e, row_base, step_a, step_b, (unsigned)p.ldo);
   }
 }
+
+
+constexpr int CA_TATTN640_WF_ELEMS = 1920 * 640;
+
+__global__ __launch_bounds__(256) void k_pack_w_tattn640(const u16* __restrict__ w, u16* __restrict__ dst) {
+  const int idx = blockIdx.x * 256 + threadIdx.x;
+  if (idx >= CA_TATTN640_WF_ELEMS / 8) return;
+  const int L = idx & 63;
+  int t = idx >> 6;
+  const int j = t % 5;
+  t /= 5;
+  const int kq = t % 20;
+  t /= 20;
+  const int ps = t % 3;
+  const int head = t / 3;
+  st16(dst + (int64_t)idx * 8, ld16(w + (int64_t)(ps * 640 + head * 80 + 16 * j + (L & 15)) * 640 + kq * 32 + (L >> 4) * 8));
+}
+
+template <int DT>
+__global__ __launch_bounds__(512, 2) void k_tattn_out640(TattnParams p, int tiles) {
+  constexpr int K = 640, KQ = 20, TM = 4, TJ = 5, BM = 64, HD = 80, CPR = 80, PXT = 4;
+  constexpr int ROWB = K * 2, TILEB = BM * ROWB;
+  constexpr unsigned CHUNKB = TJ * 1024u;
+  __shared__ __attribute__((aligned(16))) unsigned char smem[2 * TILEB];
+  static_assert(2 * TILEB <= 160 * 1024, "two tile buffers");
+
+  const int tid = threadIdx.x;
+  const int lane = tid & 63;
+  const int wid = __builtin_amdgcn_readfirstlane(tid >> 6);
+  const int g = lane >> 4, l15 = lane & 15;
+
+  const __amdgpu_buffer_rsrc_t rs_x = __builtin_amdgcn_make_buffer_rsrc((void*)p.x, 0, p.x_bytes, 0x00020000);
+  const __amdgpu_buffer_rsrc_t rs_w = __builtin_amdgcn_make_buffer_rsrc((void*)p.wf, 0, (unsigned)CA_TATTN640_WF_ELEMS * 2u, 0x00020000);
+  const __amdgpu_buffer_rsrc_t rs_o = __builtin_amdgcn_make_buffer_rsrc((void*)p.o, 0, p.o_bytes, 0x00020000);
+  const __amdgpu_buffer_rsrc_t rs_wo = __builtin_amdgcn_make_buffer_rsrc((void*)p.out.wof, 0, (unsigned)(K * K) * 2u, 0x00020000);
+  const __amdgpu_buffer_rsrc_t rs_bo = __builtin_amdgcn_make_buffer_rsrc((void*)(p.out.bias ? (const void*)p.out.bias : (const void*)p.wf), 0, p.out.bias ? (unsigned)K * 4u : 0u, 0x00020000);
+  const __amdgpu_buffer_rsrc_t rs_res = __builtin_amdgcn_make_buffer_rsrc((void*)(p.out.res ? (const void*)p.out.res : (const void*)p.wf), 0, p.out.res ? p.out.res_bytes : 0u, 0x00020000);
+
+  const int f_sw = (l15 >> 1) & 7;
+  const int fa_lane = l15 * ROWB + (((f_sw >> 2) << 2) + (g ^ (f_sw & 3))) * 16;
+  int fa_b[2][2] = {{fa_lane, fa_lane ^ 64}, {fa_lane, fa_lane ^ 64}};
+  asm volatile("" : "+v"(fa_b[0][0]), "+v"(fa_b[0][1]), "+v"(fa_b[1][0]), "+v"(fa_b[1][1]));
+
+  auto issue_tile = [&](int tile, int bufsel) __attribute__((always_inline)) {
+    if (wid >= 4) return;
+    const int g0 = tile * PXT;
+    const int bimg = g0 / p.hw, pix0 = g0 - bimg * p.hw;
+    int lane_o = lane;
+    asm volatile("" : "+v"(lane_o));
+#pragma unroll
+    for (int q = 0; q < 20; ++q) {
+      const unsigned idx = (unsigned)((wid * 20 + q) * 64 + lane_o);
+      const unsigned r = idx / (unsigned)CPR;
+      const unsigned cp = idx - r * (unsigned)CPR;
+      const unsigned c = cp ^ ((r >> 1) & 7u);
+      const unsigned grow = (unsigned)((bimg * 16 + (int)(r & 15u)) * p.hw + pix0) + (r >> 4);
+      __builtin_amdgcn_raw_ptr_buffer_load_lds(rs_x, (__attribute__((address_space(3))) void*)(smem + bufsel * TILEB + (wid * 20 + q) * 1024), 16,
+                                               grow * (unsigned)p.lda * 2u + c * 16u, 0, 0, 0);
+    }
+  };
+
+  if ((int)blockIdx.x < tiles) issue_tile(blockIdx.x, 0);
+  int it = 0;
+  for (int tile = blockIdx.x; tile < tiles; tile += gridDim.x, ++it) {
+    const int cur = it & 1;
+    unsigned char* const xb = smem + cur * TILEB;
+    const int g0 = tile * PXT;
+    const int bimg = g0 / p.hw, pix0 = g0 - bimg * p.hw;
+    asm volatile("s_waitcnt vmcnt(0)" ::: "memory");
+    __syncthreads();
+    {
+      const int r = tid >> 3, h = tid & 7;
+      const int fs = (r >> 1) & 7;
+      unsigned char* src = xb + r * ROWB + h * 160;
+      const float* bprow = p.bp + (int64_t)(r & 15) * p.ld_bp;
+      float s = 0.f, ss = 0.f;
+#pragma unroll 5
+      for (int q = 0; q < 10; ++q) {
+        const u32x4 v = ld16(src + q * 16);
+#pragma unroll
+        for (int e = 0; e < 4; ++e) {
+          const float a0 = Elem<DT>::to_f((u16)(v[e] & 0xffffu)), a1 = Elem<DT>::to_f((u16)(v[e] >> 16));
+          s += a0 + a1;
+          ss = fmaf(a0, a0, fmaf(a1, a1, ss));
+        }
+      }
+      s += __shfl_xor(s, 1);
+      ss += __shfl_xor(ss, 1);
+      s += __shfl_xor(s, 2);
+      ss += __shfl_xor(ss, 2);
+      s += __shfl_xor(s, 4);
+      ss += __shfl_xor(ss, 4);
+      const float mean = s * (1.f / K);
+      const float rstd = rsqrtf(fmaxf(ss * (1.f / K) - mean * mean, 0.f) + p.ln_eps);
+      const float nb = -mean * rstd;
+#pragma unroll 5
+      for (int q = 0; q < 10; ++q) {
+        u32x4 v = ld16(src + q * 16);
+        const int col = (((h * 10 + q) ^ fs)) * 8;
+        const float4 g0v = *reinterpret_cast<const float4*>(p.gamma + col), g1v = *reinterpret_cast<const float4*>(p.gamma + col + 4);
+        const float4 b0v = *reinterpret_cast<const float4*>(bprow + col), b1v = *reinterpret_cast<const float4*>(bprow + col + 4);
+        const float gm[8] = {g0v.x, g0v.y, g0v.z, g0v.w, g1v.x, g1v.y, g1v.z, g1v.w};
+        const float bb[8] = {b0v.x, b0v.y, b0v.z, b0v.w, b1v.x, b1v.y, b1v.z, b1v.w};
+#pragma unroll
+        for (int e = 0; e < 4; ++e) {
+          const float a0 = Elem<DT>::to_f((u16)(v[e] & 0xffffu)), a1 = Elem<DT>::to_f((u16)(v[e] >> 16));
+          v[e] = pack2<DT>(fmaf(fmaf(a0, rstd, nb), gm[2 * e], bb[2 * e]), fmaf(fmaf(a1, rstd, nb), gm[2 * e + 1], bb[2 * e + 1]));
+        }
+        st16(src + q * 16, v);
+      }
+    }
+    asm volatile("s_waitcnt vmcnt(0)" ::: "memory");
+    __syncthreads();
+
+    int lane_k = lane;
+    asm volatile("" : "+v"(lane_k));
+    const unsigned wv = (unsigned)lane_k * 16u;
+    const unsigned whead = (unsigned)wid * (3u * KQ * CHUNKB);
+    u32x4 fa[TM], fb[2][TJ];
+#pragma unroll
+    for (int c = 0; c < 2; ++c)
+#pragma unroll
+      for (int j = 0; j < TJ; ++j) fb[c][j] = __builtin_bit_cast(u32x4, __builtin_amdgcn_raw_buffer_load_b128(rs_w, wv, whead + (unsigned)(c * TJ + j) * 1024u, 0));
+    {
+      const int next = tile + (int)gridDim.x;
+      if (next < tiles) issue_tile(next, cur ^ 1);
+    }
+#pragma unroll
+    for (int i = 0; i < TM; ++i) fa[i] = ld16(xb + fa_b[0][0] + i * 16 * ROWB);
+    __builtin_amdgcn_sched_barrier(0);
+
+    auto kloop = [&](auto pass_c, f32x4(&acc)[TM][TJ]) __attribute__((always_inline)) {
+      constexpr int PS = decltype(pass_c)::value;
+#pragma unroll
+      for (int kq = 0; kq < KQ; ++kq) {
+        const int nk = (kq + 1) % KQ;
+        const int fa_off = (nk >> 1) * 128;
+#pragma unroll
+        for (int j = 0; j < TJ; ++j) {
+          __builtin_amdgcn_s_setprio(1);
+#pragma unroll
+          for (int i = 0; i < TM; ++i) {
+            const f32x4 c0 = kq == 0 ? (f32x4){0.f, 0.f, 0.f, 0.f} : acc[i][j];
+            if (PS == 2) acc[i][j] = Elem<DT>::mfma(fa[i], fb[kq & 1][j], c0);
+            else acc[i][j] = Elem<DT>::mfma(fb[kq & 1][j], fa[i], c0);
+            if (j == TJ - 1) {
+              __builtin_amdgcn_sched_barrier(0);
+              fa[i] = ld16(xb + fa_b[0][nk & 1] + fa_off + i * 16 * ROWB);
+              __builtin_amdgcn_sched_barrier(0);
+            }
+          }
+          __builtin_amdgcn_s_setprio(0);
+          __builtin_amdgcn_sched_barrier(0);
+          const int sn = PS * KQ + kq + 2;
+          if (sn < 3 * KQ) fb[kq & 1][j] = __builtin_bit_cast(u32x4, __builtin_amdgcn_raw_buffer_load_b128(rs_w, wv, whead + (unsigned)(sn * TJ + j) * 1024u, 0));
+          __builtin_amdgcn_sched_barrier(0);
+        }
+      }
+    };
+
+    u32x2 qp[TM][TJ];
+    {
+      f32x4 acc[TM][TJ];
+      kloop(IntC<0>{}, acc);
+#pragma unroll
+      for (int i = 0; i < TM; ++i)
+#pragma unroll
+        for (int j = 0; j < TJ; ++j)
+          qp[i][j] = (u32x2){pack2<DT>(acc[i][j][0] * p.scale_log2, acc[i][j][1] * p.scale_log2), pack2<DT>(acc[i][j][2] * p.scale_log2, acc[i][j][3] * p.scale_log2)};
+    }
+    u32x2 pp[TM];
+    {
+      f32x4 acc[TM][TJ];
+      kloop(IntC<1>{}, acc);
+#pragma unroll
+      for (int i = 0; i < TM; ++i) {
+        f32x4 st = {0.f, 0.f, 0.f, 0.f};
+#pragma unroll
+        for (int j = 0; j < TJ; ++j) {
+          const u32x2 kp = {pack2<DT>(acc[i][j][0], acc[i][j][1]), pack2<DT>(acc[i][j][2], acc[i][j][3])};
+          st = Elem<DT>::mfma16(kp, qp[i][j], st);
+        }
+        const float m = rowgroup_max(fmaxf(fmaxf(st[0], st[1]), fmaxf(st[2], st[3])));
+        float e[4];
+#pragma unroll
+        for (int r = 0; r < 4; ++r) e[r] = __builtin_amdgcn_exp2f(st[r] - m);
+        const float inv = __builtin_amdgcn_rcpf(rowgroup_sum((e[0] + e[1]) + (e[2] + e[3])));
+        pp[i] = (u32x2){pack2<DT>(e[0] * inv, e[1] * inv), pack2<DT>(e[2] * inv, e[3] * inv)};
+      }
+    }
+    u32x2 op[TM][TJ];
+    {
+      f32x4 acc[TM][TJ];
+      kloop(IntC<2>{}, acc);
+#pragma unroll
+      for (int i = 0; i < TM; ++i)
+#pragma unroll
+        for (int j = 0; j < TJ; ++j) {
+          const u32x2 vp = {pack2<DT>(acc[i][j][0], acc[i][j][1]), pack2<DT>(acc[i][j][2], acc[i][j][3])};
+          const f32x4 ot = Elem<DT>::mfma16(vp, pp[i], (f32x4){0.f, 0.f, 0.f, 0.f});
+          op[i][j] = (u32x2){pack2<DT>(ot[0], ot[1]), pack2<DT>(ot[2], ot[3])};
+        }
+    }
+    int lane_e = lane;
+    asm volatile("" : "+v"(lane_e));
+    const int l15e = lane_e & 15, ge = lane_e >> 4;
+    const unsigned row_base = (unsigned)((bimg * 16 + l15e) * p.hw + pix0);
+    AttnOutRegs R;
+    attn_out_prefetch<DT, K>(R, p.out, rs_wo, rs_res, wid, lane_e, row_base, 1u, 2u);
+    __syncthreads();
+#pragma unroll
+    for (int i = 0; i < TM; ++i)
+#pragma unroll
+      for (int j = 0; j < TJ; ++j) {
+        const int col = wid * HD + 16 * j + 4 * ge;
+        ca_lds_store8(xb + (16 * i + l15e) * ROWB + (((col >> 3) ^ ((l15e >> 1) & 7)) << 4) + (col & 7) * 2, op[i][j]);
+      }
+    asm volatile("s_waitcnt lgkmcnt(0)" ::: "memory");
+    __syncthreads();
+    attn_out_run<DT, K>(R, xb, fa_b, p.out, rs_wo, rs_bo, rs_o, wid, lane_e, row_base, 1u, 2u, (unsigned)p.ldo);
+  }
+}
diff --git a/controlanimate_amd/csrc/ca_xattn_fused.h b/controlanimate_amd/csrc/ca_xattn_fused.h
--- a/controlanimate_amd/csrc/ca_xattn_fused.h
+++ b/controlanimate_amd/csrc/ca_xattn_fused.h
@@ -32,31 +32,32 @@
   st16(dst + (int64_t)idx * 8, dd < 40 ? ld16(w + (int64_t)((wv + 4 * hi) * 40 + dd) * 320 + kq * 32 + (L >> 4) * 8) : zero4);
 }
 
-template <int DT>
+template <int DT, int HD = 40>
 __global__ __launch_bounds__(64) void k_xattn_pack_kv(const u16* __restrict__ kv, int64_t ld, int rows_per_batch, int row_offset, int nk, float scale_log2,
                                                       u16* __restrict__ dst) {
+  constexpr int NC = (HD + 15) / 16;
   const int head = blockIdx.x & 7, zk = blockIdx.x >> 3;
   const int L = threadIdx.x, g = L >> 4, l15 = L & 15;
-  const u16* kp = kv + ((int64_t)zk * rows_per_batch + row_offset) * ld + head * 40;
-  const u16* vp = kp + 320;
-  u16* out = dst + ((int64_t)blockIdx.x * 30 * 64 + L) * 4;
+  const u16* kp = kv + ((int64_t)zk * rows_per_batch + row_offset) * ld + head * HD;
+  const u16* vp = kp + 8 * HD;
+  u16* out = dst + ((int64_t)blockIdx.x * (10 * NC) * 64 + L) * 4;
 #pragma unroll 1
-  for (int f = 0; f < 15; ++f) {
-    const int kt = f / 3, c = f - kt * 3;
+  for (int f = 0; f < 5 * NC; ++f) {
+    const int kt = f / NC, c = f - kt * NC;
     const int key = 16 * kt + l15, d0 = 16 * c + 4 * g;
     float v[4];
 #pragma unroll
-    for (int r = 0; r < 4; ++r) v[r] = (key < nk && d0 + r < 40) ? Elem<DT>::to_f(kp[(int64_t)key * ld + d0 + r]) * scale_log2 : 0.f;
+    for (int r = 0; r < 4; ++r) v[r] = (key < nk && d0 + r < HD) ? Elem<DT>::to_f(kp[(int64_t)key * ld + d0 + r]) * scale_log2 : 0.f;
     *reinterpret_cast<u32x2*>(out + (int64_t)f * 64 * 4) = (u32x2){pack2<DT>(v[0], v[1]), pack2<DT>(v[2], v[3])};
   }
 #pragma unroll 1
-  for (int f = 0; f < 15; ++f) {
+  for (int f = 0; f < 5 * NC; ++f) {
     const int j = f / 5, kt = f - j * 5;
     const int dv = 16 * j + l15, k0 = 16 * kt + 4 * g;
     u16 v[4];
 #pragma unroll
-    for (int r = 0; r < 4; ++r) v[r] = (k0 + r < nk && dv < 40) ? vp[(int64_t)(k0 + r) * ld + dv] : (u16)0;
-    *reinterpret_cast<u32x2*>(out + (int64_t)(15 + f) * 64 * 4) = (u32x2){(unsigned)v[0] | ((unsigned)v[1] << 16), (unsigned)v[2] | ((unsigned)v[3] << 16)};
+    for (int r = 0; r < 4; ++r) v[r] = (k0 + r < nk && dv < HD) ? vp[(int64_t)(k0 + r) * ld + dv] : (u16)0;
+    *reinterpret_cast<u32x2*>(out + (int64_t)(5 * NC + f) * 64 * 4) = (u32x2){(unsigned)v[0] | ((unsigned)v[1] << 16), (unsigned)v[2] | ((unsigned)v[3] << 16)};
   }
 }
 
@@ -516,3 +517,238 @@
     attn_out_run<DT>(R, xb, fa_b, p.out, rs_wo, rs_bo, rs_o, wid, lane_e, row_base, 16u, 32u, (unsigned)p.ldo);
   }
 }
+
+
+constexpr int CA_XATTN640_WF_ELEMS = 640 * 640;
+constexpr int CA_XATTN640_KVF_ELEMS = 50 * 64 * 4;
+
+__global__ __launch_bounds__(256) void k_xattn_pack_w640(const u16* __restrict__ w, u16* __restrict__ dst) {
+  const int idx = blockIdx.x * 256 + threadIdx.x;
+  if (idx >= CA_XATTN640_WF_ELEMS / 8) return;
+  const int L = idx & 63;
+  int t = idx >> 6;
+  const int j = t % 5;
+  t /= 5;
+  const int kq = t % 20;
+  const int head = t / 20;
+  st16(dst + (int64_t)idx * 8, ld16(w + (int64_t)(head * 80 + 16 * j + (L & 15)) * 640 + kq * 32 + (L >> 4) * 8));
+}
+
+template <int DT>
+__global__ __launch_bounds__(512, 2) void k_xattn_out640(XattnParams p, int tiles) {
+  constexpr int K = 640, KQ = 20, TM = 4, TJ = 5, BM = 64, HD = 80, KT = 5, CPR = 80;
+  constexpr int ROWB = K * 2, TILEB = BM * ROWB;
+  constexpr unsigned CHUNKB = TJ * 1024u;
+  __shared__ __attribute__((aligned(16))) unsigned char smem[2 * TILEB];
+  static_assert(2 * TILEB <= 160 * 1024, "two tile buffers");
+
+  const int tid = threadIdx.x;
+  const int lane = tid & 63;
+  const int wid = __builtin_amdgcn_readfirstlane(tid >> 6);
+  const int g = lane >> 4, l15 = lane & 15;
+
+  const __amdgpu_buffer_rsrc_t rs_x = __builtin_amdgcn_make_buffer_rsrc((void*)p.x, 0, p.x_bytes, 0x00020000);
+  const __amdgpu_buffer_rsrc_t rs_w = __builtin_amdgcn_make_buffer_rsrc((void*)p.wf, 0, (unsigned)CA_XATTN640_WF_ELEMS * 2u, 0x00020000);
+  const __amdgpu_buffer_rsrc_t rs_o = __builtin_amdgcn_make_buffer_rsrc((void*)p.o, 0, p.o_bytes, 0x00020000);
+  const __amdgpu_buffer_rsrc_t rs_kv = __builtin_amdgcn_make_buffer_rsrc((void*)p.kvf, 0, p.kvf_bytes, 0x00020000);
+  const __amdgpu_buffer_rsrc_t rs_bi = __builtin_amdgcn_make_buffer_rsrc((void*)(p.bias ? (const void*)p.bias : (const void*)p.wf), 0, p.bias ? (unsigned)K * 4u : 0u, 0x00020000);
+  const __amdgpu_buffer_rsrc_t rs_wo = __builtin_amdgcn_make_buffer_rsrc((void*)p.out.wof, 0, (unsigned)(K * K) * 2u, 0x00020000);
+  const __amdgpu_buffer_rsrc_t rs_bo = __builtin_amdgcn_make_buffer_rsrc((void*)(p.out.bias ? (const void*)p.out.bias : (const void*)p.wf), 0, p.out.bias ? (unsigned)K * 4u : 0u, 0x00020000);
+  const __amdgpu_buffer_rsrc_t rs_res = __builtin_amdgcn_make_buffer_rsrc((void*)(p.out.res ? (const void*)p.out.res : (const void*)p.wf), 0, p.out.res ? p.out.res_bytes : 0u, 0x00020000);
+
+  const int f_sw = (l15 >> 1) & 7;
+  const int fa_lane = l15 * ROWB + (((f_sw >> 2) << 2) + (g ^ (f_sw & 3))) * 16;
+  int fa_b[2][2] = {{fa_lane, fa_lane ^ 64}, {fa_lane, fa_lane ^ 64}};
+  asm volatile("" : "+v"(fa_b[0][0]), "+v"(fa_b[0][1]), "+v"(fa_b[1][0]), "+v"(fa_b[1][1]));
+
+  auto issue_tile = [&](int tile, int bufsel) __attribute__((always_inline)) {
+    if (wid >= 4) return;
+    const int m0 = tile * BM;
+    int lane_o = lane;
+    asm volatile("" : "+v"(lane_o));
+#pragma unroll
+    for (int q = 0; q < 20; ++q) {
+      const unsigned idx = (unsigned)((wid * 20 + q) * 64 + lane_o);
+      const unsigned r = idx / (unsigned)CPR;
+      const unsigned cp = idx - r * (unsigned)CPR;
+      const unsigned c = cp ^ ((r >> 1) & 7u);
+      __builtin_amdgcn_raw_ptr_buffer_load_lds(rs_x, (__attribute__((address_space(3))) void*)(smem + bufsel * TILEB + (wid * 20 + q) * 1024), 16,
+                                               (unsigned)(m0 + (int)r) * (unsigned)p.lda * 2u + c * 16u, 0, 0, 0);
+    }
+  };
+
+  if ((int)blockIdx.x < tiles) issue_tile(blockIdx.x, 0);
+  int it = 0;
+  for (int tile = blockIdx.x; tile < tiles; tile += gridDim.x, ++it) {
+    const int cur = it & 1;
+    unsigned char* const xb = smem + cur * TILEB;
+    const int m0 = tile * BM;
+    const int zk = ((m0 / p.tokens) / p.frames_per_kv) % p.kv_mod;
+    asm volatile("s_waitcnt vmcnt(0)" ::: "memory");
+    __syncthreads();
+    {
+      const int r = tid >> 3, h = tid & 7;
+      unsigned char* src = xb + r * ROWB + h * 160;
+      float s = 0.f, ss = 0.f;
+#pragma unroll 5
+      for (int q = 0; q < 10; ++q) {
+        const u32x4 v = ld16(src + q * 16);
+#pragma unroll
+        for (int e = 0; e < 4; ++e) {
+          const float a0 = Elem<DT>::to_f((u16)(v[e] & 0xffffu)), a1 = Elem<DT>::to_f((u16)(v[e] >> 16));
+          s += a0 + a1;
+          ss = fmaf(a0, a0, fmaf(a1, a1, ss));
+        }
+      }
+      s += __shfl_xor(s, 1);
+      ss += __shfl_xor(ss, 1);
+      s += __shfl_xor(s, 2);
+      ss += __shfl_xor(ss, 2);
+      s += __shfl_xor(s, 4);
+      ss += __shfl_xor(ss, 4);
+      const float mean = s * (1.f / K);
+      const float rstd = rsqrtf(fmaxf(ss * (1.f / K) - mean * mean, 0.f) + p.ln_eps);
+      const float nb = -mean * rstd;
+#pragma unroll 5
+      for (int q = 0; q < 10; ++q) {
+        u32x4 v = ld16(src + q * 16);
+#pragma unroll
+        for (int e = 0; e < 4; ++e) {
+          const float a0 = Elem<DT>::to_f((u16)(v[e] & 0xffffu)), a1 = Elem<DT>::to_f((u16)(v[e] >> 16));
+          v[e] = pack2<DT>(fmaf(a0, rstd, nb), fmaf(a1, rstd, nb));
+        }
+        st16(src + q * 16, v);
+      }
+    }
+    __syncthreads();
+
+    int lane_k = lane;
+    asm volatile("" : "+v"(lane_k));
+    const unsigned wv = (unsigned)lane_k * 16u;
+    const int head = wid;
+    const unsigned whead = (unsigned)wid * ((unsigned)KQ * CHUNKB);
+    const unsigned kvb = (unsigned)(zk * 8 + head) * (unsigned)(CA_XATTN640_KVF_ELEMS * 2) + (unsigned)lane_k * 8u;
+    u32x4 fa[TM], fb[2][TJ];
+#pragma unroll
+    for (int c = 0; c < 2; ++c)
+#pragma unroll
+      for (int j = 0; j < TJ; ++j) fb[c][j] = __builtin_bit_cast(u32x4, __builtin_amdgcn_raw_buffer_load_b128(rs_w, wv, whead + (unsigned)(c * TJ + j) * 1024u, 0));
+    {
+      const int next = tile + (int)gridDim.x;
+      if (next < tiles) issue_tile(next, cur ^ 1);
+    }
+#pragma unroll
+    for (int i = 0; i < TM; ++i) fa[i] = ld16(xb + fa_b[0][0] + i * 16 * ROWB);
+    __builtin_amdgcn_sched_barrier(0);
+
+    u32x2 kf[KT][TJ], vf[TJ][KT];
+    u32x2 op[TM][TJ];
+    {
+      f32x4 acc[TM][TJ];
+#pragma unroll
+      for (int kq = 0; kq < KQ; ++kq) {
+        const int nk = (kq + 1) % KQ;
+        const int fa_off = (nk >> 1) * 128;
+#pragma unroll
+        for (int j = 0; j < TJ; ++j) {
+          __builtin_amdgcn_s_setprio(1);
+#pragma unroll
+          for (int i = 0; i < TM; ++i) {
+            const f32x4 c0 = kq == 0 ? (f32x4){0.f, 0.f, 0.f, 0.f} : acc[i][j];
+            acc[i][j] = Elem<DT>::mfma(fb[kq & 1][j], fa[i], c0);
+            if (j == TJ - 1 && kq + 1 < KQ) {
+              __builtin_amdgcn_sched_barrier(0);
+              fa[i] = ld16(xb + fa_b[0][nk & 1] + fa_off + i * 16 * ROWB);
+              __builtin_amdgcn_sched_barrier(0);
+            }
+          }
+          __builtin_amdgcn_s_setprio(0);
+          __builtin_amdgcn_sched_barrier(0);
+          if (kq + 2 < KQ) fb[kq & 1][j] = __builtin_bit_cast(u32x4, __builtin_amdgcn_raw_buffer_load_b128(rs_w, wv, whead + (unsigned)((kq + 2) * TJ + j) * 1024u, 0));
+          __builtin_amdgcn_sched_barrier(0);
+        }
+        if (kq == KQ - 2) {
+#pragma unroll
+          for (int kt = 0; kt < KT; ++kt)
+#pragma unroll
+            for (int c = 0; c < TJ; ++c) kf[kt][c] = __builtin_bit_cast(u32x2, __builtin_amdgcn_raw_buffer_load_b64(rs_kv, kvb, (unsigned)((kt * TJ + c) * 512), 0));
+          __builtin_amdgcn_sched_barrier(0);
+        }
+      }
+      int lane_q = lane;
+      asm volatile("" : "+v"(lane_q));
+      const int gq = lane_q >> 4;
+      u32x2 qp[TM][TJ];
+      {
+        f32x4 bi[TJ];
+#pragma unroll
+        for (int j = 0; j < TJ; ++j)
+#pragma unroll
+          for (int kt = 0; kt < KT; ++kt) vf[j][kt] = __builtin_bit_cast(u32x2, __builtin_amdgcn_raw_buffer_load_b64(rs_kv, kvb, (unsigned)((KT * TJ + j * 5 + kt) * 512), 0));
+#pragma unroll
+        for (int j = 0; j < TJ; ++j) bi[j] = __builtin_bit_cast(f32x4, __builtin_amdgcn_raw_buffer_load_b128(rs_bi, (unsigned)(head * HD + 16 * j + 4 * gq) * 4u, 0, 0));
+#pragma unroll
+        for (int i = 0; i < TM; ++i)
+#pragma unroll
+          for (int j = 0; j < TJ; ++j)
+            qp[i][j] = (u32x2){pack2<DT>(acc[i][j][0] + bi[j][0], acc[i][j][1] + bi[j][1]), pack2<DT>(acc[i][j][2] + bi[j][2], acc[i][j][3] + bi[j][3])};
+      }
+      __builtin_amdgcn_sched_barrier(0);
+#pragma unroll
+      for (int i = 0; i < TM; ++i) {
+        f32x4 st[KT];
+#pragma unroll
+        for (int kt = 0; kt < KT; ++kt) {
+          st[kt] = Elem<DT>::mfma16(kf[kt][0], qp[i][0], (f32x4){0.f, 0.f, 0.f, 0.f});
+#pragma unroll
+          for (int c = 1; c < TJ; ++c) st[kt] = Elem<DT>::mfma16(kf[kt][c], qp[i][c], st[kt]);
+        }
+#pragma unroll
+        for (int r = 0; r < 4; ++r)
+          if (64 + 4 * gq + r >= p.nk) st[KT - 1][r] = -INFINITY;
+        float m = fmaxf(fmaxf(st[0][0], st[0][1]), fmaxf(st[0][2], st[0][3]));
+#pragma unroll
+        for (int kt = 1; kt < KT; ++kt) m = fmaxf(m, fmaxf(fmaxf(st[kt][0], st[kt][1]), fmaxf(st[kt][2], st[kt][3])));
+        m = rowgroup_max(m);
+        float l = 0.f;
+        u32x2 pp[KT];
+#pragma unroll
+        for (int kt = 0; kt < KT; ++kt) {
+          float e[4];
+#pragma unroll
+          for (int r = 0; r < 4; ++r) {
+            e[r] = __builtin_amdgcn_exp2f(st[kt][r] - m);
+            l += e[r];
+          }
+          pp[kt] = (u32x2){pack2_prob<DT>(e[0], e[1]), pack2_prob<DT>(e[2], e[3])};
+        }
+        const float inv = __builtin_amdgcn_rcpf(rowgroup_sum(l));
+#pragma unroll
+        for (int j = 0; j < TJ; ++j) {
+          f32x4 ot = Elem<DT>::mfma16(vf[j][0], pp[0], (f32x4){0.f, 0.f, 0.f, 0.f});
+#pragma unroll
+          for (int kt = 1; kt < KT; ++kt) ot = Elem<DT>::mfma16(vf[j][kt], pp[kt], ot);
+          op[i][j] = (u32x2){pack2<DT>(ot[0] * inv, ot[1] * inv), pack2<DT>(ot[2] * inv, ot[3] * inv)};
+        }
+      }
+      __builtin_amdgcn_sched_barrier(0);
+    }
+    int lane_e = lane;
+    asm volatile("" : "+v"(lane_e));
+    const int l15e = lane_e & 15, ge = lane_e >> 4;
+    const unsigned row_base = (unsigned)(m0 + l15e);
+    AttnOutRegs R;
+    attn_out_prefetch<DT, K>(R, p.out, rs_wo, rs_res, wid, lane_e, row_base, 16u, 32u);
+    __syncthreads();
+#pragma unroll
+    for (int i = 0; i < TM; ++i)
+#pragma unroll
+      for (int j = 0; j < TJ; ++j) {
+        const int col = head * HD + 16 * j + 4 * ge;
+        ca_lds_store8(xb + (16 * i + l15e) * ROWB + (((col >> 3) ^ ((l15e >> 1) & 7)) << 4) + (col & 7) * 2, op[i][j]);
+      }
+    asm volatile("s_waitcnt lgkmcnt(0)" ::: "memory");
+    __syncthreads();
+    attn_out_run<DT, K>(R, xb, fa_b, p.out, rs_wo, rs_bo, rs_o, wid, lane_e, row_base, 16u, 32u, (unsigned)p.ldo);
+  }
+}
diff --git a/controlanimate_amd/kernels.py b/controlanimate_amd/kernels.py
--- a/controlanimate_amd/kernels.py
+++ b/controlanimate_amd/kernels.py
@@ -163,7 +163,7 @@
 def tattn_fused(x: torch.Tensor, w_frag: torch.Tensor, gamma: torch.Tensor, bias_pe: torch.Tensor, b: int, frames: int, tokens: int,
                 heads: int, ln_eps: float, scale: float, *, w_out_frag: Optional[torch.Tensor] = None, bias_out: Optional[torch.Tensor] = None,
                 residual: Optional[torch.Tensor] = None) -> Optional[torch.Tensor]:
-    if not dispatch.tattn_fused:
+    if not dispatch.tattn_fused or (x.shape[-1] == 640 and not dispatch.tattn_fused_c640):
         return None
     _req_cuda(x, w_frag, gamma, bias_pe, w_out_frag, bias_out, residual)
     if x.dim() != 2 or x.stride(1) != 1 or x.shape[0] != b * frames * tokens or bias_pe.shape[0] < frames or bias_pe.stride(1) != 1:
@@ -181,21 +181,25 @@
     if not lib().ca_tattn_fused_supported(C.byref(args)):
         return None
     if _plan_sink is not None:
-        _plan_sink.append("tattn_out128" if w_out_frag is not None else "tattn_fused128")
+        _plan_sink.append("tattn_out64c640" if c == 640 else "tattn_out128" if w_out_frag is not None else "tattn_fused128")
     check(lib().ca_tattn_fused(C.byref(args), _stream()), "ca_tattn_fused")
     return o
 
 
 def xattn_pack_kv(kv: torch.Tensor, kv_batches: int, rows_per_batch: int, nk: int, scale: float, row_offset: int = 0,
                   out: Optional[torch.Tensor] = None) -> Optional[torch.Tensor]:
-    if (not dispatch.xattn_fused or kv.dim() != 2 or kv.shape[1] != 640 or kv.stride(1) != 1 or not (64 < nk <= 80 or 1 <= nk <= 16)
+    if (not dispatch.xattn_fused or kv.dim() != 2 or kv.shape[1] not in (640, 1280) or kv.stride(1) != 1 or not (64 < nk <= 80 or 1 <= nk <= 16)
             or kv.dtype not in (torch.float16, torch.bfloat16)):
         return None
+    wide = kv.shape[1] == 1280
+    if wide and (not dispatch.xattn_fused_c640 or nk <= 64):
+        return None
     _req_cuda(kv)
-    dst = out if out is not None else torch.empty((kv_batches, 8, _capi.XATTN_KV_FRAG_ELEMS), device=kv.device, dtype=kv.dtype)
-    assert dst.shape == (kv_batches, 8, _capi.XATTN_KV_FRAG_ELEMS) and dst.dtype == kv.dtype and dst.is_contiguous()
-    check(lib().ca_xattn_pack_kv(kv.data_ptr(), kv.stride(0), kv_batches, rows_per_batch, row_offset, nk, float(scale), dt_code(kv.dtype),
-                                 dst.data_ptr(), _stream()), "ca_xattn_pack_kv")
+    elems = _capi.XATTN_KV_FRAG_ELEMS_C640 if wide else _capi.XATTN_KV_FRAG_ELEMS
+    dst = out if out is not None else torch.empty((kv_batches, 8, elems), device=kv.device, dtype=kv.dtype)
+    assert dst.shape == (kv_batches, 8, elems) and dst.dtype == kv.dtype and dst.is_contiguous()
+    check(lib().ca_xattn_pack_kv_hd(kv.data_ptr(), kv.stride(0), 80 if wide else 40, kv_batches, rows_per_batch, row_offset, nk, float(scale),
+                                    dt_code(kv.dtype), dst.data_ptr(), _stream()), "ca_xattn_pack_kv_hd")
     return dst
 
 
@@ -203,7 +207,9 @@
                 frames_per_kv: int, kv_mod: int, nk: int, ln_eps: float, *, w_out_frag: Optional[torch.Tensor] = None,
                 bias_out: Optional[torch.Tensor] = None, residual: Optional[torch.Tensor] = None, kv_frag_ip: Optional[torch.Tensor] = None,
                 nk_ip: int = 0, ip_scale: float = 1.0) -> Optional[torch.Tensor]:
-    if not dispatch.xattn_fused or kv_frag is None:
+    if not dispatch.xattn_fused or kv_frag is None or (x.shape[-1] == 640 and not dispatch.xattn_fused_c640):
+        return None
+    if kv_frag.shape[-1] != (_capi.XATTN_KV_FRAG_ELEMS_C640 if x.shape[-1] == 640 else _capi.XATTN_KV_FRAG_ELEMS):
         return None
     _req_cuda(x, wq_frag, bias, kv_frag, w_out_frag, bias_out, residual, kv_frag_ip)
     if kv_frag_ip is not None and (w_out_frag is None or kv_frag_ip.shape != kv_frag.shape or kv_frag_ip.dtype != x.dtype or not kv_frag_ip.is_contiguous()):
@@ -225,7 +231,7 @@
     if not lib().ca_xattn_fused_supported(C.byref(args)):
         return None
     if _plan_sink is not None:
-        _plan_sink.append(("xattn_ip_out128" if kv_frag_ip is not None else "xattn_out128") if w_out_frag is not None else "xattn_fused128")
+        _plan_sink.append("xattn_out64c640" if c == 640 else ("xattn_ip_out128" if kv_frag_ip is not None else "xattn_out128") if w_out_frag is not None else "xattn_fused128")
     check(lib().ca_xattn_fused(C.byref(args), _stream()), "ca_xattn_fused")
     return o
 
diff --git a/controlanimate_amd/layers.py b/controlanimate_amd/layers.py
--- a/controlanimate_amd/layers.py
+++ b/controlanimate_amd/layers.py
@@ -90,6 +90,9 @@
 
 
 def frag_order_tattn(wqkv: torch.Tensor) -> torch.Tensor:
+    if tuple(wqkv.shape) == (1920, 640):
+        x = wqkv.view(3, 8, 5, 16, 20, 4, 8)
+        return x.permute(1, 0, 4, 2, 5, 3, 6).reshape(-1).contiguous()
     assert tuple(wqkv.shape) == (960, 320)
     wpad = wqkv.new_zeros(3, 8, 48, 320)
     wpad[:, :, :40] = wqkv.view(3, 8, 40, 320)
@@ -98,6 +101,9 @@
 
 
 def frag_order_xattn(wq: torch.Tensor) -> torch.Tensor:
+    if tuple(wq.shape) == (640, 640):
+        x = wq.view(8, 5, 16, 20, 4, 8)
+        return x.permute(0, 3, 1, 4, 2, 5).reshape(-1).contiguous()
     assert tuple(wq.shape) == (320, 320)
     wpad = wq.new_zeros(8, 48, 320)
     wpad[:, :40] = wq.view(8, 40, 320)
@@ -106,12 +112,13 @@
 
 
 def frag_order_wout(w: torch.Tensor) -> torch.Tensor:
-    assert tuple(w.shape) == (320, 320)
+    c = w.shape[0]
+    assert tuple(w.shape) in ((320, 320), (640, 640))
     j = torch.arange(5).view(5, 1)
     i = torch.arange(16).view(1, 16)
     col = torch.where(j == 4, 64 + i, 32 * (j >> 1) + 8 * (i >> 2) + 4 * (j & 1) + (i & 3))
-    rows = (torch.arange(4).view(4, 1, 1) * 80 + col.view(1, 5, 16)).to(w.device)
-    x = w[rows.reshape(-1)].view(4, 5, 16, 10, 4, 8)
+    rows = (torch.arange(c // 80).view(c // 80, 1, 1) * 80 + col.view(1, 5, 16)).to(w.device)
+    x = w[rows.reshape(-1)].view(c // 80, 5, 16, c // 32, 4, 8)
     return x.permute(0, 3, 1, 4, 2, 5).reshape(-1).contiguous()
 
 
diff --git a/controlanimate_amd/motion_module.py b/controlanimate_amd/motion_module.py
--- a/controlanimate_amd/motion_module.py
+++ b/controlanimate_amd/motion_module.py
@@ -53,12 +53,14 @@
             self.pos_encoder.pack(arena, dtype)
         self.tfrag = self.tgamma = self.tbias_pe = None
         no_bias = all(getattr(m, "bias", None) is None for m in (self.to_q, self.to_k, self.to_v))
-        if self.fold is not None and pe is not None and no_bias and (self.heads, self.inner_dim, self.query_dim) == (8, 320, 320):
+        if self.fold is not None and pe is not None and no_bias and (self.heads, self.inner_dim, self.query_dim) in ((8, 320, 320), (8, 640, 640)):
             from .layers import _f32, frag_order_tattn
-            self.tfrag = arena.add((368640,), dtype, lambda: frag_order_tattn(torch.cat([_f32(m.weight) for m in (self.to_q, self.to_k, self.to_v)], 0)))
-            self.tgamma = arena.add((320,), torch.float32, lambda: _f32(fold_ln.weight))
-            self.tbias_pe = arena.add((pe.shape[-2], 320), torch.float32,
-                                      lambda: _f32(pe).reshape(pe.shape[-2], 320).to(fold_ln.bias.device) + _f32(fold_ln.bias)[None, :])
+            c = self.query_dim
+            self.tfrag = arena.add((368640 if c == 320 else 1228800,), dtype,
+                                   lambda: frag_order_tattn(torch.cat([_f32(m.weight) for m in (self.to_q, self.to_k, self.to_v)], 0)))
+            self.tgamma = arena.add((c,), torch.float32, lambda: _f32(fold_ln.weight))
+            self.tbias_pe = arena.add((pe.shape[-2], c), torch.float32,
+                                      lambda: _f32(pe).reshape(pe.shape[-2], c).to(fold_ln.bias.device) + _f32(fold_ln.bias)[None, :])
             self.tln_eps = fold_ln.eps
 
     def pos_table(self, frames: int):
diff --git a/include/controlanimate_hip.h b/include/controlanimate_hip.h
--- a/include/controlanimate_hip.h
+++ b/include/controlanimate_hip.h
@@ -7,7 +7,7 @@
 extern "C" {
 #endif
 
-#define CA_ABI_VERSION 15
+#define CA_ABI_VERSION 16
 
 #define CA_BF16 0
 #define CA_F16 1
@@ -120,6 +120,12 @@
 int ca_xattn_pack_w(const void* w, int32_t n, int32_t k, void* dst, void* stream);
 int ca_xattn_pack_kv(const void* kv, int64_t ld, int32_t kv_batches, int32_t rows_per_batch, int32_t row_offset, int32_t nk, float scale, int32_t dtype,
                      void* dst, void* stream);
+#define CA_TATTN_W_FRAG_ELEMS_C640 1228800
+#define CA_ATTN_WOUT_FRAG_ELEMS_C640 409600
+#define CA_XATTN_W_FRAG_ELEMS_C640 409600
+#define CA_XATTN_KV_FRAG_ELEMS_C640 12800
+int ca_xattn_pack_kv_hd(const void* kv, int64_t ld, int32_t head_dim, int32_t kv_batches, int32_t rows_per_batch, int32_t row_offset, int32_t nk, float scale,
+                        int32_t dtype, void* dst, void* stream);
 int64_t ca_gemm_workspace_bytes(const ca_gemm_args* args);
 int ca_gemm_row_sums_parts(const ca_gemm_args* args);
 int ca_gemm_ln_inline_supported(const ca_gemm_args* args);
```

Result: faster. 16.40, median of 6 (+2.2%).
